# halajun/diasss

Hardware: AMD Instinct MI355X
Metric: sonar frames/sec end-to-end (extract+match+LM solve) (higher is better)
Workload: dtype u8/int32 (extract, match) + f64 (geo gate, LM); 1 GPU; 200 synthetic 2000x1024 frames, dense all-pairs; frames=200, pings=2000, bins=1024, pairs=19900

## Files before the change

diasss_amd/csrc/dsss_pg.hip:

```cpp
#include "dsss_internal.h"
#include "dsss_lm.h"
#include <utility>
#include "dsss_pg_kernels.h"
#include <algorithm>
#include <numeric>
#include <random>
#include <cstdlib>
#include <chrono>
#include <thread>
#include <mutex>
#include <future>

namespace {

struct pg_dev {
    dsss_ctx* ctx = nullptr;
    int rc = DSSS_OK;
    static constexpr size_t CHUNK = (size_t)256 << 20;
    template <typename T> int alloc(dsss_ctx* c, T** p, size_t n) { void* q = nullptr; if (!rc) rc = grab(c, &q, std::max<size_t>(n, 1) * sizeof(T)); *p = (T*)q; return rc; }
    int grab(dsss_ctx* c, void** p, size_t n) {
        if (!ctx) { ctx = c; c->pg_chunk_cur = 0; c->pg_chunk_off = 0; }
        const size_t bytes = (n + 255) & ~(size_t)255;
        for (;;) {
            if (c->pg_chunk_cur < c->pg_chunks.size()) {
                auto& ch = c->pg_chunks[c->pg_chunk_cur];
                if (c->pg_chunk_off + bytes <= ch.second) { *p = (char*)ch.first + c->pg_chunk_off; c->pg_chunk_off += bytes; return DSSS_OK; }
                ++c->pg_chunk_cur; c->pg_chunk_off = 0;
                continue;
            }
            void* q = nullptr; const size_t sz = std::max(bytes, CHUNK);
            HIPCHK(c, hipMalloc(&q, sz));
            c->pg_chunks.push_back({ q, sz });
        }
    }
    template <typename T> int upload(dsss_ctx* c, T** p, const std::vector<T>& v) { if (!alloc(c, p, v.size()) && !v.empty()) rc = copy(c, *p, v.data(), v.size() * sizeof(T)); return rc; }
    static int copy(dsss_ctx* c, void* d, const void* h, size_t bytes) { HIPCHK(c, hipMemcpy(d, h, bytes, hipMemcpyHostToDevice)); return DSSS_OK; }
    struct pend { void** p; const void* src; size_t bytes, off; };
    std::vector<pend> pending; size_t pend_total = 0;
    template <typename T> void later(T** p, const std::vector<T>& v) {
        *p = nullptr;
        pending.push_back({ (void**)p, v.data(), v.size() * sizeof(T), pend_total });
        pend_total += (std::max<size_t>(v.size(), 1) * sizeof(T) + 255) & ~(size_t)255;
    }
    hipEvent_t stage_ev = nullptr; bool stage_ev_live = false;
    int flush(dsss_ctx* c, hipStream_t st) { if (!rc) rc = flush_now(c, st); return rc; }
    int flush_now(dsss_ctx* c, hipStream_t st) {
        if (pending.empty()) return DSSS_OK;
        if (stage_ev_live) { hipEventSynchronize(stage_ev); stage_ev_live = false; }
        char* dev = nullptr;
        if (alloc(c, &dev, pend_total)) return rc;
        if (const int r = c->pg_stage.reserve(c, pend_total, pend_total + pend_total / 4)) return r;
        char* stage = c->pg_stage.as<char>();
        const int T = pend_total > ((size_t)1 << 20) ? 4 : 1;
        dsss_pool_run(T, [&](int t) { for (size_t k = t; k < pending.size(); k += T) if (pending[k].bytes) memcpy(stage + pending[k].off, pending[k].src, pending[k].bytes); });
        HIPCHK(c, hipMemcpyAsync(dev, stage, pend_total, hipMemcpyHostToDevice, st));
        if (!stage_ev) stage_ev = event();
        if (stage_ev) { hipEventRecord(stage_ev, st); stage_ev_live = true; }
        for (const pend& q : pending) *q.p = dev + q.off;
        pending.clear(); pend_total = 0;
        return DSSS_OK;
    }
    std::vector<hipEvent_t> events;
    hipEvent_t event() { hipEvent_t e = nullptr; hipEventCreateWithFlags(&e, hipEventDisableTiming); events.push_back(e); return e; }
    void release() { stage_ev_live = false; stage_ev = nullptr; if (ctx) { hipStreamSynchronize(ctx->stream); ctx->pg_chunk_cur = 0; ctx->pg_chunk_off = 0; } for (hipEvent_t e : events) if (e) hipEventDestroy(e); events.clear(); pending.clear(); pend_total = 0; }
};

}

void dsss_pg_free(dsss_ctx* c) { for (auto& ch : c->pg_chunks) hipFree(ch.first); c->pg_chunks.clear(); c->pg_chunk_cur = 0; c->pg_chunk_off = 0; }

namespace {

double ms_since(std::chrono::steady_clock::time_point t) { return std::chrono::duration<double, std::milli>(std::chrono::steady_clock::now() - t).count(); }

struct pg_window { int f0 = 0, p0 = 0; bool online = false; };

struct pg_solve {
    dsss_ctx* const c; const double* const dr6; const int n; const dsss_lc_edge* const edges; const int ne;
    double* const poses12; double* const stats4; double* const rpy6; const int nframes; const int* const ends; const pg_window win;
    const pg_switches sw = pg_switches_read();
    const hipStream_t st;
    int world = 1, rank = 0, nparts = 1, part_lo = 0, part_hi = 1, mp0 = 0, mp1 = 0;
    std::vector<int> foff, pbound;
    pg_weights W;
    std::vector<int> ea, eb, eo; std::vector<pose_t> emeas; std::vector<double> ew;
    std::vector<unsigned long long> tbits; std::vector<int> tpre;
    std::vector<int> sep1, sep_pose, t2, sym_part, ord1, ord2, adj_ptr, adj_edge, lc_link;
    int ns = 0, nseg = 0, ns1 = 0, nseg1 = 0, kp0 = 0, kp1 = 0, nf = 0, nblk = 0;
    std::vector<std::pair<int, int>> redges;
    std::vector<double> cx, cy, sxy; std::vector<unsigned long long> fp;
    static constexpr int chunk = 16;
    pg_analysis A;
    const pg_sym& S = A.S;
    std::promise<void> bottom_prom, lists_prom, coords_prom;
    std::future<void> bottom_fut = bottom_prom.get_future(), lists_fut = lists_prom.get_future(), coords_fut = coords_prom.get_future();
    bool bottom_signalled = false, lists_signalled = false, coords_given = false;
    std::thread sym_thread;
    pg_dev dv;
    pose_t *d_X, *d_Xn, *d_meas, *d_emeas; int *d_ea, *d_eb, *d_eo, *d_adj_ptr, *d_adj_edge, *d_lc_link = nullptr;
    int *d_sep, *d_sep1, *d_t2, *d_ord1, *d_ord2, *d_foff = nullptr; unsigned long long* d_fp = nullptr;
    double *d_dr6, *d_sxy, *d_ew, *d_r, *d_Ji, *d_r2, *d_Ji2, *d_D, *d_C, *d_g, *d_delta, *d_E, *d_Dl, *d_gi, *d_sDL, *d_sDR, *d_sGL, *d_sGR, *d_sS;
    double *d_D1, *d_C1, *d_g1, *d_E1, *d_Dl1, *d_gi1, *d_delta1, *d_s2DL, *d_s2DR, *d_s2GL, *d_s2GR, *d_s2S;
    double *d_part, *d_scal, *d_red; int* d_fail;
    int *d_perm, *d_binperm = nullptr, *d_colptr, *d_rowidx, *d_rlptr, *d_rlcol, *d_rlpos, *d_rlrow, *d_binptr, *d_bincols, *d_dest, *d_map; long long* d_mapptr;
    int *d_binroot_ptr, *d_binroot_idx, *d_broot_b, *d_broot_of_col, *d_anc_first, *d_anc_rel, *d_rel, *d_fa_src, *d_fa_col, *d_fa_tr, *d_frows, *d_xr_ptr;
    int *d_xr_child, *d_xr_row, *d_fa_rowptr, *d_pk_child, *d_pk_row, *d_ifslot = nullptr, *d_ifsep = nullptr;
    long long* d_broot_uoff; pg_front* d_FD; pg_child* d_CH; pg_pack* d_PK;
    double *d_rdiag, *d_x, *d_L, *d_ubin, *d_aval, *d_F, *d_R, *d_FL, *d_Tinv, *d_bwp = nullptr;
    double *d_comm = nullptr, *d_avalif = nullptr, *d_xif = nullptr, *d_commU = nullptr;
    struct dsched { int *lv_front, *lv_step, *asm_front, *asm_row, *tile_item, *tile_ij; } DO = {}, DI = {};
    std::vector<int> ifslot;
    size_t nnzL = 0, ncv = 0, nif = 0, comm_total = 8, if_ld = 0, if_count = 0;
    int nval = 0, bin_lo = 0, bin_hi = 0, nbins = 0, n_pack = 0, f_if = -1, bwd_lds = 0;
    double lambda = 0, err = 0, err0 = 0;
    int iters = 0, nfact = 0;
    bool will_iterate = false, pre_lin = false, pre_chain = false, pre_bins = false;

    pg_solve(dsss_ctx* c_, const double* dr6_, int n_, const dsss_lc_edge* edges_, int ne_, double* poses12_, double* stats4_, double* rpy6_ = nullptr,
             int nframes_ = 0, const int* ends_ = nullptr, pg_window win_ = {})
        : c(c_), dr6(dr6_), n(n_), edges(edges_), ne(ne_), poses12(poses12_), stats4(stats4_), rpy6(rpy6_), nframes(nframes_), ends(ends_), win(win_), st(c_->stream) {}
    ~pg_solve() {
        give_coords();
        if (sym_thread.joinable()) sym_thread.join();
        dv.release();
    }
    void give_coords() { if (!coords_given) { coords_given = true; coords_prom.set_value(); } }

    int run() {
        const auto T0 = std::chrono::steady_clock::now();
        int rc = plan();
        if (rc || (rc = separators())) return rc;
        const auto T1 = std::chrono::steady_clock::now();
        start_analysis();
        if ((rc = upload_dr()) || (rc = upload_chain())) return rc;
        const double t_prep = ms_since(T0);
        if ((rc = upload_links()) || (rc = initial_values()) || (rc = early_trial()) || (rc = join_analysis())) return rc;
        const double t_sym = ms_since(T1);
        const auto T2 = std::chrono::steady_clock::now();
        if ((rc = upload_fronts())) return rc;
        const double t_up = ms_since(T2);
        const auto T3 = std::chrono::steady_clock::now();
        dsss_scope sc(c, DSSS_K_PG);
        if ((rc = lm_loop())) return rc;
        const double t_lm = ms_since(T3);
        const auto T4 = std::chrono::steady_clock::now();
        if ((rc = finish())) return rc;
        if (sw.opt.verbose)
            fprintf(stderr, "[dsss pg] LM iterations %d  factorisations %d  err %.6g -> %.6g | host prep %.1f ms, symbolic %.1f ms, "
                    "alloc+upload %.1f ms, LM loop %.1f ms, download %.1f ms\n", iters, nfact, err0, err, t_prep, t_sym, t_up, t_lm, ms_since(T4));
        return DSSS_OK;
    }

    int plan() {
        if (!dr6) { foff.assign(nframes + 1, 0); for (int f = 0; f < nframes; ++f) foff[f + 1] = foff[f] + c->frames[win.f0 + f].N; }
        if (n < 2) DSSS_FAIL(c, DSSS_E_ARG, "pose graph needs at least 2 poses");
        world = dsss_comm_world(c); rank = dsss_comm_rank(c);
        nparts = std::max(world, c->pg_parts > 0 ? c->pg_parts : world);
        nparts = std::min(nparts, dr6 ? std::max(1, n / 4) : std::max(1, nframes));
        if (nparts < world) DSSS_FAIL(c, DSSS_E_ARG, "%d ranks need at least %d frames", world, world);
        pbound.assign(nparts + 1, n);
        for (int p = 0; p < nparts; ++p) pbound[p] = dr6 ? (int)((long long)n * p / nparts) : foff[(int)((long long)nframes * p / nparts)];
        for (int p = 0; p < nparts; ++p) if (pbound[p + 1] <= pbound[p]) DSSS_FAIL(c, DSSS_E_ARG, "empty pose-graph partition %d", p);
        part_lo = (int)((long long)nparts * rank / world); part_hi = (int)((long long)nparts * (rank + 1) / world);
        mp0 = pbound[part_lo]; mp1 = pbound[part_hi];
        const double PI = DSSS_PI_REF;
        { const double wgt1 = 0.001, wgt2 = 10;
          const double so[6] = { wgt1 * PI / 180, wgt1 * PI / 180, 0.1 * wgt1 * wgt2 * PI / 180, wgt1 * wgt2, wgt1 * wgt2, wgt1 };
          for (int k = 0; k < 6; ++k) { W.prior[k] = 1.0 / 0.000001; W.odo[k] = 1.0 / so[k]; } }
        ea.resize(ne); eb.resize(ne); eo.resize(ne);
        const int TE = ne >= 65536 ? 8 : 1;
        std::vector<int> bad(TE, -1);
        dsss_pool_run(TE, [&](int t) {
            const int e0 = (int)((long long)ne * t / TE), e1 = (int)((long long)ne * (t + 1) / TE);
            for (int e = e0; e < e1; ++e) {
                if (ends) { ea[e] = ends[2 * (size_t)e]; eb[e] = ends[2 * (size_t)e + 1]; } else { ea[e] = edges[e].a; eb[e] = edges[e].b; }
                eo[e] = std::max(ea[e], eb[e]);
                if ((ea[e] < 0 || ea[e] >= n || eb[e] < 0 || eb[e] >= n || ea[e] == eb[e]) && bad[t] < 0) bad[t] = e;
            }
        });
        for (int t = 0; t < TE; ++t) if (bad[t] >= 0) DSSS_FAIL(c, DSSS_E_ARG, "LC edge %d out of range", bad[t]);
        return DSSS_OK;
    }
    void mark(int i) { tbits[(size_t)i >> 6] |= 1ull << (i & 63); }
    static int rank_of(const std::vector<unsigned long long>& bits, const std::vector<int>& pre, int pose) {
        return pre[(size_t)pose >> 6] + __builtin_popcountll(bits[(size_t)pose >> 6] & ((1ull << (pose & 63)) - 1ull));
    }
    int separators() {
        tbits.assign(((size_t)n + 63) / 64, 0ull);
        mark(0); mark(n - 1);
        for (int e = 0; e < ne; ++e) { mark(ea[e]); mark(eb[e]); }
        if (const int rc = nparts > 1 && ne > 0 ? move_boundaries() : DSSS_OK) return rc;
        for (int p = 1; p < nparts; ++p) mark(pbound[p] - 1);
        const int run = 16 * chunk;
        sep_pose.reserve((size_t)2 * ne + nparts + n / run + 8);
        int last = 0;
        for (size_t w = 0; w < tbits.size(); ++w)
            for (unsigned long long bits = tbits[w]; bits; bits &= bits - 1) {
                const int b = (int)(w * 64) + __builtin_ctzll(bits);
                for (;;) {
                    const long long nx = ((long long)last + run + chunk - 1) / chunk * chunk;
                    if (nx >= b) break;
                    sep_pose.push_back((int)nx); last = (int)nx;
                }
                sep_pose.push_back(b); last = b;
            }
        for (int v : sep_pose) mark(v);
        tpre.assign(tbits.size() + 1, 0);
        for (size_t w = 0; w < tbits.size(); ++w) tpre[w + 1] = tpre[w] + __builtin_popcountll(tbits[w]);
        ns = (int)sep_pose.size(); nseg = ns - 1;
        redges.reserve((size_t)ns + ne);
        sym_part.resize(ns);
        { int p = 0; for (int k = 0; k < ns; ++k) { while (p + 1 < nparts && sep_pose[k] >= pbound[p + 1]) ++p; sym_part[k] = p; } }
        return DSSS_OK;
    }
    int move_boundaries() {
        std::vector<int> lc_ends; lc_ends.reserve((size_t)2 * ne + 2);
        for (size_t w = 0; w < tbits.size(); ++w)
            for (unsigned long long bits = tbits[w]; bits; bits &= bits - 1) lc_ends.push_back((int)(w * 64) + __builtin_ctzll(bits));
        std::vector<int> pre(tbits.size() + 1, 0);
        for (size_t w = 0; w < tbits.size(); ++w) pre[w + 1] = pre[w] + __builtin_popcountll(tbits[w]);
        const int m = (int)lc_ends.size();
        std::vector<int> cross(m + 1, 0);
        for (int e = 0; e < ne; ++e) { const int lo = rank_of(tbits, pre, std::min(ea[e], eb[e])), hi = rank_of(tbits, pre, std::max(ea[e], eb[e])); cross[lo + 1]++; cross[hi + 1]--; }
        for (int i = 1; i <= m; ++i) cross[i] += cross[i - 1];
        const int width = n / nparts / 3;
        for (int p = 1; p < nparts; ++p) {
            int bcost = 0;
            const int best = pg_cheapest_gap(lc_ends.data(), cross, pbound[p], width, pbound[p - 1], &bcost);
            if (best > pbound[p - 1] && best < n) pbound[p] = best;
        }
        for (int p = 0; p < nparts; ++p) if (pbound[p + 1] <= pbound[p]) DSSS_FAIL(c, DSSS_E_ARG, "empty pose-graph partition %d", p);
        mp0 = pbound[part_lo]; mp1 = pbound[part_hi];
        return DSSS_OK;
    }

    void start_analysis() {
        cx.resize(ns); cy.resize(ns);
        sym_thread = std::thread([this] {
            pg_sym_opts opt = sw.opt;
            opt.on_bottom_ready = [&] { bottom_signalled = true; bottom_prom.set_value(); };
            opt.on_lists_ready = [&] { lists_signalled = true; lists_prom.set_value(); };
            opt.before_order = [&] { coords_fut.wait(); };
            opt.lists_on_device = true;
            for (int k = 0; k + 1 < ns; ++k) redges.push_back({ k, k + 1 });
            for (int e = 0; e < ne; ++e) redges.push_back({ rank_of(tbits, tpre, ea[e]), rank_of(tbits, tpre, eb[e]) });
            pg_analyse(ns, redges, cx.data(), cy.data(), sym_part.data(), nparts, part_lo, part_hi, world, rank, sw, std::move(opt), A);
            if (!lists_signalled) lists_prom.set_value();
            if (!bottom_signalled) bottom_prom.set_value();
        });
    }

    int upload_dr() {
        dv.alloc(c, &d_dr6, (size_t)n * 6); dv.alloc(c, &d_sxy, (size_t)ns * 2); dv.later(&d_sep, sep_pose);
        sxy.resize((size_t)ns * 2);
        if (!dr6) {
            fp.resize(nframes);
            for (int f = 0; f < nframes; ++f) fp[f] = (unsigned long long)(uintptr_t)c->frames[win.f0 + f].pose6;
            dv.later(&d_fp, fp); dv.later(&d_foff, foff);
        }
        if (dv.flush(c, st)) return dv.rc;
        if (dr6) HIPCHK(c, hipMemcpyAsync(d_dr6, dr6, (size_t)n * 6 * sizeof(double), hipMemcpyHostToDevice, st));
        else {
            hipLaunchKernelGGL(pg_gather_dr_kernel, dim3(8, nframes), dim3(256), 0, st, d_fp, d_foff, d_dr6);
            HIPCHK(c, hipGetLastError());
        }
        hipLaunchKernelGGL(pg_sep_xy_kernel, dim3((ns + 255) / 256), dim3(256), 0, st, ns, d_sep, d_dr6, d_sxy);
        HIPCHK(c, hipGetLastError());
        HIPCHK(c, hipMemcpyAsync(sxy.data(), d_sxy, sxy.size() * sizeof(double), hipMemcpyDeviceToHost, st));
        HIPCHK(c, hipStreamSynchronize(st));
        for (int k = 0; k < ns; ++k) { cx[k] = sxy[2 * (size_t)k]; cy[k] = sxy[2 * (size_t)k + 1]; }
        give_coords();
        emeas.resize(ne); ew.resize((size_t)ne * 6);
        const int TE = ne >= 65536 ? 4 : 1;
        std::vector<int> bad_var(TE, -1), bad_rel(TE, -1);
        dsss_pool_run(TE, [&](int t) {
            const int e0 = (int)((long long)ne * t / TE), e1 = (int)((long long)ne * (t + 1) / TE);
            for (int e = e0; e < e1; ++e) {
                for (int k = 0; k < 9; ++k) emeas[e].R[k] = edges[e].rel[k];
                for (int k = 0; k < 3; ++k) emeas[e].t[k] = edges[e].rel[9 + k];
                for (int k = 0; k < 6; ++k) {
                    if ((!(edges[e].var[k] > 0) || !std::isfinite(edges[e].var[k])) && bad_var[t] < 0) bad_var[t] = e * 6 + k;
                    ew[(size_t)e * 6 + k] = 1.0 / std::sqrt(edges[e].var[k]);
                }
                for (int k = 0; k < 12; ++k) if (!std::isfinite(edges[e].rel[k]) && bad_rel[t] < 0) bad_rel[t] = e;
            }
        });
        for (int t = 0; t < TE; ++t) {
            if (bad_var[t] >= 0) DSSS_FAIL(c, DSSS_E_NUMERIC, "LC edge %d: variance %d is not finite and positive", bad_var[t] / 6, bad_var[t] % 6);
            if (bad_rel[t] >= 0) DSSS_FAIL(c, DSSS_E_NUMERIC, "LC edge %d: relative pose is not finite", bad_rel[t]);
        }
        return DSSS_OK;
    }
    int upload_chain() {
        sep1.reserve(sep_pose.size() + n / chunk + 2); t2.reserve(sep_pose.size());
        for (size_t it = 0, m = 0; it < sep_pose.size() || m < (size_t)n;) {
            const long long a = it < sep_pose.size() ? sep_pose[it] : (1LL << 40), bm = m < (size_t)n ? (long long)m : (1LL << 40);
            if (a <= bm) { t2.push_back((int)sep1.size()); sep1.push_back((int)a); ++it; if (a == bm) m += chunk; }
            else { sep1.push_back((int)bm); m += chunk; }
        }
        ns1 = (int)sep1.size(); nseg1 = ns1 - 1;
        kp0 = (int)(std::lower_bound(sep1.begin(), sep1.end(), mp0) - sep1.begin()); kp1 = (int)(std::lower_bound(sep1.begin(), sep1.end(), mp1) - sep1.begin());
        dv.later(&d_sep1, sep1); dv.later(&d_t2, t2);
        auto by_length = [](const std::vector<int>& ends, std::vector<int>& ord) {
            const int m = (int)ends.size() - 1;
            ord.resize(std::max(m, 1));
            int maxlen = 0;
            for (int k = 0; k < m; ++k) maxlen = std::max(maxlen, ends[k + 1] - ends[k]);
            std::vector<int> cnt(maxlen + 2, 0);
            for (int k = 0; k < m; ++k) cnt[maxlen - (ends[k + 1] - ends[k]) + 1]++;
            for (int l = 0; l <= maxlen; ++l) cnt[l + 1] += cnt[l];
            for (int k = 0; k < m; ++k) ord[cnt[maxlen - (ends[k + 1] - ends[k])]++] = k;
        };
        by_length(sep1, ord1); by_length(t2, ord2);
        dv.later(&d_ord1, ord1); dv.later(&d_ord2, ord2);
        return dv.flush(c, st);
    }
    int upload_links() {
        adj_ptr.assign(n + 1, 0); adj_edge.resize(2 * (size_t)ne);
        for (int e = 0; e < ne; ++e) { adj_ptr[ea[e] + 1]++; adj_ptr[eb[e] + 1]++; }
        for (int i = 0; i < n; ++i) adj_ptr[i + 1] += adj_ptr[i];
        { std::vector<int> fill(adj_ptr.begin(), adj_ptr.end() - 1);
          for (int e = 0; e < ne; ++e) { adj_edge[fill[ea[e]]++] = e << 1; adj_edge[fill[eb[e]]++] = (e << 1) | 1; } }
        bool plain = true;
        for (int e = 0; e < ne && plain; ++e) plain = ea[e] < eb[e] && (e == 0 || eb[e - 1] < eb[e]);
        if (!plain) {
            std::vector<std::pair<unsigned long long, int>> key(ne);
            for (int e = 0; e < ne; ++e) key[e] = { ((unsigned long long)(unsigned)std::min(ea[e], eb[e]) << 32) | (unsigned)std::max(ea[e], eb[e]), e };
            std::sort(key.begin(), key.end());
            bool dups = false;
            for (int k = 0; k + 1 < ne && !dups; ++k) dups = key[k].first == key[k + 1].first;
            if (dups) {
                lc_link.assign((size_t)2 * ne, -1);
                for (int k = 0; k < ne; ++k) {
                    lc_link[2 * (size_t)key[k].second] = (k == 0 || key[k - 1].first != key[k].first) ? 1 : 0;
                    if (k + 1 < ne && key[k + 1].first == key[k].first) lc_link[2 * (size_t)key[k].second + 1] = key[k + 1].second;
                }
            }
        }
        nf = n + ne; nblk = (nf + 255) / 256;
        const size_t sg = std::max(nseg, 1);
        dv.alloc(c, &d_X, n); dv.alloc(c, &d_Xn, n); dv.alloc(c, &d_meas, n); dv.upload(c, &d_emeas, emeas);
        dv.upload(c, &d_ea, ea); dv.upload(c, &d_eb, eb); dv.upload(c, &d_eo, eo); dv.upload(c, &d_ew, ew);
        dv.upload(c, &d_adj_ptr, adj_ptr); dv.upload(c, &d_adj_edge, adj_edge);
        if (!lc_link.empty()) dv.upload(c, &d_lc_link, lc_link);
        dv.alloc(c, &d_r, (size_t)nf * 6); dv.alloc(c, &d_Ji, (size_t)nf * 36);
        dv.alloc(c, &d_r2, (size_t)nf * 6); dv.alloc(c, &d_Ji2, (size_t)nf * 36);
        dv.alloc(c, &d_D, (size_t)n * 36); dv.alloc(c, &d_C, (size_t)n * 36); dv.alloc(c, &d_g, (size_t)n * 6); dv.alloc(c, &d_delta, (size_t)n * 6);
        dv.alloc(c, &d_E, (size_t)n * 36); dv.alloc(c, &d_Dl, (size_t)n * 36); dv.alloc(c, &d_gi, (size_t)n * 6);
        dv.alloc(c, &d_sDL, (size_t)nseg1 * 36); dv.alloc(c, &d_sDR, (size_t)nseg1 * 36); dv.alloc(c, &d_sGL, (size_t)nseg1 * 6);
        dv.alloc(c, &d_sGR, (size_t)nseg1 * 6); dv.alloc(c, &d_sS, (size_t)nseg1 * 36);
        dv.alloc(c, &d_D1, (size_t)ns1 * 36); dv.alloc(c, &d_C1, (size_t)ns1 * 36); dv.alloc(c, &d_g1, (size_t)ns1 * 6); dv.alloc(c, &d_delta1, (size_t)ns1 * 6);
        dv.alloc(c, &d_E1, (size_t)ns1 * 36); dv.alloc(c, &d_Dl1, (size_t)ns1 * 36); dv.alloc(c, &d_gi1, (size_t)ns1 * 6);
        dv.alloc(c, &d_s2DL, sg * 36); dv.alloc(c, &d_s2DR, sg * 36); dv.alloc(c, &d_s2GL, sg * 6); dv.alloc(c, &d_s2GR, sg * 6); dv.alloc(c, &d_s2S, sg * 36);
        dv.alloc(c, &d_rdiag, (size_t)ns * 6);
        dv.alloc(c, &d_x, (size_t)ns * 6); dv.alloc(c, &d_part, (size_t)nblk); dv.alloc(c, &d_scal, 8); dv.alloc(c, &d_fail, 1); dv.alloc(c, &d_red, 8);
        return dv.rc;
    }

    int reduce_scalars(double* host3, int* failed) {
        if (world > 1) {
            hipLaunchKernelGGL(pg_comm_scal_kernel, dim3(1), dim3(64), 0, st, d_scal, d_fail, d_red);
            if (const int rc = dsss_comm_allreduce(c, d_red, 4, st)) return rc;
            double h4[4];
            HIPCHK(c, hipMemcpyAsync(h4, d_red, 4 * sizeof(double), hipMemcpyDeviceToHost, st));
            HIPCHK(c, hipStreamSynchronize(st));
            host3[0] = h4[0]; host3[1] = h4[1]; host3[2] = h4[2]; *failed = h4[3] != 0.0;
        } else {
            if (const int r = c->pg_scal_host.reserve(c, 8 * sizeof(double))) return r;
            double* const scal_host = c->pg_scal_host.as<double>();
            HIPCHK(c, hipMemcpyAsync(scal_host, d_scal, 3 * sizeof(double), hipMemcpyDeviceToHost, st));
            HIPCHK(c, hipMemcpyAsync(scal_host + 4, d_fail, sizeof(int), hipMemcpyDeviceToHost, st));
            HIPCHK(c, hipStreamSynchronize(st));
            host3[0] = scal_host[0]; host3[1] = scal_host[1]; host3[2] = scal_host[2];
            *failed = *reinterpret_cast<const int*>(scal_host + 4);
        }
        return DSSS_OK;
    }
    int initial_values() {
        double* d_norm = nullptr;
        if (c->pg.add_noise) {
            const long long need_pairs = 3LL * n;
            long long natt = (long long)(need_pairs * 1.32) + 4096;
            for (int attempt = 0;; ++attempt) {
                double* d_pairs; int* d_flags; int* d_bsum; int* d_total;
                const int nb = (int)((natt + 4095) / 4096);
                dv.alloc(c, &d_pairs, (size_t)natt * 2); dv.alloc(c, &d_flags, (size_t)natt); dv.alloc(c, &d_bsum, (size_t)nb); dv.alloc(c, &d_total, 1);
                if (!d_norm) dv.alloc(c, &d_norm, (size_t)need_pairs * 2);
                if (dv.rc) return dv.rc;
                const long long nthr = (natt + RNG_PER_THREAD - 1) / RNG_PER_THREAD;
                hipLaunchKernelGGL(pg_rng_attempts_kernel, dim3((unsigned)((nthr + 255) / 256)), dim3(256), 0, st, natt, d_pairs, d_flags);
                hipLaunchKernelGGL(pg_flag_blocksum_kernel, dim3(nb), dim3(256), 0, st, d_flags, natt, d_bsum);
                hipLaunchKernelGGL(pg_flag_scan_kernel, dim3(1), dim3(256), 0, st, d_bsum, nb, d_total);
                hipLaunchKernelGGL(pg_flag_compact_kernel, dim3(nb), dim3(256), 0, st, d_flags, d_pairs, natt, d_bsum, need_pairs, d_norm);
                int total_ok = 0;
                HIPCHK(c, hipMemcpyAsync(&total_ok, d_total, sizeof(int), hipMemcpyDeviceToHost, st));
                HIPCHK(c, hipStreamSynchronize(st));
                if (total_ok >= need_pairs) break;
                if (attempt > 3) DSSS_FAIL(c, DSSS_E_NUMERIC, "normal generator: not enough accepted attempts");
                natt *= 2;
            }
        }
        hipLaunchKernelGGL(pg_init_kernel, dim3((n + 255) / 256), dim3(256), 0, st, n, d_dr6, d_norm, c->pg.add_noise, d_X, d_meas);
        if (win.online && c->pg_warm_n > win.p0) {
            const pose_t* warm = c->pg_warm.as<const pose_t>() + win.p0;
            HIPCHK(c, hipMemcpyAsync(d_X, warm, (size_t)std::min(n, c->pg_warm_n - win.p0) * sizeof(pose_t), hipMemcpyDeviceToDevice, st));
            if (win.p0 > 0) HIPCHK(c, hipMemcpyAsync(d_meas, warm, sizeof(pose_t), hipMemcpyDeviceToDevice, st));
        }
        hipLaunchKernelGGL(pg_linearize_kernel<false>, dim3(nblk), dim3(256), 0, st, n, ne, d_X, d_meas, W, d_ea, d_eb, d_eo, d_emeas, d_ew, (double*)nullptr, (double*)nullptr, d_part, mp0, mp1);
        hipLaunchKernelGGL(pg_final_sum_kernel, dim3(1), dim3(256), 0, st, d_part, nblk, 0.5, d_scal);
        double h3[3]; int failed = 0;
        HIPCHK(c, hipMemsetAsync(d_fail, 0, sizeof(int), st));
        if (const int rc = reduce_scalars(h3, &failed)) return rc;
        lambda = c->pg.lambda0; err = err0 = h3[0];
        return DSSS_OK;
    }

    void chain_part() {
        hipMemsetAsync(d_fail, 0, sizeof(int), st);
        hipLaunchKernelGGL(pg_assemble_kernel, dim3((ns1 + PG_ASM_POSES - 1) / PG_ASM_POSES), dim3(6 * PG_ASM_POSES), 0, st, n, W, d_r, d_Ji, d_adj_ptr, d_adj_edge, d_ew, d_scal + 3, d_D, d_C, d_g, d_eo, mp0, mp1, d_sep1, ns1);
        hipLaunchKernelGGL(pg_segment_kernel<true>, dim3((nseg1 + 31) / 32), dim3(256), 0, st, nseg1, d_ord1, d_sep1, d_D, d_C, d_g, d_E, d_Dl, d_gi, d_sDL, d_sDR, d_sGL, d_sGR, d_sS, d_fail, mp0, mp1, d_r, d_Ji, W, d_scal + 3);
        hipLaunchKernelGGL(pg_chain1_kernel, dim3((unsigned)(((long long)ns1 * 42 + 255) / 256)), dim3(256), 0, st, ns1, d_sep1, d_D, d_g, d_sDL, d_sDR, d_sGL, d_sGR, d_sS, d_D1, d_C1, d_g1, mp0, mp1);
        if (nseg > 0) hipLaunchKernelGGL(pg_segment_kernel<false>, dim3((nseg + 31) / 32), dim3(256), 0, st, nseg, d_ord2, d_t2, d_D1, d_C1, d_g1, d_E1, d_Dl1, d_gi1, d_s2DL, d_s2DR, d_s2GL, d_s2GR, d_s2S, d_fail, kp0, kp1, (const double*)nullptr, (const double*)nullptr, W, (const double*)nullptr);
    }
    int early_trial() {
        will_iterate = err > 0 && c->pg.max_iters > 0;
        if (!will_iterate) return DSSS_OK;
        hipLaunchKernelGGL(pg_linearize_kernel<true>, dim3(nblk), dim3(256), 0, st, n, ne, d_X, d_meas, W, d_ea, d_eb, d_eo, d_emeas, d_ew, d_r, d_Ji, d_part, mp0, mp1);
        hipLaunchKernelGGL(pg_final_sum_kernel, dim3(1), dim3(256), 0, st, d_part, nblk, 0.5, d_scal);
        HIPCHK(c, hipMemcpyAsync(d_scal + 3, &lambda, sizeof(double), hipMemcpyHostToDevice, st));
        chain_part();
        pre_lin = pre_chain = true;
        if (nparts > 1) return DSSS_OK;
        lists_fut.wait();
        if (const int rc = upload_lists()) return rc;
        bottom_fut.wait();
        if (const int rc = upload_bottom()) return rc;
        bottom_trial(0.0);
        pre_bins = true;
        return DSSS_OK;
    }
    int upload_lists() {
        nnzL = S.rowidx.size();
        const int nsa = S.ns;
        char* d_binned = nullptr; int* d_rootof = nullptr;
        dv.later(&d_colptr, S.colptr); dv.later(&d_rowidx, S.rowidx); dv.later(&d_binned, S.binned); dv.later(&d_rootof, S.root_of);
        dv.flush(c, st);
        int *d_cnt, *d_cur, *d_bs32, *d_tot32; long long *d_bs64, *d_tot64;
        const int nsb = (nsa + 1023) / 1024;
        dv.alloc(c, &d_cnt, (size_t)nsa); dv.alloc(c, &d_cur, (size_t)nsa); dv.alloc(c, &d_bs32, (size_t)nsb); dv.alloc(c, &d_tot32, 1);
        dv.alloc(c, &d_bs64, (size_t)nsb); dv.alloc(c, &d_tot64, 1); dv.alloc(c, &d_rlptr, (size_t)nsa + 1); dv.alloc(c, &d_mapptr, (size_t)nsa + 1);
        dv.alloc(c, &d_rlcol, nnzL); dv.alloc(c, &d_rlpos, nnzL); dv.alloc(c, &d_rlrow, nnzL);
        if (dv.alloc(c, &d_anc_first, (size_t)nsa) || dv.alloc(c, &d_anc_rel, nnzL)) return dv.rc;
        if (nsb > 1024 * 1024) DSSS_FAIL(c, DSSS_E_CAPACITY, "%d separators", nsa);
        hipMemsetAsync(d_cnt, 0, sizeof(int) * (size_t)nsa, st); hipMemsetAsync(d_cur, 0, sizeof(int) * (size_t)nsa, st);
        hipMemsetAsync(d_anc_first, 0, sizeof(int) * (size_t)nsa, st); hipMemsetAsync(d_anc_rel, 0xff, sizeof(int) * nnzL, st);
        const dim3 gcol((nsa + 255) / 256);
        hipLaunchKernelGGL(pg_rl_count_kernel, gcol, dim3(256), 0, st, nsa, d_colptr, d_rowidx, d_binned, d_cnt);
        hipLaunchKernelGGL((pg_scan_block_kernel<int, 0>), dim3(nsb), dim3(1024), 0, st, nsa, d_cnt, d_colptr, d_rlptr, d_bs32);
        hipLaunchKernelGGL((pg_scan_tops_kernel<int>), dim3(1), dim3(1024), 0, st, nsb, d_bs32, d_tot32);
        hipLaunchKernelGGL((pg_scan_add_kernel<int>), dim3(nsb), dim3(1024), 0, st, nsa, d_rlptr, d_bs32, d_tot32);
        hipLaunchKernelGGL((pg_scan_block_kernel<long long, 1>), dim3(nsb), dim3(1024), 0, st, nsa, d_cnt, d_colptr, d_mapptr, d_bs64);
        hipLaunchKernelGGL((pg_scan_tops_kernel<long long>), dim3(1), dim3(1024), 0, st, nsb, d_bs64, d_tot64);
        hipLaunchKernelGGL((pg_scan_add_kernel<long long>), dim3(nsb), dim3(1024), 0, st, nsa, d_mapptr, d_bs64, d_tot64);
        hipLaunchKernelGGL(pg_rl_fill_kernel, gcol, dim3(256), 0, st, nsa, d_colptr, d_rowidx, d_binned, d_rlptr, d_cur, d_rlcol, d_rlpos);
        hipLaunchKernelGGL(pg_rl_sort_kernel, dim3((nsa + 3) / 4), dim3(256), 0, st, nsa, d_rlptr, d_rlcol, d_rlpos, d_rlrow, d_fail);
        hipLaunchKernelGGL(pg_anc_rel_kernel, gcol, dim3(256), 0, st, nsa, d_colptr, d_rowidx, d_binned, d_rootof, d_anc_first, d_anc_rel);
        const long long mapsz = 42LL * (long long)nnzL; const int nupd = (int)nnzL;
        if (mapsz > (1LL << 31)) DSSS_FAIL(c, DSSS_E_CAPACITY, "update map bound of %lld entries", mapsz);
        if (dv.alloc(c, &d_map, (size_t)mapsz)) return dv.rc;
        hipLaunchKernelGGL(pg_fill_map_kernel, dim3(2048), dim3(256), 0, st, d_map, d_tot64);
        if (nupd > 0) hipLaunchKernelGGL(pg_build_map_kernel, dim3((nupd + 255) / 256), dim3(256), 0, st, nupd, d_rlrow, d_rlptr, d_rlcol, d_rlpos, d_colptr, d_rowidx, d_mapptr, d_map, d_tot32);
        return DSSS_OK;
    }
    int upload_bottom() {
        nnzL = S.rowidx.size(); nval = A.local ? (int)A.dest_g.size() : (int)S.dest_bin.size();
        ncv = S.comm_vals.size(); nif = S.iface_seps.size();
        comm_total = ncv * 36 + nif * 6 + (size_t)S.comm_doubles + 8;
        dv.later(&d_perm, A.local ? A.perm_g : S.perm);
        dv.alloc(c, &d_L, nnzL * 36); dv.alloc(c, &d_ubin, (size_t)S.ubin_doubles);
        if (dv.alloc(c, &d_aval, (size_t)nval * 36 + comm_total)) return dv.rc;
        d_comm = d_aval + (size_t)nval * 36; d_avalif = d_comm; d_xif = d_comm + ncv * 36; d_commU = d_xif + nif * 6;
        if (A.local) ifslot.swap(A.ifslot_g);
        else { ifslot.assign(ns, -1); for (size_t q = 0; q < nif; ++q) ifslot[S.iface_seps[q]] = (int)q; }
        dv.later(&d_ifslot, ifslot); dv.later(&d_ifsep, A.local ? A.ifsep_g : S.iface_seps);
        dv.later(&d_binptr, S.binptr); dv.later(&d_bincols, S.bincols); dv.later(&d_binperm, S.bin_perm);
        dv.later(&d_dest, A.local ? A.dest_g : S.dest_bin);
        dv.later(&d_binroot_ptr, S.binroot_ptr); dv.later(&d_binroot_idx, S.binroot_idx); dv.later(&d_broot_b, S.broot_b); dv.later(&d_broot_uoff, S.broot_uoff);
        dv.later(&d_broot_of_col, S.broot_of_col);
        if (dv.flush(c, st)) return dv.rc;
        { const int nb_all = (int)S.binptr.size() - 1, sel_lo = A.local ? 0 : part_lo, sel_hi = A.local ? 1 : part_hi;
          bin_lo = 0; while (bin_lo < nb_all && S.bin_part[bin_lo] < sel_lo) ++bin_lo; bin_hi = bin_lo; while (bin_hi < nb_all && S.bin_part[bin_hi] < sel_hi) ++bin_hi; }
        nbins = bin_hi - bin_lo;
        return DSSS_OK;
    }
    void bottom_trial(double bins_flops) {
        hipMemsetAsync(d_L, 0, nnzL * 36 * sizeof(double), st);
        if (nparts > 1) hipMemsetAsync(d_comm, 0, comm_total * sizeof(double), st);
        hipLaunchKernelGGL(pg_scatter_base_kernel, dim3((unsigned)(((long long)ns * 78 + 255) / 256)), dim3(256), 0, st, ns, d_t2, d_perm, d_D1, d_g1, d_s2DL, d_s2DR, d_s2GL, d_s2GR, d_s2S, d_dest, d_L, d_aval, d_x,
                           d_ifslot, d_avalif, d_xif, kp0, kp1);
        if (ne > 0) hipLaunchKernelGGL(pg_scatter_lc_kernel, dim3((unsigned)(((long long)ne * 36 + 255) / 256)), dim3(256), 0, st, n, ne, ns, d_Ji, d_ew, d_dest, d_L, d_aval, d_avalif, d_eo, mp0, mp1, d_lc_link);
        if (nbins > 0) { dsss_scope s1(c, DSSS_K_PG_SUBTREE, bins_flops);
                         hipLaunchKernelGGL(sw.bins_serial ? pg_factor_subtree_serial_kernel : pg_factor_subtree_kernel, dim3(nbins), dim3(256), 0, st, d_binperm + bin_lo, d_binptr, d_bincols, d_colptr, d_rlptr, d_rlcol, d_rlpos, d_mapptr, d_map, d_L, d_x, d_fail,
                                            d_binroot_ptr, d_binroot_idx, d_broot_b, d_broot_uoff, d_broot_of_col, d_anc_first, d_anc_rel, d_ubin, d_rdiag); }
    }
    int join_analysis() {
        sym_thread.join();
        if (S.ownership_violations) DSSS_FAIL(c, DSSS_E_STATE, "pose-graph analysis: %d separators with a higher-rank neighbour are not interface", S.ownership_violations);
        return DSSS_OK;
    }

    int upload_fronts() {
        if (!pre_bins) {
            if (const int rc = upload_lists()) return rc;
            if (const int rc = upload_bottom()) return rc;
        } else if (c->prof.on) c->prof.work[DSSS_K_PG_SUBTREE] += std::max(0.0, S.flops_factor - S.flops_fronts);
        if (sw.opt.verbose)
            fprintf(stderr, "[dsss pg] rank %d/%d parts %d (own %d..%d, poses %d..%d)  %s analysis of %d separators  poses %d  LC edges %d  separators %d "
                    "(interface %zu)  nnz(L) blocks %zu  bins %d (%d cols)  fronts %d (largest %d block rows, arena %.0f MB)  panels %d in %d levels  "
                    "all-reduce %.1f MB\n", rank, world, nparts, part_lo, part_hi, mp0, mp1, A.local ? "rank-local" : "replicated", S.ns, n, ne, ns,
                    S.iface_seps.size(), nnzL, (int)S.binptr.size() - 1, (int)S.bincols.size(), (int)S.f_c0.size(), S.max_front_n, S.front_doubles * 8e-6,
                    S.npanels, S.nlev, (S.comm_doubles + 36.0 * S.comm_vals.size() + 6.0 * S.iface_seps.size()) * 8e-6);
        const int nfr = (int)S.f_c0.size();
        f_if = A.local && !S.iface_seps.empty() ? nfr - 1 : -1;
        if_ld = f_if >= 0 ? (size_t)S.f_ld[f_if] : 0; if_count = if_ld * if_ld + if_ld;
        if (f_if >= 0 && (S.f_part[f_if] != -1 || S.f_off[f_if] + (long long)(if_ld * if_ld) != S.front_doubles))
            DSSS_FAIL(c, DSSS_E_STATE, "pose-graph analysis: the interface front is not the last one");
        dv.alloc(c, &d_F, (size_t)S.front_doubles + if_ld); dv.alloc(c, &d_R, (size_t)S.frhs_doubles); dv.alloc(c, &d_FL, (size_t)S.front_doubles);
        dv.later(&d_rel, S.rel); dv.later(&d_fa_src, S.fa_src); dv.later(&d_fa_col, S.fa_col); dv.later(&d_fa_tr, S.fa_tr);
        dv.later(&d_frows, S.f_rows); dv.later(&d_xr_ptr, S.xr_ptr); dv.later(&d_xr_child, S.xr_child);
        dv.later(&d_xr_row, S.xr_row); dv.later(&d_fa_rowptr, S.fa_rowptr);
        for (int w2 = 0; w2 < 2; ++w2) {
            const pg_sched& H = w2 ? A.SI : A.SO; dsched& Dv = w2 ? DI : DO;
            dv.later(&Dv.lv_front, H.lv_front); dv.later(&Dv.lv_step, H.lv_step); dv.later(&Dv.asm_front, H.asmrow_front); dv.later(&Dv.asm_row, H.asmrow_row);
            dv.later(&Dv.tile_item, H.tile_item); dv.later(&Dv.tile_ij, H.tile_ij);
        }
        std::vector<pg_front> FD(nfr); std::vector<pg_child> CH(S.ch_kind.size());
        for (int f = 0; f < nfr; ++f) {
            pg_front& d = FD[f];
            d.off = S.f_off[f]; d.roff = S.f_roff[f]; d.ld = S.f_ld[f]; d.n6 = 6 * S.f_n[f]; d.s6 = 6 * S.f_s[f]; d.c0 = S.f_c0[f];
            d.rowptr = S.f_rowptr[f]; d.pan0 = S.f_pan0[f]; d.ch0 = S.ch_ptr[f]; d.ch1 = S.ch_ptr[f + 1]; d.fa0 = S.fa_ptr[f]; d.fa1 = S.fa_ptr[f + 1];
            if (f == f_if) d.roff = (d_F + S.front_doubles) - d_R;
        }
        for (size_t q = 0; q < CH.size(); ++q) {
            pg_child& d = CH[q]; d.relptr = S.ch_relptr[q];
            if (S.ch_kind[q]) { const int ri = S.ch_id[q]; d.cb = S.broot_b[ri]; d.cld = 6 * d.cb; d.U = d_ubin + S.broot_uoff[ri]; d.g = d.U + (size_t)d.cld * d.cld; }
            else { const int gf = S.ch_id[q]; d.cb = S.f_n[gf] - S.f_s[gf]; d.cld = S.f_ld[gf]; d.U = d_F + S.f_off[gf] + (size_t)(6 * S.f_s[gf]) * d.cld + 6 * S.f_s[gf]; d.g = d_R + S.f_roff[gf] + 6 * S.f_s[gf]; }
        }
        std::vector<int> comm_of_front(nfr, -1), comm_of_broot(S.broot.size(), -1);
        for (size_t q = 0; q < S.comm_kind.size(); ++q) (S.comm_kind[q] ? comm_of_broot[S.comm_id[q]] : comm_of_front[S.comm_id[q]]) = (int)q;
        std::vector<pg_pack> PK(S.comm_kind.size()); std::vector<int> pk_child, pk_row;
        for (int f = 0; f < nfr; ++f) {
            if (S.f_part[f] >= 0) continue;
            for (int q = S.ch_ptr[f]; q < S.ch_ptr[f + 1]; ++q) {
                const int cq = S.ch_kind[q] ? comm_of_broot[S.ch_id[q]] : comm_of_front[S.ch_id[q]];
                if (cq < 0) continue;
                pg_child& d = CH[q];
                pg_pack& k = PK[cq]; k.U = d.U; k.g = d.g; k.cld = d.cld; k.cb = d.cb; k.dst = d_commU + S.comm_off[cq];
                d.U = k.dst; d.cld = 6 * d.cb; d.g = d.U + (size_t)d.cld * d.cld;
                if (S.comm_part[cq] >= part_lo && S.comm_part[cq] < part_hi) for (int r2 = 0; r2 < d.cb; ++r2) { pk_child.push_back(cq); pk_row.push_back(r2); }
            }
        }
        dv.later(&d_FD, FD); dv.later(&d_CH, CH); dv.later(&d_PK, PK); dv.later(&d_pk_child, pk_child); dv.later(&d_pk_row, pk_row);
        if (dv.flush(c, st)) return dv.rc;
        n_pack = (int)pk_child.size();
        const int max_n6 = std::max(A.SO.max_n6, A.SI.max_n6);
        c->pg_last_levels.clear();
        for (const pg_sched* H : { &A.SO, &A.SI })
            for (int l = 0; l < H->nlev; ++l) {
                const int nit = H->lv_ptr[l + 1] - H->lv_ptr[l];
                if (nit > 0) c->pg_last_levels.insert(c->pg_last_levels.end(), { nit, H->max_w6[l], H->max_rows[l], H == &A.SI ? 1 : 0 });
            }
        dv.alloc(c, &d_Tinv, (size_t)std::max(S.npanels, 1) * PG_NB4 * 16);
        size_t need = 0;
        for (const pg_sched* H : { &A.SO, &A.SI })
            for (int l = 0; l < H->nlev; ++l)
                if (64 * H->trsm_chunks[l] > PG_BWD_SPLIT) need = std::max(need, (size_t)(H->lv_ptr[l + 1] - H->lv_ptr[l]) * ((64 * H->trsm_chunks[l] + PG_BWD_RC - 1) / PG_BWD_RC) * 96);
        if ((need > 0 && dv.alloc(c, &d_bwp, need)) || dv.rc) return dv.rc;
        bwd_lds = (int)(((PG_PW * 6) * PG_BWD2_LD + PG_NB4 * 16 + 10 * (PG_PW * 6) + std::min(max_n6, PG_BWD2_SX) + 16) * sizeof(double));
        if (bwd_lds > 160 * 1024) DSSS_FAIL(c, DSSS_E_CAPACITY, "front of %d scalar rows: back-substitution needs %d B of LDS", max_n6, bwd_lds);
        hipFuncSetAttribute((const void*)pg_front_bwd2_kernel, hipFuncAttributeMaxDynamicSharedMemorySize, 160 * 1024);
        (void)hipGetLastError();
        return DSSS_OK;
    }

    void run_levels(const pg_sched& H, const dsched& Dv, int part = 0) {
        for (int l = 0; l < H.nlev; ++l) {
            const int nas = part == 2 ? 0 : H.asmrow_ptr[l + 1] - H.asmrow_ptr[l], nit = part == 1 ? 0 : H.lv_ptr[l + 1] - H.lv_ptr[l], ntl = H.tile_ptr[l + 1] - H.tile_ptr[l];
            const int* itf = Dv.lv_front + H.lv_ptr[l]; const int* its = Dv.lv_step + H.lv_ptr[l];
            if (nas > 0) { dsss_scope s2(c, DSSS_K_PG_ASM);
                hipLaunchKernelGGL(pg_front_asm_kernel, dim3(nas), dim3(256), 0, st, Dv.asm_front + H.asmrow_ptr[l], Dv.asm_row + H.asmrow_ptr[l], d_FD, d_CH, d_rel, d_xr_ptr, d_xr_child, d_xr_row,
                                   d_fa_rowptr, d_fa_src, d_fa_col, d_fa_tr, d_aval, d_x, d_F, d_R); }
            if (nit == 0) continue;
            { dsss_scope s3(c, DSSS_K_PG_DIAG, H.fl_diag[l]);
              hipLaunchKernelGGL(pg_front_diag4_kernel, dim3(nit), dim3(256), 0, st, itf, its, d_FD, d_F, d_R, d_fail, d_Tinv); }
            if (ntl > 0 && ntl <= PG_RSU_MAX_TILES) {
                dsss_scope s45(c, DSSS_K_PG_RSU, H.fl_trsm[l] + H.fl_syrk[l]);
                if (ntl <= PG_RSU32_MAX_TILES)
                    hipLaunchKernelGGL(pg_front_rsu_kernel<32>, dim3(4 * ntl), dim3(256), 0, st, itf, its, d_FD, Dv.tile_item + H.tile_ptr[l], Dv.tile_ij + H.tile_ptr[l], d_F, d_FL, d_R, d_Tinv);
                else hipLaunchKernelGGL(pg_front_rsu_kernel<64>, dim3(ntl), dim3(512), 0, st, itf, its, d_FD, Dv.tile_item + H.tile_ptr[l], Dv.tile_ij + H.tile_ptr[l], d_F, d_FL, d_R, d_Tinv);
            } else if (H.trsm_chunks[l] > 0) {
                { dsss_scope s4(c, DSSS_K_PG_TRSM, H.fl_trsm[l]);
                  hipLaunchKernelGGL(pg_front_trsm2_kernel, dim3(nit, H.trsm_chunks[l]), dim3(256), 0, st, itf, its, d_FD, d_F, d_R, d_Tinv); }
                { dsss_scope s5(c, DSSS_K_PG_ACC, H.fl_syrk[l]);
                  if (ntl > 0) hipLaunchKernelGGL(pg_front_syrk_kernel, dim3(ntl), dim3(256), 0, st, itf, its, d_FD, Dv.tile_item + H.tile_ptr[l], Dv.tile_ij + H.tile_ptr[l], d_F); }
            }
        }
    }
    void run_levels_bwd(const pg_sched& H, const dsched& Dv) {
        for (int l = H.nlev - 1; l >= 0; --l) {
            const int nit = H.lv_ptr[l + 1] - H.lv_ptr[l];
            if (nit == 0) continue;
            dsss_scope s6(c, DSSS_K_PG_BWD, H.fl_bwd[l], 2);
            const int ntl = H.tile_ptr[l + 1] - H.tile_ptr[l];
            const double* Fl = (ntl > 0 && ntl <= PG_RSU_MAX_TILES) ? d_FL : d_F;
            const int nch = 64 * H.trsm_chunks[l] > PG_BWD_SPLIT ? (64 * H.trsm_chunks[l] + PG_BWD_RC - 1) / PG_BWD_RC : 0;
            if (nch > 0) hipLaunchKernelGGL(pg_front_bwd_part_kernel, dim3(nch, nit), dim3(1024), 0, st, Dv.lv_front + H.lv_ptr[l], Dv.lv_step + H.lv_ptr[l], d_FD, d_frows, Fl, d_x, d_bwp, nch);
            hipLaunchKernelGGL(pg_front_bwd2_kernel, dim3(nit), dim3(1024), bwd_lds, st, Dv.lv_front + H.lv_ptr[l], Dv.lv_step + H.lv_ptr[l], d_FD, d_frows, d_F, Fl, d_R, d_x, d_Tinv,
                               nch > 0 ? (const double*)d_bwp : (const double*)nullptr, nch);
        }
    }
    int trial() {
        if (!pre_chain) {
            HIPCHK(c, hipMemcpyAsync(d_scal + 3, &lambda, sizeof(double), hipMemcpyHostToDevice, st));
            chain_part();
        }
        pre_chain = false;
        if (!pre_bins) bottom_trial(std::max(0.0, S.flops_factor - S.flops_fronts));
        pre_bins = false;
        run_levels(A.SO, DO);
        if (A.local) {
            if (f_if >= 0) {
                hipLaunchKernelGGL(pg_comm_xif_kernel, dim3(((int)nif + 255) / 256), dim3(256), 0, st, (int)nif, d_ifsep, d_perm, d_xif, d_x);
                hipMemsetAsync(d_F + S.f_off[f_if], 0, if_count * sizeof(double), st);
                run_levels(A.SI, DI, 1);
                { dsss_scope s8(c, DSSS_K_PG_COMM, (double)if_count * 8);
                  if (const int rc = dsss_comm_allreduce(c, d_F + S.f_off[f_if], if_count, st)) return rc; }
                run_levels(A.SI, DI, 2);
                run_levels_bwd(A.SI, DI);
            }
        } else if (nparts > 1) {
            if (n_pack > 0) hipLaunchKernelGGL(pg_comm_pack_kernel, dim3(n_pack), dim3(256), 0, st, d_pk_child, d_pk_row, d_PK);
            { dsss_scope s8(c, DSSS_K_PG_COMM, (double)comm_total * 8);
              if (const int rc = dsss_comm_allreduce(c, d_comm, comm_total - 8, st)) return rc; }
            if (nif > 0) hipLaunchKernelGGL(pg_comm_xif_kernel, dim3(((int)nif + 255) / 256), dim3(256), 0, st, (int)nif, d_ifsep, d_perm, d_xif, d_x);
            run_levels(A.SI, DI);
            run_levels_bwd(A.SI, DI);
        }
        run_levels_bwd(A.SO, DO);
        if (nbins > 0) { dsss_scope s7(c, DSSS_K_PG_SUBTREE);
            hipLaunchKernelGGL(pg_bwd_subtree_kernel, dim3(nbins), dim3(64), 0, st, d_binperm + bin_lo, d_binptr, d_bincols, d_colptr, d_rowidx, d_L, d_x, d_rdiag); }
        hipLaunchKernelGGL(pg_sep_delta_kernel, dim3((ns + 255) / 256), dim3(256), 0, st, ns, d_t2, d_perm, d_x, d_delta1);
        if (nseg > 0)
            hipLaunchKernelGGL(pg_backsub_kernel<false>, dim3((nseg + 31) / 32), dim3(256), 0, st, nseg, d_ord2, d_t2, d_C1, d_E1, d_Dl1, d_gi1, d_delta1, kp0, kp1, (const double*)nullptr, W);
        hipLaunchKernelGGL(pg_sep_delta_kernel, dim3((ns1 + 255) / 256), dim3(256), 0, st, ns1, d_sep1, (const int*)nullptr, d_delta1, d_delta);
        hipLaunchKernelGGL(pg_backsub_kernel<true>, dim3((nseg1 + 31) / 32), dim3(256), 0, st, nseg1, d_ord1, d_sep1, d_C, d_E, d_Dl, d_gi, d_delta, mp0, mp1, d_Ji, W);
        hipLaunchKernelGGL(pg_linerr_kernel, dim3(nblk), dim3(256), 0, st, n, ne, W, d_ea, d_eb, d_eo, d_ew, d_r, d_Ji, d_delta, d_part, mp0, mp1);
        hipLaunchKernelGGL(pg_final_sum_kernel, dim3(1), dim3(256), 0, st, d_part, nblk, 0.5, d_scal + 1);
        return DSSS_OK;
    }

    int lm_loop() {
        const lm_rule R = { c->pg.rel_tol, c->pg.abs_tol, c->pg.lambda_max, c->pg.min_fidelity, c->pg.lambda_factor, c->pg.max_iters };
        double cur = 0;
        if (will_iterate) do {
            cur = err;
            double oldLin = err;
            if (!pre_lin) {
                hipLaunchKernelGGL(pg_linearize_kernel<true>, dim3(nblk), dim3(256), 0, st, n, ne, d_X, d_meas, W, d_ea, d_eb, d_eo, d_emeas, d_ew, d_r, d_Ji, d_part, mp0, mp1);
                hipLaunchKernelGGL(pg_final_sum_kernel, dim3(1), dim3(256), 0, st, d_part, nblk, 0.5, d_scal);
            }
            pre_lin = false;
            for (;;) {
                if (const int rc = trial()) return rc;
                ++nfact;
                hipLaunchKernelGGL(pg_retract_kernel, dim3((n + 255) / 256), dim3(256), 0, st, n, d_X, d_delta, d_Xn);
                hipLaunchKernelGGL(pg_linearize_kernel<true>, dim3(nblk), dim3(256), 0, st, n, ne, d_Xn, d_meas, W, d_ea, d_eb, d_eo, d_emeas, d_ew, d_r2, d_Ji2, d_part, mp0, mp1);
                hipLaunchKernelGGL(pg_final_sum_kernel, dim3(1), dim3(256), 0, st, d_part, nblk, 0.5, d_scal + 2);
                HIPCHK(c, hipGetLastError());
                double h[3]; int failed = 0;
                if (const int rc = reduce_scalars(h, &failed)) return rc;
                const lm_verdict v = !failed && std::isfinite(h[1]) ? lm_judge(R, oldLin, h[1], err, h[2]) : lm_verdict{ false, false };
                if (v.success) { std::swap(d_X, d_Xn); std::swap(d_r, d_r2); std::swap(d_Ji, d_Ji2); pre_lin = true; err = h[2]; lm_accepted(R, &lambda); ++iters; break; }
                if (v.stop || lm_refused(R, &lambda)) break;
            }
        } while (lm_continue(R, iters, cur, err));
        return DSSS_OK;
    }

    int finish() {
        if (world > 1) {
            size_t maxlen = 0;
            std::vector<int> r_lo(world), r_len(world);
            for (int r = 0; r < world; ++r) {
                r_lo[r] = pbound[(int)((long long)nparts * r / world)]; r_len[r] = pbound[(int)((long long)nparts * (r + 1) / world)] - r_lo[r];
                maxlen = std::max(maxlen, (size_t)r_len[r]);
            }
            const size_t slice = maxlen * sizeof(pose_t);
            char* d_gath;
            if (dv.alloc(c, &d_gath, slice * (size_t)world)) return dv.rc;
            HIPCHK(c, hipMemcpyAsync(d_gath + slice * (size_t)rank, d_X + mp0, (size_t)(mp1 - mp0) * sizeof(pose_t), hipMemcpyDeviceToDevice, st));
            if (const int rc = dsss_comm_allgather(c, d_gath, slice, st)) return rc;
            for (int r = 0; r < world; ++r)
                if (r != rank && r_len[r] > 0) HIPCHK(c, hipMemcpyAsync(d_X + r_lo[r], d_gath + slice * (size_t)r, (size_t)r_len[r] * sizeof(pose_t), hipMemcpyDeviceToDevice, st));
        }
        static_assert(sizeof(pose_t) == 12 * sizeof(double), "pose_t layout");
        const int p0 = win.p0;
        if (win.online) {
            const size_t all = (size_t)p0 + (size_t)n;
            if (const int r = c->pg_warm.reserve_keep(c, all * sizeof(pose_t), (all + all / 2 + 1024) * sizeof(pose_t), (size_t)p0 * sizeof(pose_t))) return r;
            HIPCHK(c, hipMemcpyAsync(c->pg_warm.as<pose_t>() + p0, d_X, (size_t)n * sizeof(pose_t), hipMemcpyDeviceToDevice, st));
            c->pg_warm_n = (int)all;
        }
        const pose_t* d_out = p0 > 0 ? c->pg_warm.as<const pose_t>() : d_X;
        const int n_out = p0 + n;
        if (poses12)
            HIPCHK(c, hipMemcpyAsync(poses12, d_out, (size_t)n_out * sizeof(pose_t), hipMemcpyDeviceToHost, st));
        if (rpy6) {
            double* d_rpy;
            if (dv.alloc(c, &d_rpy, (size_t)n_out * 6)) return dv.rc;
            hipLaunchKernelGGL(pg_rpy_kernel, dim3((n_out + 255) / 256), dim3(256), 0, st, n_out, d_out, d_rpy);
            HIPCHK(c, hipMemcpyAsync(rpy6, d_rpy, (size_t)n_out * 6 * sizeof(double), hipMemcpyDeviceToHost, st));
        }
        HIPCHK(c, hipStreamSynchronize(st));
        if (stats4) { stats4[0] = iters; stats4[1] = err0; stats4[2] = err; stats4[3] = lambda; }
        c->pg_last_trials = nfact;
        return DSSS_OK;
    }
};

}

__global__ __launch_bounds__(256) void lc_select_kernel(const double* __restrict__ kp7, int n, const int* __restrict__ kp7_pair,
                                                        const int* __restrict__ kp7_off, const int* __restrict__ act_t,
                                                        const int* __restrict__ frame_off, unsigned long long* __restrict__ slot)
{
    const int i = blockIdx.x * 256 + threadIdx.x;
    if (i >= n) return;
    const int p = kp7_pair[i];
    const int t = act_t[p];
    const int ping = (int)kp7[(size_t)i * 7 + 3];
    const unsigned long long key = ((unsigned long long)(unsigned)(p + 1) << 32) | (unsigned long long)(0xffffffffu - (unsigned)(i - kp7_off[p]));
    atomicMax(&slot[frame_off[t] + ping], key);
}

__global__ __launch_bounds__(256) void lc_edge_flag_kernel(const unsigned long long* __restrict__ slot, int total, const int* __restrict__ kp7_off,
                                                           const dsss_lc* __restrict__ lcs, int* __restrict__ flags)
{
    const int g = blockIdx.x * 256 + threadIdx.x;
    if (g >= total) return;
    const unsigned long long key = slot[g];
    int f = 0;
    if (key) {
        const int p = (int)(key >> 32) - 1, k = (int)(0xffffffffu - (unsigned)(key & 0xffffffffu));
        const dsss_lc& m = lcs[kp7_off[p] + k];
        f = m.score > 0 && isfinite(m.score);
        for (int q = 0; q < 6; ++q) f = f && m.var[q] > 0 && isfinite(m.var[q]);
    }
    flags[g] = f;
}

#define PG_AB_PREFIX 32768
static int pg_select_impl(dsss_ctx* c, int nframes, dsss_lc_edge* edges, int cap, int* n_edges, const int** ends)
{
    if (!c || nframes <= 0 || nframes > c->max_frames) return DSSS_E_ARG;
    if (!c->has_lc) DSSS_FAIL(c, DSSS_E_STATE, "dsss_lc_solve_all has not run");
    HIPCHK(c, hipSetDevice(c->device));
    std::vector<int> off(nframes + 1, 0);
    for (int f = 0; f < nframes; ++f) {
        if (!c->frames[f].has_geom) DSSS_FAIL(c, DSSS_E_STATE, "frame %d has no geometry", f);
        off[f + 1] = off[f] + c->frames[f].N;
    }
    const int total = off[nframes], n = c->total_kp7;
    int ne = 0;
    if (n > 0) {
        for (int p = 0; p < c->npairs; ++p)
            if (c->pair_s[p] >= nframes || c->pair_t[p] >= nframes) DSSS_FAIL(c, DSSS_E_ARG, "pair %d references a frame >= nframes", p);
        pg_dev dv;
        unsigned long long* d_slot; int *d_off, *d_flags, *d_bsum, *d_total; dsss_lc_edge* d_edges; int2* d_ab = nullptr;
        const int nb = (total + 4095) / 4096;
        int rc = dv.alloc(c, &d_slot, (size_t)total); if (rc) return rc;
        rc = dv.alloc(c, &d_off, (size_t)nframes + 1); if (rc) return rc;
        rc = dv.alloc(c, &d_flags, (size_t)total); if (rc) return rc;
        rc = dv.alloc(c, &d_bsum, (size_t)nb); if (rc) return rc;
        rc = dv.alloc(c, &d_total, 1); if (rc) return rc;
        rc = dv.alloc(c, &d_edges, (size_t)cap); if (rc) return rc;
        if (ends) {
            rc = dv.alloc(c, &d_ab, (size_t)cap); if (rc) return rc;
            if ((rc = c->pg_ab_host.reserve(c, (size_t)cap * sizeof(int2)))) return rc;
        }
        hipStream_t st = c->stream;
        HIPCHK(c, hipMemsetAsync(d_slot, 0, (size_t)total * sizeof(unsigned long long), st));
        HIPCHK(c, hipMemcpyAsync(d_off, off.data(), (nframes + 1) * sizeof(int), hipMemcpyHostToDevice, st));
        hipLaunchKernelGGL(lc_select_kernel, dim3((n + 255) / 256), dim3(256), 0, st, c->kp7, n, c->kp7_pair, c->kp7_off, c->act_t, d_off, d_slot);
        hipLaunchKernelGGL(lc_edge_flag_kernel, dim3((total + 255) / 256), dim3(256), 0, st, d_slot, total, c->kp7_off, c->lcs.as<dsss_lc>(), d_flags);
        hipLaunchKernelGGL(pg_flag_blocksum_kernel, dim3(nb), dim3(256), 0, st, d_flags, (long long)total, d_bsum);
        hipLaunchKernelGGL(pg_flag_scan_kernel, dim3(1), dim3(256), 0, st, d_bsum, nb, d_total);
        hipLaunchKernelGGL(lc_edge_compact_kernel, dim3(nb), dim3(256), 0, st, d_flags, d_bsum, d_slot, total, c->kp7_off, c->kp7, c->lcs.as<dsss_lc>(), c->act_s, d_off, cap, d_edges, d_ab);
        HIPCHK(c, hipGetLastError());
        HIPCHK(c, hipMemcpyAsync(&ne, d_total, sizeof(int), hipMemcpyDeviceToHost, st));
        const int pre = std::min(cap, PG_AB_PREFIX);
        if (ends) HIPCHK(c, hipMemcpyAsync(c->pg_ab_host.p, d_ab, (size_t)pre * sizeof(int2), hipMemcpyDeviceToHost, st));
        HIPCHK(c, hipStreamSynchronize(st));
        if (ne > cap) { dv.release(); DSSS_FAIL(c, DSSS_E_CAPACITY, "more than %d LC edges", cap); }
        if (ends) {
            if (ne > pre) { HIPCHK(c, hipMemcpyAsync(c->pg_ab_host.as<int>() + 2 * (size_t)pre, d_ab + pre, (size_t)(ne - pre) * sizeof(int2), hipMemcpyDeviceToHost, st)); HIPCHK(c, hipStreamSynchronize(st)); }
            if (ne > 0) HIPCHK(c, hipMemcpyAsync(edges, d_edges, (size_t)ne * sizeof(dsss_lc_edge), hipMemcpyDeviceToHost, st));
            *ends = c->pg_ab_host.as<int>();
        }
        else if (ne > 0) HIPCHK(c, hipMemcpy(edges, d_edges, (size_t)ne * sizeof(dsss_lc_edge), hipMemcpyDeviceToHost));
        dv.release();
    }
    else if (ends) *ends = nullptr;
    if (n_edges) *n_edges = ne;
    return DSSS_OK;
}

static int pg_exchange_edges(dsss_ctx* c, dsss_lc_edge** edges, int* n_edges)
{
    const int world = dsss_comm_world(c), rank = dsss_comm_rank(c);
    dsss_lc_edge* edges_p = *edges;
    int ne = *n_edges, rc;
    std::vector<double> cnt(world, 0.0); cnt[rank] = ne;
    auto xch = [&](size_t n) { return c->xch_dev.reserve(c, n * sizeof(double), (n + n / 2 + 1024) * sizeof(double)); };
    rc = xch(world); if (rc) return rc;
    double* d_tmp = c->xch_dev.as<double>();
    hipError_t e = hipMemcpyAsync(d_tmp, cnt.data(), world * sizeof(double), hipMemcpyHostToDevice, c->stream);
    if (e == hipSuccess) { rc = dsss_comm_allreduce(c, d_tmp, world, c->stream); if (rc) return rc; }
    if (e == hipSuccess) e = hipMemcpyAsync(cnt.data(), d_tmp, world * sizeof(double), hipMemcpyDeviceToHost, c->stream);
    if (e == hipSuccess) e = hipStreamSynchronize(c->stream);
    HIPCHK(c, e);
    size_t tot = 0, maxc = 0;
    for (int r = 0; r < world; ++r) { tot += (size_t)cnt[r]; maxc = std::max(maxc, (size_t)cnt[r]); }
    if (tot > 0) {
        const size_t slice = maxc * sizeof(dsss_lc_edge), all = slice * (size_t)world;
        rc = xch((2 * all + sizeof(double) - 1) / sizeof(double)); if (rc) return rc;
        if ((rc = c->xch_host.reserve(c, all, all + all / 2))) return rc;
        char* d_all = c->xch_dev.as<char>();
        char* d_cmp = d_all + all;
        e = hipSuccess;
        if (ne > 0) e = hipMemcpyAsync(d_all + slice * (size_t)rank, edges_p, (size_t)ne * sizeof(dsss_lc_edge), hipMemcpyHostToDevice, c->stream);
        if (e == hipSuccess) { rc = dsss_comm_allgather(c, d_all, slice, c->stream); if (rc) return rc; }
        size_t w = 0;
        for (int r = 0; r < world && e == hipSuccess; ++r) {
            const size_t k = (size_t)cnt[r];
            if (k) e = hipMemcpyAsync(d_cmp + w * sizeof(dsss_lc_edge), d_all + slice * (size_t)r, k * sizeof(dsss_lc_edge), hipMemcpyDeviceToDevice, c->stream);
            w += k;
        }
        if (e == hipSuccess) e = hipMemcpyAsync(c->xch_host.p, d_cmp, tot * sizeof(dsss_lc_edge), hipMemcpyDeviceToHost, c->stream);
        if (e == hipSuccess) e = hipStreamSynchronize(c->stream);
        HIPCHK(c, e);
        edges_p = c->xch_host.as<dsss_lc_edge>();
    }
    ne = (int)tot;
    bool ascending = true;
    for (int i = 1; i < ne && ascending; ++i) ascending = edges_p[i - 1].b <= edges_p[i].b;
    if (!ascending) std::stable_sort(edges_p, edges_p + ne, [](const dsss_lc_edge& x, const dsss_lc_edge& y) { return x.b < y.b; });
    *edges = edges_p; *n_edges = ne;
    return DSSS_OK;
}

extern "C" {

int dsss_posegraph_select(dsss_ctx* c, int nframes, dsss_lc_edge* edges, int cap, int* n_edges) { return pg_select_impl(c, nframes, edges, cap, n_edges, nullptr); }

int dsss_posegraph_solve_edges(dsss_ctx* c, const double* dr6, int total, const dsss_lc_edge* edges, int ne, double* poses12, double* stats4)
{
    if (!c || !dr6 || total <= 0 || ne < 0 || (ne > 0 && !edges)) return DSSS_E_ARG;
    HIPCHK(c, hipSetDevice(c->device));
    std::vector<double> h_dr((size_t)total * 6);
    HIPCHK(c, hipMemcpy(h_dr.data(), dr6, h_dr.size() * sizeof(double), hipMemcpyDefault));
    std::vector<dsss_lc_edge> h_e(ne);
    if (ne) HIPCHK(c, hipMemcpy(h_e.data(), edges, (size_t)ne * sizeof(dsss_lc_edge), hipMemcpyDefault));
    return pg_solve(c, h_dr.data(), total, h_e.data(), ne, poses12, stats4).run();
}

int dsss_posegraph_solve(dsss_ctx* c, int nframes, double* poses12, double* rpy6, double* stats4)
{
    if (!c || nframes <= 0 || nframes > c->max_frames) return DSSS_E_ARG;
    const auto t0 = std::chrono::steady_clock::now();
    auto ms = [&](std::chrono::steady_clock::time_point a) { return std::chrono::duration<double, std::milli>(std::chrono::steady_clock::now() - a).count(); };
    size_t total = 0;
    for (int f = 0; f < nframes; ++f) {
        if (!c->frames[f].has_geom) DSSS_FAIL(c, DSSS_E_STATE, "frame %d has no geometry", f);
        total += (size_t)c->frames[f].N;
    }
    const size_t ecap = (size_t)std::max(c->total_kp7, 1);
    if (const int r = c->pg_edges_host.reserve(c, ecap * sizeof(dsss_lc_edge))) return r;
    dsss_lc_edge* edges_p = c->pg_edges_host.as<dsss_lc_edge>();
    int ne = 0;
    const double t_dr = ms(t0);
    const auto t1 = std::chrono::steady_clock::now();
    const int world = dsss_comm_world(c);
    const int* ends = nullptr;
    int rc = pg_select_impl(c, nframes, edges_p, (int)ecap, &ne, world == 1 ? &ends : nullptr);
    if (rc) return rc;
    if (world > 1 && (rc = pg_exchange_edges(c, &edges_p, &ne))) return rc;
    const double t_sel = ms(t1);
    const auto t2 = std::chrono::steady_clock::now();
    rc = pg_solve(c, nullptr, (int)total, edges_p, ne, poses12, stats4, rpy6, nframes, ends).run();
    if (rc) return rc;
    if (pg_switches_read().opt.verbose) fprintf(stderr, "[dsss pg] DR rows %.1f ms, LC selection %.1f ms, solve + download %.1f ms\n", t_dr, t_sel, ms(t2));
    return DSSS_OK;
}

int dsss_posegraph_reset(dsss_ctx* c)
{
    if (!c) return DSSS_E_ARG;
    c->pg_inc_edges.clear(); c->pg_inc_gen = c->lc_gen; c->pg_warm_n = 0;
    return DSSS_OK;
}

int dsss_posegraph_online_edges(dsss_ctx* c) { return c ? (int)c->pg_inc_edges.size() : DSSS_E_ARG; }

int dsss_posegraph_schedule_get(dsss_ctx* c, int* levels4, int cap_levels, int* n_levels, int* n_trials)
{
    if (!c || (cap_levels > 0 && !levels4)) return DSSS_E_ARG;
    const int nl = (int)(c->pg_last_levels.size() / 4);
    if (n_levels) *n_levels = nl;
    if (n_trials) *n_trials = c->pg_last_trials;
    for (int l = 0; l < std::min(nl, cap_levels); ++l) for (int k = 0; k < 4; ++k) levels4[4 * l + k] = c->pg_last_levels[4 * (size_t)l + k];
    return DSSS_OK;
}

static int pg_update_impl(dsss_ctx* c, int nframes, int window_frames, double* poses12, double* rpy6, double* stats4)
{
    if (!c || nframes <= 0 || nframes > c->max_frames) return DSSS_E_ARG;
    if (dsss_comm_world(c) > 1) DSSS_FAIL(c, DSSS_E_STATE, "dsss_posegraph_update is a single-rank call (the online use is one vehicle, one GPU)");
    size_t total = 0;
    for (int f = 0; f < nframes; ++f) {
        if (!c->frames[f].has_geom) DSSS_FAIL(c, DSSS_E_STATE, "frame %d has no geometry", f);
        total += (size_t)c->frames[f].N;
    }
    for (const dsss_lc_edge& e : c->pg_inc_edges)
        if (e.a >= (int)total || e.b >= (int)total)
            DSSS_FAIL(c, DSSS_E_ARG, "an accumulated LC edge references ping %d of %zu: nframes went down; dsss_posegraph_reset first", std::max(e.a, e.b), total);
    if (c->has_lc && c->pg_inc_gen != c->lc_gen && c->total_kp7 > 0) {
        std::vector<dsss_lc_edge> fresh((size_t)c->total_kp7);
        int ne = 0;
        const int rc = dsss_posegraph_select(c, nframes, fresh.data(), (int)fresh.size(), &ne);
        if (rc) return rc;
        if (ne > 0 && !c->pg_inc_edges.empty()) {
            std::vector<char> hit(total, 0);
            for (int e = 0; e < ne; ++e) hit[fresh[e].b] = 1;
            size_t w = 0;
            for (size_t e = 0; e < c->pg_inc_edges.size(); ++e) if (!hit[c->pg_inc_edges[e].b]) c->pg_inc_edges[w++] = c->pg_inc_edges[e];
            c->pg_inc_edges.resize(w);
        }
        const bool append_only = ne == 0 || c->pg_inc_edges.empty() || c->pg_inc_edges.back().b <= fresh[0].b;
        c->pg_inc_edges.insert(c->pg_inc_edges.end(), fresh.begin(), fresh.begin() + ne);
        if (!append_only) std::stable_sort(c->pg_inc_edges.begin(), c->pg_inc_edges.end(), [](const dsss_lc_edge& x, const dsss_lc_edge& y) { return x.b < y.b; });
    }
    c->pg_inc_gen = c->lc_gen;
    int f0 = window_frames > 0 ? std::max(0, nframes - window_frames) : 0;
    int p0 = 0;
    for (int f = 0; f < f0; ++f) p0 += c->frames[f].N;
    while (f0 > 0 && c->pg_warm_n <= p0) { --f0; p0 -= c->frames[f0].N; }
    if (f0 == 0)
        return pg_solve(c, nullptr, (int)total, c->pg_inc_edges.data(), (int)c->pg_inc_edges.size(), poses12, stats4, rpy6, nframes, nullptr, { 0, 0, true }).run();
    std::vector<dsss_lc_edge> we; std::vector<int> frozen;
    for (const dsss_lc_edge& e : c->pg_inc_edges) {
        if (std::max(e.a, e.b) < p0) continue;
        if (e.a >= p0 && e.b >= p0) { dsss_lc_edge w = e; w.a -= p0; w.b -= p0; we.push_back(w); continue; }
        if (e.a > e.b) DSSS_FAIL(c, DSSS_E_ARG, "window update: loop closure %d -> %d runs from the window into the frozen part (the pipeline's closures end in the later frame)", e.a, e.b);
        dsss_lc_edge w = e; w.b -= p0; w.a = -1 - (int)frozen.size(); frozen.push_back(e.a); we.push_back(w);
    }
    if (!frozen.empty()) {
        HIPCHK(c, hipSetDevice(c->device));
        std::vector<int> idx(frozen); idx.push_back(p0);
        pg_dev gv;
        int* d_idx = nullptr; pose_t* d_g = nullptr;
        int rg = gv.alloc(c, &d_idx, idx.size()); if (rg) return rg;
        rg = gv.alloc(c, &d_g, idx.size()); if (rg) { gv.release(); return rg; }
        std::vector<pose_t> g(idx.size());
        hipError_t e = hipMemcpyAsync(d_idx, idx.data(), idx.size() * sizeof(int), hipMemcpyHostToDevice, c->stream);
        if (e == hipSuccess) { hipLaunchKernelGGL(pg_gather_pose_kernel, dim3(((int)idx.size() + 255) / 256), dim3(256), 0, c->stream, (int)idx.size(), d_idx, c->pg_warm.as<const pose_t>(), d_g); e = hipGetLastError(); }
        if (e == hipSuccess) e = hipMemcpyAsync(g.data(), d_g, g.size() * sizeof(pose_t), hipMemcpyDeviceToHost, c->stream);
        gv.release();
        HIPCHK(c, e);
        pose_t X0inv; pose_inverse(&g.back(), &X0inv);
        for (dsss_lc_edge& w : we) {
            if (w.a >= 0) continue;
            const pose_t& Xa = g[(size_t)(-1 - w.a)];
            pose_t rel, Y, M;
            for (int k = 0; k < 9; ++k) rel.R[k] = w.rel[k];
            for (int k = 0; k < 3; ++k) rel.t[k] = w.rel[9 + k];
            pose_compose(&X0inv, &Xa, &Y); pose_compose(&Y, &rel, &M);
            for (int k = 0; k < 9; ++k) w.rel[k] = M.R[k];
            for (int k = 0; k < 3; ++k) w.rel[9 + k] = M.t[k];
            w.a = 0;
        }
    }
    return pg_solve(c, nullptr, (int)total - p0, we.data(), (int)we.size(), poses12, stats4, rpy6, nframes - f0, nullptr, { f0, p0, true }).run();
}

int dsss_posegraph_update(dsss_ctx* c, int nframes, double* poses12, double* rpy6, double* stats4) { return pg_update_impl(c, nframes, 0, poses12, rpy6, stats4); }
int dsss_posegraph_update_window(dsss_ctx* c, int nframes, int window_frames, double* poses12, double* rpy6, double* stats4)
{
    if (window_frames < 1) { if (c) c->err = "window_frames must be at least 1"; return DSSS_E_ARG; }
    return pg_update_impl(c, nframes, window_frames, poses12, rpy6, stats4);
}

}
```

diasss_amd/csrc/dsss_pg_bins.hip:

```cpp
#include "dsss_pg_kernels.h"
#include "dsss_pg_dev.h"
#pragma clang fp contract(fast)
__global__ __launch_bounds__(256) void pg_build_map_kernel(int nupd, const int* __restrict__ rlrow, const int* __restrict__ rlptr,
                                                           const int* __restrict__ rlcol, const int* __restrict__ rlpos,
                                                           const int* __restrict__ colptr, const int* __restrict__ rowidx,
                                                           const long long* __restrict__ mapptr, int* __restrict__ upd_map, const int* __restrict__ nupd_dev)
{
    const int e = blockIdx.x * 256 + threadIdx.x;
    if (e >= (nupd_dev ? *nupd_dev : nupd)) return;
    const int j = rlrow[e], k = rlcol[e];
    const int c0 = colptr[j], m = colptr[j + 1] - c0;
    int* mp = upd_map + mapptr[j] + (long long)(e - rlptr[j]) * m;
    int q = 0;
    for (int p = rlpos[e]; p < colptr[k + 1]; ++p) {
        const int i = rowidx[p];
        while (q < m && rowidx[c0 + q] < i) ++q;
        if (q < m && rowidx[c0 + q] == i) mp[q] = p;
    }
}

__global__ __launch_bounds__(256) void pg_rl_count_kernel(int ns, const int* __restrict__ colptr, const int* __restrict__ rowidx, const char* __restrict__ binned,
                                                          int* __restrict__ cnt)
{
    const int k = blockIdx.x * 256 + threadIdx.x;
    if (k >= ns || !binned[k]) return;
    for (int q = colptr[k] + 1; q < colptr[k + 1]; ++q) { const int j = rowidx[q]; if (binned[j]) atomicAdd(&cnt[j], 1); }
}
template <typename T, int VAL>
__global__ __launch_bounds__(1024) void pg_scan_block_kernel(int n, const int* __restrict__ cnt, const int* __restrict__ colptr, T* __restrict__ out, T* __restrict__ block_sum)
{
    __shared__ T s_w[16];
    const int i = blockIdx.x * 1024 + threadIdx.x;
    T v = 0, tot;
    if (i < n) v = VAL == 0 ? (T)cnt[i] : (T)cnt[i] * (T)(colptr[i + 1] - colptr[i]);
    const T pos = dsss_block_scan_excl<16, T>(v, &tot, s_w);
    if (i < n) out[i] = pos;
    if (threadIdx.x == 0) block_sum[blockIdx.x] = tot;
}
template <typename T>
__global__ __launch_bounds__(1024) void pg_scan_tops_kernel(int nblocks, T* __restrict__ block_sum, T* __restrict__ total)
{
    __shared__ T s_w[16];
    T carry = 0;
    for (int b0 = 0; b0 < nblocks; b0 += 1024) {
        const int i = b0 + threadIdx.x;
        const T v = i < nblocks ? block_sum[i] : (T)0;
        T tot;
        const T pos = dsss_block_scan_excl<16, T>(v, &tot, s_w);
        if (i < nblocks) block_sum[i] = carry + pos;
        carry += tot;
    }
    if (threadIdx.x == 0) *total = carry;
}
template <typename T>
__global__ __launch_bounds__(1024) void pg_scan_add_kernel(int n, T* __restrict__ out, const T* __restrict__ block_sum, const T* __restrict__ total)
{
    const int i = blockIdx.x * 1024 + threadIdx.x;
    if (i < n) out[i] += block_sum[blockIdx.x];
    if (i == 0) out[n] = *total;
}
__global__ __launch_bounds__(256) void pg_rl_fill_kernel(int ns, const int* __restrict__ colptr, const int* __restrict__ rowidx, const char* __restrict__ binned,
                                                         const int* __restrict__ rlptr, int* __restrict__ cur, int* __restrict__ rlcol, int* __restrict__ rlpos)
{
    const int k = blockIdx.x * 256 + threadIdx.x;
    if (k >= ns || !binned[k]) return;
    for (int q = colptr[k] + 1; q < colptr[k + 1]; ++q) {
        const int j = rowidx[q];
        if (!binned[j]) continue;
        const int at = rlptr[j] + atomicAdd(&cur[j], 1);
        rlcol[at] = k; rlpos[at] = q;
    }
}
#define PG_RL_SORT_CAP 1024
__global__ __launch_bounds__(256) void pg_rl_sort_kernel(int ns, const int* __restrict__ rlptr, int* __restrict__ rlcol, int* __restrict__ rlpos, int* __restrict__ rlrow,
                                                         int* __restrict__ fail)
{
    __shared__ int s_k[4][PG_RL_SORT_CAP], s_q[4][PG_RL_SORT_CAP];
    const int wv = threadIdx.x >> 6, lane = threadIdx.x & 63;
    const int j = blockIdx.x * 4 + wv;
    if (j >= ns) return;
    const int b = rlptr[j], len = rlptr[j + 1] - b;
    if (len <= 0) return;
    if (len > PG_RL_SORT_CAP) { if (lane == 0) *fail = 2; return; }
    for (int e = lane; e < len; e += 64) { s_k[wv][e] = rlcol[b + e]; s_q[wv][e] = rlpos[b + e]; }
    asm volatile("s_waitcnt vmcnt(0) lgkmcnt(0)" ::: "memory"); __builtin_amdgcn_wave_barrier();
    for (int e = lane; e < len; e += 64) {
        const int key = s_k[wv][e];
        int rank = 0;
        for (int f = 0; f < len; ++f) rank += s_k[wv][f] < key;
        rlcol[b + rank] = key; rlpos[b + rank] = s_q[wv][e]; rlrow[b + rank] = j;
    }
}
__global__ __launch_bounds__(256) void pg_fill_map_kernel(int* __restrict__ upd_map, const long long* __restrict__ total)
{
    const long long n = *total;
    for (long long i = (long long)blockIdx.x * 256 + threadIdx.x; i < n; i += (long long)gridDim.x * 256) upd_map[i] = -1;
}
__global__ __launch_bounds__(256) void pg_anc_rel_kernel(int ns, const int* __restrict__ colptr, const int* __restrict__ rowidx, const char* __restrict__ binned,
                                                         const int* __restrict__ root_of, int* __restrict__ anc_first, int* __restrict__ anc_rel)
{
    const int k = blockIdx.x * 256 + threadIdx.x;
    if (k >= ns || !binned[k]) return;
    const int r = root_of[k], c0 = colptr[k], m = colptr[k + 1] - c0;
    int q = 0;
    while (q < m && rowidx[c0 + q] <= r) ++q;
    anc_first[k] = q;
    const int* __restrict__ rb = rowidx + colptr[r] + 1; const int nb = colptr[r + 1] - colptr[r] - 1;
    int w = 0;
    for (; q < m; ++q) { const int row = rowidx[c0 + q]; while (w < nb && rb[w] < row) ++w; anc_rel[c0 + q] = (w < nb && rb[w] == row) ? w : -1; }
}

#define PG_TCH 128
__device__ inline void pg_acc_rows(const int* __restrict__ mp, int m, int tn, const double* __restrict__ Lvals, int r,
                                   const double* __restrict__ s_Ljk, double* acc)
{
    int t = 0;
    for (; t + 4 <= tn; t += 4) {
        int pos[4]; double a[4][6];
#pragma unroll
        for (int u = 0; u < 4; ++u) pos[u] = mp[(size_t)(t + u) * m];
#pragma unroll
        for (int u = 0; u < 4; ++u) {
            const double* Lik = Lvals + (size_t)(pos[u] < 0 ? 0 : pos[u]) * 36 + r * 6;
#pragma unroll
            for (int c = 0; c < 6; ++c) a[u][c] = Lik[c];
        }
#pragma unroll
        for (int u = 0; u < 4; ++u) {
            if (pos[u] < 0) continue;
            const double* B = s_Ljk + (t + u) * 36;
#pragma unroll
            for (int s = 0; s < 6; ++s)
                acc[s] += a[u][0] * B[s * 6] + a[u][1] * B[s * 6 + 1] + a[u][2] * B[s * 6 + 2] + a[u][3] * B[s * 6 + 3] + a[u][4] * B[s * 6 + 4] + a[u][5] * B[s * 6 + 5];
        }
    }
    for (; t < tn; ++t) {
        const int pos = mp[(size_t)t * m];
        if (pos < 0) continue;
        const double* Lik = Lvals + (size_t)pos * 36 + r * 6;
        const double* B = s_Ljk + t * 36;
        const double a0 = Lik[0], a1 = Lik[1], a2 = Lik[2], a3 = Lik[3], a4 = Lik[4], a5 = Lik[5];
#pragma unroll
        for (int s = 0; s < 6; ++s)
            acc[s] += a0 * B[s * 6] + a1 * B[s * 6 + 1] + a2 * B[s * 6 + 2] + a3 * B[s * 6 + 3] + a4 * B[s * 6 + 4] + a5 * B[s * 6 + 5];
    }
}
__global__ __launch_bounds__(256) void pg_factor_subtree_serial_kernel(const int* __restrict__ bin_perm, const int* __restrict__ binptr, const int* __restrict__ bincols,
                                                                const int* __restrict__ colptr, const int* __restrict__ rlptr,
                                                                const int* __restrict__ rlcol, const int* __restrict__ rlpos,
                                                                const long long* __restrict__ mapptr, const int* __restrict__ upd_map,
                                                                double* __restrict__ Lvals, double* __restrict__ x, int* __restrict__ fail,
                                                                const int* __restrict__ binroot_ptr, const int* __restrict__ binroot_idx,
                                                                const int* __restrict__ broot_b, const long long* __restrict__ broot_uoff,
                                                                const int* __restrict__ broot_of_col, const int* __restrict__ anc_first,
                                                                const int* __restrict__ anc_rel, double* __restrict__ ubin, double* __restrict__ rdiag)
{
    __shared__ double s_Ljk[PG_TCH * 36];
    __shared__ double s_yk[PG_TCH * 6];
    __shared__ double s_diag[36];
    __shared__ int s_arel[48];
    __shared__ double s_ri[6];
    __shared__ double s_y[6];
    __shared__ double s_xj[6];
    __shared__ int s_ok;
    const int bin = bin_perm[blockIdx.x];
    for (int q = binroot_ptr[bin]; q < binroot_ptr[bin + 1]; ++q) {
        const int ri = binroot_idx[q]; const long long b6 = 6LL * broot_b[ri]; double* U = ubin + broot_uoff[ri];
        for (long long e = threadIdx.x; e < b6 * b6 + b6; e += 256) U[e] = 0.0;
    }
    struct colinfo { int j, c0, m, t0, T, af, ri, b6; long long mapoff, uoff; };
    auto col_of = [&](int ci2) {
        colinfo k;
        k.j = bincols[ci2];
        k.c0 = colptr[k.j]; k.m = colptr[k.j + 1] - k.c0;
        k.t0 = rlptr[k.j]; k.T = rlptr[k.j + 1] - k.t0;
        k.mapoff = mapptr[k.j]; k.af = anc_first[k.j]; k.ri = broot_of_col[k.j];
        k.b6 = k.ri >= 0 ? 6 * broot_b[k.ri] : 0; k.uoff = k.ri >= 0 ? broot_uoff[k.ri] : 0;
        return k;
    };
    const int ci_end = binptr[bin + 1];
    colinfo cur = {}, nxt = {};
    if (binptr[bin] < ci_end) cur = col_of(binptr[bin]);
    for (int ci = binptr[bin]; ci < ci_end; ++ci, cur = nxt) {
        if (ci + 1 < ci_end) nxt = col_of(ci + 1);
        const int j = cur.j;
        const int c0 = cur.c0, m = cur.m;
        const int t0 = cur.t0, T = cur.T;
        const int* mp = upd_map + cur.mapoff;
        const int idx = threadIdx.x;
        const bool act = idx < 6 * m;
        const int q = act ? idx / 6 : 0, r = idx - q * 6;
        const bool rhs = threadIdx.x >= 250;
        const int rs_ = threadIdx.x - 250;
        double acc[6] = { 0, 0, 0, 0, 0, 0 }, accy = 0;
        double rowv[6] = { 0, 0, 0, 0, 0, 0 };
        if (act) {
#pragma unroll
            for (int s2 = 0; s2 < 6; ++s2) rowv[s2] = Lvals[(size_t)(c0 + q) * 36 + r * 6 + s2];
        }
        for (int tc = 0; tc < T; tc += PG_TCH) {
            const int tn = min(PG_TCH, T - tc);
            __syncthreads();
            for (int x0 = threadIdx.x; x0 < tn * 36; x0 += 4 * 256) {
                int pos[4]; double val[4];
#pragma unroll
                for (int u = 0; u < 4; ++u) { const int xx = x0 + u * 256; pos[u] = xx < tn * 36 ? rlpos[t0 + tc + xx / 36] : 0; }
#pragma unroll
                for (int u = 0; u < 4; ++u) { const int xx = x0 + u * 256; val[u] = xx < tn * 36 ? Lvals[(size_t)pos[u] * 36 + (xx % 36)] : 0.0; }
#pragma unroll
                for (int u = 0; u < 4; ++u) { const int xx = x0 + u * 256; if (xx < tn * 36) s_Ljk[xx] = val[u]; }
            }
            for (int xx = threadIdx.x; xx < tn * 6; xx += 256) s_yk[xx] = x[(size_t)rlcol[t0 + tc + xx / 6] * 6 + (xx % 6)];
            __syncthreads();
            if (rhs)
                for (int t = 0; t < tn; ++t) {
                    const double* yk = s_yk + t * 6; const double* B = s_Ljk + t * 36 + rs_ * 6;
                    accy += B[0] * yk[0] + B[1] * yk[1] + B[2] * yk[2] + B[3] * yk[3] + B[4] * yk[4] + B[5] * yk[5];
                }
            if (act)
                pg_acc_rows(mp + (size_t)tc * m + q, m, tn, Lvals, r, s_Ljk, acc);
        }
        if (rhs) s_xj[rs_] = x[(size_t)j * 6 + rs_] - accy;
        if (act) {
#pragma unroll
            for (int s = 0; s < 6; ++s) rowv[s] -= acc[s];
            if (idx < 6) { for (int s = 0; s < 6; ++s) s_diag[r * 6 + s] = rowv[s]; }
        }
        __syncthreads();
        if (threadIdx.x == 0) {
            double A[36], xj[6], ri[6];
#pragma unroll
            for (int a = 0; a < 36; ++a) A[a] = s_diag[a];
#pragma unroll
            for (int a = 0; a < 6; ++a) xj[a] = s_xj[a];
            const int bad = chol6_recip(A, ri);
            if (bad) *fail = 1;
            s_ok = !bad;
#pragma unroll
            for (int a = 0; a < 6; ++a)
#pragma unroll
                for (int b = 0; b < 6; ++b) { const double v = b <= a ? A[a * 6 + b] : 0.0; s_diag[a * 6 + b] = v; Lvals[(size_t)c0 * 36 + a * 6 + b] = v; }
#pragma unroll
            for (int a = 0; a < 6; ++a) { s_ri[a] = ri[a]; rdiag[(size_t)j * 6 + a] = ri[a]; }
            if (!bad) {
                double v[6];
#pragma unroll
                for (int a = 0; a < 6; ++a) {
                    double t = xj[a];
#pragma unroll
                    for (int b = 0; b < 6; ++b) if (b < a) t -= A[a * 6 + b] * v[b];
                    v[a] = t * ri[a];
                }
#pragma unroll
                for (int a = 0; a < 6; ++a) { x[(size_t)j * 6 + a] = v[a]; s_y[a] = v[a]; }
            }
        }
        __syncthreads();
        if (!s_ok) return;
        const int af = cur.af, ta = m - af;
        if (act && idx >= 6) {
            double* row = Lvals + (size_t)(c0 + q) * 36 + r * 6;
            double xr[6];
#pragma unroll
            for (int s = 0; s < 6; ++s) { double v = rowv[s];
#pragma unroll
                                          for (int c = 0; c < 6; ++c) if (c < s) v -= xr[c] * s_diag[s * 6 + c];
                                          xr[s] = v * s_ri[s]; }
            for (int s = 0; s < 6; ++s) row[s] = xr[s];
            if (q >= af) for (int s = 0; s < 6; ++s) s_Ljk[(q - af) * 36 + r * 6 + s] = xr[s];
        }
        __syncthreads();
        const int ri = cur.ri;
        if (ri >= 0 && ta > 0) {
            const int b6 = cur.b6;
            double* __restrict__ U = ubin + cur.uoff;
            double* __restrict__ g = U + (size_t)b6 * b6;
            if ((int)threadIdx.x < ta) s_arel[threadIdx.x] = anc_rel[c0 + af + threadIdx.x];
            __syncthreads();
            if ((int)threadIdx.x < 6 * ta) {
                const int pa = threadIdx.x / 6, a = threadIdx.x - pa * 6;
                const double* La = s_Ljk + pa * 36 + a * 6;
                g[s_arel[pa] * 6 + a] -= La[0] * s_y[0] + La[1] * s_y[1] + La[2] * s_y[2] + La[3] * s_y[3] + La[4] * s_y[4] + La[5] * s_y[5];
            }
            const int npair = ta * (ta + 1) / 2;
            for (int e = threadIdx.x; e < 36 * npair; e += 256) {
                const int pr = e / 36, ab = e - 36 * pr;
                int pa = (int)((sqrtf(8.0f * (float)pr + 1.0f) - 1.0f) * 0.5f);
                while (pa * (pa + 1) / 2 > pr) --pa;
                while ((pa + 1) * (pa + 2) / 2 <= pr) ++pa;
                const int pb = pr - pa * (pa + 1) / 2, a = ab / 6, b = ab - 6 * a;
                const double* La = s_Ljk + pa * 36 + a * 6; const double* Lb = s_Ljk + pb * 36 + b * 6;
                U[(size_t)(s_arel[pa] * 6 + a) * b6 + s_arel[pb] * 6 + b] -= La[0] * Lb[0] + La[1] * Lb[1] + La[2] * Lb[2] + La[3] * Lb[3] + La[4] * Lb[4] + La[5] * Lb[5];
            }
        }
        __syncthreads();
        __threadfence_block();
    }
}
#define PG_PCH 42
#define PG_NIDX 4
#define PG_DW 64
struct pg_coldesc { int j, c0, m, t0, T, af, ri, b6, fpos, c0p; long long mapoff, uoff; };
__device__ inline void pg_upd_term(double (&acc)[6], const double (&a)[6], const double* __restrict__ B)
{
#pragma unroll
    for (int s = 0; s < 6; ++s)
        acc[s] += a[0] * B[s * 6] + a[1] * B[s * 6 + 1] + a[2] * B[s * 6 + 2] + a[3] * B[s * 6 + 3] + a[4] * B[s * 6 + 4] + a[5] * B[s * 6 + 5];
}
__device__ inline void pg_upd_group(const int (&pos)[4], int t, const double* __restrict__ Lvals, int r, const double* __restrict__ s_B, double (&acc)[6])
{
    double a[4][6];
#pragma unroll
    for (int u = 0; u < 4; ++u) {
        const double* Lik = Lvals + (size_t)(pos[u] < 0 ? 0 : pos[u]) * 36 + r * 6;
#pragma unroll
        for (int c = 0; c < 6; ++c) a[u][c] = Lik[c];
    }
#pragma unroll
    for (int u = 0; u < 4; ++u) {
        if (pos[u] < 0) continue;
        pg_upd_term(acc, a[u], s_B + (t + u) * 36);
    }
}
__device__ inline void pg_acc_rows_ahead(const int (&mpi)[PG_NIDX], const int* __restrict__ mp, int m, int tn, const double* __restrict__ Lvals, int r,
                                         const double* __restrict__ s_B, double (&acc)[6])
{
    const int ng = (tn + 3) >> 2;
#pragma unroll
    for (int g = 0; g < PG_NIDX / 4; ++g)
        if (g < ng) {
            int pos[4];
#pragma unroll
            for (int u = 0; u < 4; ++u) pos[u] = 4 * g + u < tn ? mpi[4 * g + u] : -1;
            pg_upd_group(pos, 4 * g, Lvals, r, s_B, acc);
        }
    for (int g = PG_NIDX / 4; g < ng; ++g) {
        int pos[4];
#pragma unroll
        for (int u = 0; u < 4; ++u) pos[u] = mp[(size_t)min(4 * g + u, tn - 1) * m];
#pragma unroll
        for (int u = 0; u < 4; ++u) if (4 * g + u >= tn) pos[u] = -1;
        pg_upd_group(pos, 4 * g, Lvals, r, s_B, acc);
    }
}
__global__ __launch_bounds__(256, 3) void pg_factor_subtree_kernel(const int* __restrict__ bin_perm, const int* __restrict__ binptr, const int* __restrict__ bincols,
                                                                const int* __restrict__ colptr, const int* __restrict__ rlptr,
                                                                const int* __restrict__ rlcol, const int* __restrict__ rlpos,
                                                                const long long* __restrict__ mapptr, const int* __restrict__ upd_map,
                                                                double* __restrict__ Lvals, double* __restrict__ x, int* __restrict__ fail,
                                                                const int* __restrict__ binroot_ptr, const int* __restrict__ binroot_idx,
                                                                const int* __restrict__ broot_b, const long long* __restrict__ broot_uoff,
                                                                const int* __restrict__ broot_of_col, const int* __restrict__ anc_first,
                                                                const int* __restrict__ anc_rel, double* __restrict__ ubin, double* __restrict__ rdiag)
{
    __shared__ double s_st[2][PG_PCH * 36];
    __shared__ double s_sy[2][PG_PCH * 6];
    __shared__ double s_col[42 * 36];
    __shared__ double s_diag[36];
    __shared__ double s_ri[6];
    __shared__ double s_y[2][6];
    __shared__ int s_arel[2][48];
    __shared__ int s_di[PG_DW][10];
    __shared__ long long s_dl[PG_DW][2];
    __shared__ double s_xj[6];
    __shared__ int s_ok;
    const int tid = threadIdx.x;
    const int bin = bin_perm[blockIdx.x];
    for (int q = binroot_ptr[bin]; q < binroot_ptr[bin + 1]; ++q) {
        const int ri = binroot_idx[q]; const long long b6 = 6LL * broot_b[ri]; double* U = ubin + broot_uoff[ri];
        for (long long e = threadIdx.x; e < b6 * b6 + b6; e += 256) U[e] = 0.0;
    }
    const int ci0 = binptr[bin], ci_end = binptr[bin + 1];
    if (ci0 >= ci_end) return;
    auto fill = [&](int base, int cnt) {
        if (tid < cnt) {
            const int ci = base + tid, j = bincols[ci];
            const int c0 = colptr[j], m = colptr[j + 1] - c0, t0 = rlptr[j], T = rlptr[j + 1] - t0, ri = broot_of_col[j];
            int fpos = -1, c0p = 0;
            if (ci > ci0 && T > 0) {
                const int jp = bincols[ci - 1];
                if (rlcol[t0 + T - 1] == jp) { c0p = colptr[jp]; fpos = rlpos[t0 + T - 1] - c0p; }
            }
            int* d = s_di[(ci - ci0) & (PG_DW - 1)];
            d[0] = j; d[1] = c0; d[2] = m; d[3] = t0; d[4] = T; d[5] = anc_first[j]; d[6] = ri; d[7] = ri >= 0 ? 6 * broot_b[ri] : 0; d[8] = fpos; d[9] = c0p;
            long long* dl = s_dl[(ci - ci0) & (PG_DW - 1)];
            dl[0] = mapptr[j]; dl[1] = ri >= 0 ? broot_uoff[ri] : 0;
        }
    };
    auto desc = [&](int ci) {
        const int* d = s_di[(ci - ci0) & (PG_DW - 1)]; const long long* dl = s_dl[(ci - ci0) & (PG_DW - 1)];
        pg_coldesc k;
        k.j = __builtin_amdgcn_readfirstlane(d[0]); k.c0 = __builtin_amdgcn_readfirstlane(d[1]); k.m = __builtin_amdgcn_readfirstlane(d[2]);
        k.t0 = __builtin_amdgcn_readfirstlane(d[3]); k.T = __builtin_amdgcn_readfirstlane(d[4]); k.af = __builtin_amdgcn_readfirstlane(d[5]);
        k.ri = __builtin_amdgcn_readfirstlane(d[6]); k.b6 = __builtin_amdgcn_readfirstlane(d[7]); k.fpos = __builtin_amdgcn_readfirstlane(d[8]);
        k.c0p = __builtin_amdgcn_readfirstlane(d[9]);
        const long long mo = dl[0], uo = dl[1];
        k.mapoff = ((long long)__builtin_amdgcn_readfirstlane((int)(mo >> 32)) << 32) | (unsigned)__builtin_amdgcn_readfirstlane((int)mo);
        k.uoff = ((long long)__builtin_amdgcn_readfirstlane((int)(uo >> 32)) << 32) | (unsigned)__builtin_amdgcn_readfirstlane((int)uo);
        return k;
    };
    auto u_update = [&](const pg_coldesc& k, const double* sy, const int* sa) {
        const int ta = k.m - k.af;
        if (k.ri < 0 || ta <= 0) return;
        const int b6 = k.b6;
        double* __restrict__ U = ubin + k.uoff;
        double* __restrict__ g = U + (size_t)b6 * b6;
        const double* sL = s_col + k.af * 36;
        if (tid < 6 * ta) {
            const int pa = tid / 6, a = tid - pa * 6;
            const double* La = sL + pa * 36 + a * 6;
            g[sa[pa] * 6 + a] -= La[0] * sy[0] + La[1] * sy[1] + La[2] * sy[2] + La[3] * sy[3] + La[4] * sy[4] + La[5] * sy[5];
        }
        const int npair = ta * (ta + 1) / 2;
        for (int it = tid; it < 6 * npair; it += 256) {
            const int pr = it / 6, a = it - 6 * pr;
            int pa = (int)((sqrtf(8.0f * (float)pr + 1.0f) - 1.0f) * 0.5f);
            while (pa * (pa + 1) / 2 > pr) --pa;
            while ((pa + 1) * (pa + 2) / 2 <= pr) ++pa;
            const int pb = pr - pa * (pa + 1) / 2;
            const double* La = sL + pa * 36 + a * 6;
            double* Ur = U + (size_t)(sa[pa] * 6 + a) * b6 + sa[pb] * 6;
            double old[6];
#pragma unroll
            for (int b = 0; b < 6; ++b) old[b] = Ur[b];
            const double la[6] = { La[0], La[1], La[2], La[3], La[4], La[5] };
#pragma unroll
            for (int b = 0; b < 6; ++b) {
                const double* Lb = sL + pb * 36 + b * 6;
                Ur[b] = old[b] - (la[0] * Lb[0] + la[1] * Lb[1] + la[2] * Lb[2] + la[3] * Lb[3] + la[4] * Lb[4] + la[5] * Lb[5]);
            }
        }
    };
    fill(ci0, min(PG_DW, ci_end - ci0));
    __syncthreads();
    const int q = tid / 6, r = tid - q * 6;
    const bool rhs = tid >= 250;
    const int rs_ = rhs ? tid - 250 : 0;
    pg_coldesc cur = desc(ci0), prv = cur;
    double acc[6] = { 0, 0, 0, 0, 0, 0 }, accy = 0, rowv[6] = { 0, 0, 0, 0, 0, 0 }, xa = 0;
    const int* idle = bin_perm + blockIdx.x;
    int mpf = -1, arel, ip, ic;
#pragma unroll
    for (int s = 0; s < 6; ++s) rowv[s] = Lvals[(size_t)(cur.c0 + (tid < 6 * cur.m ? q : 0)) * 36 + r * 6 + s];
    xa = x[(size_t)cur.j * 6 + rs_];
    arel = *(tid < cur.m - cur.af ? anc_rel + cur.c0 + cur.af + tid : idle);
    {
        const pg_coldesc d1 = ci0 + 1 < ci_end ? desc(ci0 + 1) : cur;
        const bool st1 = ci0 + 1 < ci_end && tid < 6 * min(PG_PCH, d1.T - (d1.fpos >= 0));
        ip = *(st1 ? rlpos + d1.t0 + q : idle); ic = *(st1 ? rlcol + d1.t0 + q : idle);
    }
    for (int ci = ci0; ci < ci_end; ++ci) {
        const int par = ci & 1, rel = ci - ci0;
        const bool have1 = ci + 1 < ci_end, have2 = ci + 2 < ci_end;
        if (rel >= 32 && (rel & 31) == 0 && ci + 32 < ci_end) fill(ci + 32, min(32, ci_end - (ci + 32)));
        const pg_coldesc d1 = have1 ? desc(ci + 1) : cur;
        const int m = cur.m, c0 = cur.c0, j = cur.j;
        const bool act = tid < 6 * m;
        const int Tnf = cur.T - (cur.fpos >= 0);
        const int* mp = upd_map + cur.mapoff;
        const int Tnf1 = have1 ? d1.T - (d1.fpos >= 0) : 0, tn1 = min(PG_PCH, Tnf1);
        const bool act1 = have1 && tid < 6 * d1.m;
        const int* mp1 = upd_map + d1.mapoff;
        int mpi[PG_NIDX], mpf1, arel1, ip2, ic2;
#pragma unroll
        for (int u = 0; u < PG_NIDX; ++u) mpi[u] = *(act1 && u < tn1 ? mp1 + (size_t)u * d1.m + q : idle);
        mpf1 = *(act1 && d1.fpos >= 0 ? mp1 + (size_t)(d1.T - 1) * d1.m + q : idle);
        arel1 = *(have1 && tid < d1.m - d1.af ? anc_rel + d1.c0 + d1.af + tid : idle);
        double sv[6], syv;
        {
            const bool st1 = tid < 6 * tn1;
            const size_t ipc = st1 ? ip : 0, icc = st1 ? ic : 0;
#pragma unroll
            for (int s = 0; s < 6; ++s) sv[s] = Lvals[ipc * 36 + r * 6 + s];
            syv = x[icc * 6 + r];
        }
        {
            const pg_coldesc d2 = have2 ? desc(ci + 2) : cur;
            const bool st2 = have2 && tid < 6 * min(PG_PCH, d2.T - (d2.fpos >= 0));
            ip2 = *(st2 ? rlpos + d2.t0 + q : idle); ic2 = *(st2 ? rlcol + d2.t0 + q : idle);
        }
        for (int tc = ci == ci0 ? 0 : min(PG_PCH, Tnf); tc < Tnf; tc += PG_PCH) {
            const int tn = min(PG_PCH, Tnf - tc);
            __syncthreads();
            if (tid < 6 * tn) {
                const int pos = rlpos[cur.t0 + tc + q], col = rlcol[cur.t0 + tc + q];
#pragma unroll
                for (int s = 0; s < 6; ++s) s_st[par][tid * 6 + s] = Lvals[(size_t)pos * 36 + r * 6 + s];
                s_sy[par][tid] = x[(size_t)col * 6 + r];
            }
            __syncthreads();
            if (rhs)
                for (int t = 0; t < tn; ++t) {
                    const double* yk = s_sy[par] + t * 6; const double* B = s_st[par] + t * 36 + rs_ * 6;
                    accy += B[0] * yk[0] + B[1] * yk[1] + B[2] * yk[2] + B[3] * yk[3] + B[4] * yk[4] + B[5] * yk[5];
                }
            if (act) pg_acc_rows(mp + (size_t)tc * m + q, m, tn, Lvals, r, s_st[par], acc);
        }
        if (cur.fpos >= 0) {
            const double* Bf = s_col + cur.fpos * 36;
            if (rhs) {
                const double* yk = s_y[par ^ 1]; const double* B = Bf + rs_ * 6;
                accy += B[0] * yk[0] + B[1] * yk[1] + B[2] * yk[2] + B[3] * yk[3] + B[4] * yk[4] + B[5] * yk[5];
            }
            if (act && mpf >= 0) {
                const double* Lik = s_col + (mpf - cur.c0p) * 36 + r * 6;
                const double a[6] = { Lik[0], Lik[1], Lik[2], Lik[3], Lik[4], Lik[5] };
                pg_upd_term(acc, a, Bf);
            }
        }
        if (rhs) s_xj[rs_] = xa - accy;
        if (act) {
#pragma unroll
            for (int s = 0; s < 6; ++s) rowv[s] -= acc[s];
            if (tid < 6) { for (int s = 0; s < 6; ++s) s_diag[r * 6 + s] = rowv[s]; }
        }
        if (tid < m - cur.af) s_arel[par][tid] = arel;
        if (tid < 6 * tn1) {
#pragma unroll
            for (int s = 0; s < 6; ++s) s_st[par ^ 1][tid * 6 + s] = sv[s];
            s_sy[par ^ 1][tid] = syv;
        }
        __syncthreads();
        double acc1[6] = { 0, 0, 0, 0, 0, 0 }, accy1 = 0, rowv1[6] = { 0, 0, 0, 0, 0, 0 }, xa1 = 0;
        if (tid == 250) {
            double A[36], xj[6], ri[6];
#pragma unroll
            for (int a = 0; a < 36; ++a) A[a] = s_diag[a];
#pragma unroll
            for (int a = 0; a < 6; ++a) xj[a] = s_xj[a];
            const int bad = chol6_recip(A, ri);
            if (bad) *fail = 1;
            s_ok = !bad;
#pragma unroll
            for (int a = 0; a < 6; ++a)
#pragma unroll
                for (int b = 0; b < 6; ++b) { const double v = b <= a ? A[a * 6 + b] : 0.0; s_diag[a * 6 + b] = v; Lvals[(size_t)c0 * 36 + a * 6 + b] = v; }
#pragma unroll
            for (int a = 0; a < 6; ++a) { s_ri[a] = ri[a]; rdiag[(size_t)j * 6 + a] = ri[a]; }
            if (!bad) {
                double v[6];
#pragma unroll
                for (int a = 0; a < 6; ++a) {
                    double t = xj[a];
#pragma unroll
                    for (int b = 0; b < 6; ++b) if (b < a) t -= A[a * 6 + b] * v[b];
                    v[a] = t * ri[a];
                }
#pragma unroll
                for (int a = 0; a < 6; ++a) { x[(size_t)j * 6 + a] = v[a]; s_y[par][a] = v[a]; }
            }
        }
        if (ci > ci0) u_update(prv, s_y[par ^ 1], s_arel[par ^ 1]);
        if (tn1 > 0) {
            if (rhs)
                for (int t = 0; t < tn1; ++t) {
                    const double* yk = s_sy[par ^ 1] + t * 6; const double* B = s_st[par ^ 1] + t * 36 + rs_ * 6;
                    accy1 += B[0] * yk[0] + B[1] * yk[1] + B[2] * yk[2] + B[3] * yk[3] + B[4] * yk[4] + B[5] * yk[5];
                }
            if (act1) pg_acc_rows_ahead(mpi, mp1 + q, d1.m, tn1, Lvals, r, s_st[par ^ 1], acc1);
        }
#pragma unroll
        for (int s = 0; s < 6; ++s) rowv1[s] = Lvals[(size_t)(d1.c0 + (act1 ? q : 0)) * 36 + r * 6 + s];
        xa1 = x[(size_t)d1.j * 6 + rs_];
        __syncthreads();
        if (!s_ok) return;
        if (act && tid >= 6) {
            double* row = Lvals + (size_t)(c0 + q) * 36 + r * 6;
            double xr[6];
#pragma unroll
            for (int s = 0; s < 6; ++s) { double v = rowv[s];
#pragma unroll
                                          for (int c = 0; c < 6; ++c) if (c < s) v -= xr[c] * s_diag[s * 6 + c];
                                          xr[s] = v * s_ri[s]; }
            for (int s = 0; s < 6; ++s) { row[s] = xr[s]; s_col[tid * 6 + s] = xr[s]; }
        }
        __syncthreads();
        prv = cur; cur = d1;
#pragma unroll
        for (int s = 0; s < 6; ++s) { acc[s] = acc1[s]; rowv[s] = rowv1[s]; }
        accy = accy1; xa = xa1; mpf = mpf1; arel = arel1; ip = ip2; ic = ic2;
    }
    u_update(prv, s_y[(ci_end - 1) & 1], s_arel[(ci_end - 1) & 1]);
}
__global__ __launch_bounds__(64) void pg_bwd_subtree_kernel(const int* __restrict__ bin_perm, const int* __restrict__ binptr, const int* __restrict__ bincols,
                                                            const int* __restrict__ colptr, const int* __restrict__ rowidx,
                                                            const double* __restrict__ Lvals, double* __restrict__ x, const double* __restrict__ rdiag)
{
    const int lane = threadIdx.x;
    const int bin = bin_perm[blockIdx.x];
    const int ci_lo = binptr[bin];
    int jn = 0, cn0 = 0, cn1 = 0;
    double ldn[36], rin[6];
    auto ahead = [&](int ci2) {
        jn = bincols[ci2]; cn0 = colptr[jn]; cn1 = colptr[jn + 1];
        if (lane == 0) {
            const double* Ld = Lvals + (size_t)cn0 * 36;
#pragma unroll
            for (int a = 0; a < 36; ++a) ldn[a] = Ld[a];
#pragma unroll
            for (int a = 0; a < 6; ++a) rin[a] = rdiag[(size_t)jn * 6 + a];
        }
    };
    if (binptr[bin + 1] - 1 >= ci_lo) ahead(binptr[bin + 1] - 1);
    for (int ci = binptr[bin + 1] - 1; ci >= ci_lo; --ci) {
        const int j = jn, c0 = cn0, c1 = cn1;
        double ld[36], ri[6];
#pragma unroll
        for (int a = 0; a < 36; ++a) ld[a] = ldn[a];
#pragma unroll
        for (int a = 0; a < 6; ++a) ri[a] = rin[a];
        if (ci - 1 >= ci_lo) ahead(ci - 1);
        double acc[6] = { 0, 0, 0, 0, 0, 0 };
        for (int p = c0 + 1 + lane; p < c1; p += 64) {
            const double* B = Lvals + (size_t)p * 36; const double* xi = x + (size_t)rowidx[p] * 6;
            for (int a = 0; a < 6; ++a) { double s = 0; for (int b = 0; b < 6; ++b) s += B[b * 6 + a] * xi[b]; acc[a] += s; }
        }
#pragma unroll
        for (int a = 0; a < 6; ++a) acc[a] = dsss_wave_sum(acc[a]);
        if (lane == 0) {
            double v[6], xj[6];
#pragma unroll
            for (int a = 0; a < 6; ++a) xj[a] = x[(size_t)j * 6 + a];
#pragma unroll
            for (int a = 5; a >= 0; --a) { double s = xj[a] - acc[a];
#pragma unroll
                                           for (int b = 0; b < 6; ++b) if (b > a) s -= ld[b * 6 + a] * v[b];
                                           v[a] = s * ri[a]; }
#pragma unroll
            for (int a = 0; a < 6; ++a) x[(size_t)j * 6 + a] = v[a];
        }
        __threadfence_block();
        __builtin_amdgcn_s_barrier();
    }
}

template __global__ void pg_scan_block_kernel<int, 0>(int, const int* __restrict__, const int* __restrict__, int* __restrict__, int* __restrict__);
template __global__ void pg_scan_block_kernel<long long, 1>(int, const int* __restrict__, const int* __restrict__, long long* __restrict__, long long* __restrict__);
template __global__ void pg_scan_tops_kernel<int>(int, int* __restrict__, int* __restrict__);
template __global__ void pg_scan_tops_kernel<long long>(int, long long* __restrict__, long long* __restrict__);
template __global__ void pg_scan_add_kernel<int>(int, int* __restrict__, const int* __restrict__, const int* __restrict__);
template __global__ void pg_scan_add_kernel<long long>(int, long long* __restrict__, const long long* __restrict__, const long long* __restrict__);
```

diasss_amd/csrc/dsss_pg_chain.hip:

```cpp
#include "dsss_pg_kernels.h"
#include "dsss_pg_dev.h"
__device__ inline bool pg_owned_factor(int k, int n, const int* __restrict__ eo, int mp0, int mp1)
{
    const int p = k < n ? k : eo[k - n];
    return p >= mp0 && p < mp1;
}
template <bool WJ>
__global__ __launch_bounds__(256) void pg_linearize_kernel(int n, int ne, const pose_t* __restrict__ X, const pose_t* __restrict__ meas,
                                                           pg_weights W, const int* __restrict__ ea, const int* __restrict__ eb, const int* __restrict__ eo,
                                                           const pose_t* __restrict__ emeas, const double* __restrict__ ew,
                                                           double* __restrict__ r, double* __restrict__ Ji, double* __restrict__ partial, int mp0, int mp1)
{
    __shared__ double s_w[4];
    __shared__ double s_j[4][64 * 19];
    const int k = blockIdx.x * 256 + threadIdx.x;
    const int lane = threadIdx.x & 63, wv = threadIdx.x >> 6;
    double e2 = 0;
    const bool own = k < n + ne && pg_owned_factor(k, n, eo, mp0, mp1);
    double rr[6], J[36];
    if (own) {
        factor_eval<WJ>(k, n, X, meas, W, ea, eb, emeas, ew, rr, J);
#pragma unroll
        for (int a = 0; a < 6; ++a) { e2 += rr[a] * rr[a]; if (WJ) r[(size_t)k * 6 + a] = rr[a]; }
    }
    if (WJ) {
        const unsigned long long owned = __ballot(own);
        const size_t k0 = (size_t)(blockIdx.x * 256 + wv * 64);
        double* __restrict__ sj = s_j[wv];
#pragma unroll
        for (int h = 0; h < 2; ++h) {
            if (own) {
#pragma unroll
                for (int a = 0; a < 18; ++a) sj[lane * 19 + a] = J[18 * h + a];
            }
            __builtin_amdgcn_wave_barrier();
            asm volatile("s_waitcnt lgkmcnt(0)" ::: "memory");
#pragma unroll
            for (int i = 0; i < 18; ++i) {
                const int e = i * 64 + lane, f = e / 18, a = e - 18 * f;
                if ((owned >> f) & 1ull) Ji[(k0 + f) * 36 + 18 * h + a] = sj[f * 19 + a];
            }
            __builtin_amdgcn_wave_barrier();
            asm volatile("s_waitcnt lgkmcnt(0)" ::: "memory");
        }
    }
    const double s = block_sum256(e2, s_w);
    if (threadIdx.x == 0) partial[blockIdx.x] = s;
}

template __global__ void pg_linearize_kernel<false>(int, int, const pose_t* __restrict__, const pose_t* __restrict__, pg_weights, const int* __restrict__, const int* __restrict__, const int* __restrict__, const pose_t* __restrict__, const double* __restrict__, double* __restrict__, double* __restrict__, double* __restrict__, int, int);
template __global__ void pg_linearize_kernel<true>(int, int, const pose_t* __restrict__, const pose_t* __restrict__, pg_weights, const int* __restrict__, const int* __restrict__, const int* __restrict__, const pose_t* __restrict__, const double* __restrict__, double* __restrict__, double* __restrict__, double* __restrict__, int, int);

__global__ __launch_bounds__(256) void pg_final_sum_kernel(const double* __restrict__ partial, int n, double scale, double* __restrict__ out)
{
    __shared__ double s_w[4];
    double acc = 0;
    for (int i = threadIdx.x; i < n; i += 256) acc += partial[i];
    const double s = block_sum256(acc, s_w);
    if (threadIdx.x == 0) *out = s * scale;
}

__global__ __launch_bounds__(6 * PG_ASM_POSES) void pg_assemble_kernel(int n, pg_weights W, const double* __restrict__ r, const double* __restrict__ Ji,
                                                          const int* __restrict__ adj_ptr, const int* __restrict__ adj_edge,
                                                          const double* __restrict__ ew, const double* __restrict__ lambda_ptr,
                                                          double* __restrict__ D, double* __restrict__ C, double* __restrict__ g,
                                                          const int* __restrict__ eo, int mp0, int mp1, const int* __restrict__ plist, int np)
{
    __shared__ double s_dc[2][PG_ASM_POSES * 36];
    __shared__ double s_j[PG_ASM_POSES * 36];
    const int slot_ = blockIdx.x * PG_ASM_POSES + threadIdx.x / 6, a = threadIdx.x % 6;
    const int i = plist ? (slot_ < np ? plist[slot_] : n) : slot_;
    const bool live = i < n;
    if (!plist) {
        const size_t jb = ((size_t)blockIdx.x * PG_ASM_POSES + 1) * 36, lim = (size_t)n * 36;
#pragma unroll
        for (int u = 0; u < 3; ++u) {
            const int e = 2 * (u * (6 * PG_ASM_POSES) + (int)threadIdx.x);
            double2 v = make_double2(0.0, 0.0);
            if (jb + e + 1 < lim) v = *reinterpret_cast<const double2*>(Ji + jb + e);
            s_j[e] = v.x; s_j[e + 1] = v.y;
        }
    }
    __syncthreads();
    double Dd[6] = { 0, 0, 0, 0, 0, 0 }, Cc[6] = { 0, 0, 0, 0, 0, 0 }, gg = 0;
    if (live) {
    const bool own_i = i >= mp0 && i < mp1, own_next = i + 1 >= mp0 && i + 1 < mp1;
    const double* w2 = i == 0 ? W.prior : W.odo;
    if (own_i) {
        const double wa = w2[a];
#pragma unroll
        for (int b = 0; b < 6; ++b) if (b == a) Dd[b] += wa * wa;
        gg += wa * r[(size_t)i * 6 + a];
    }
    if (i + 1 < n && own_next) {
        const double* J = plist ? Ji + (size_t)(i + 1) * 36 : s_j + (threadIdx.x / 6) * 36; const double* rr = r + (size_t)(i + 1) * 6;
        double ja[6], sb[6] = { 0, 0, 0, 0, 0, 0 };
#pragma unroll
        for (int q = 0; q < 6; ++q) ja[q] = J[q * 6 + a];
#pragma unroll
        for (int q = 0; q < 6; ++q)
#pragma unroll
            for (int b = 0; b < 6; ++b) sb[b] += ja[q] * J[q * 6 + b];
#pragma unroll
        for (int b = 0; b < 6; ++b) { Dd[b] += sb[b]; Cc[b] = ja[b] * W.odo[b]; }
        double s = 0;
#pragma unroll
        for (int q = 0; q < 6; ++q) s += ja[q] * rr[q];
        gg += s;
    }
    for (int p = adj_ptr[i]; p < adj_ptr[i + 1]; ++p) {
        const int code = adj_edge[p], e = code >> 1, second = code & 1;
        if (eo[e] < mp0 || eo[e] >= mp1) continue;
        const double* rr = r + (size_t)(n + e) * 6;
        if (second) {
            const double wa = ew[(size_t)e * 6 + a];
#pragma unroll
            for (int b = 0; b < 6; ++b) if (b == a) Dd[b] += wa * wa;
            gg += wa * rr[a];
        } else {
            const double* J = Ji + (size_t)(n + e) * 36;
            double ja[6], sb[6] = { 0, 0, 0, 0, 0, 0 };
#pragma unroll
            for (int q = 0; q < 6; ++q) ja[q] = J[q * 6 + a];
#pragma unroll
            for (int q = 0; q < 6; ++q)
#pragma unroll
                for (int b = 0; b < 6; ++b) sb[b] += ja[q] * J[q * 6 + b];
#pragma unroll
            for (int b = 0; b < 6; ++b) Dd[b] += sb[b];
            double s = 0;
#pragma unroll
            for (int q = 0; q < 6; ++q) s += ja[q] * rr[q];
            gg += s;
        }
    }
    const double lambda = *lambda_ptr;
    if (own_i) {
#pragma unroll
        for (int b = 0; b < 6; ++b) if (b == a) Dd[b] += lambda;
    }
    g[(size_t)i * 6 + a] = gg;
    if (plist) {
#pragma unroll
        for (int b = 0; b < 6; ++b) { D[(size_t)i * 36 + a * 6 + b] = Dd[b]; C[(size_t)i * 36 + a * 6 + b] = Cc[b]; }
    }
    }
    if (plist) return;
#pragma unroll
    for (int b = 0; b < 6; ++b) { s_dc[0][threadIdx.x * 6 + b] = Dd[b]; s_dc[1][threadIdx.x * 6 + b] = Cc[b]; }
    __syncthreads();
    {
        const size_t base = (size_t)blockIdx.x * PG_ASM_POSES * 36;
        const size_t lim = (size_t)n * 36;
#pragma unroll
        for (int u = 0; u < 3; ++u) {
            const int e = 2 * (u * (6 * PG_ASM_POSES) + (int)threadIdx.x);
            if (base + e + 1 < lim) {
                *reinterpret_cast<double2*>(D + base + e) = make_double2(s_dc[0][e], s_dc[0][e + 1]);
                *reinterpret_cast<double2*>(C + base + e) = make_double2(s_dc[1][e], s_dc[1][e + 1]);
            }
        }
    }
}

struct pg_seg_lds { double E[2][36], D[2][36], G[2][6], C[36], L[36], Rv[6], Wo[6]; };
#define PG_COMPILER_FENCE() asm volatile("" ::: "memory")
#define PG_GROUP_SYNC() do { asm volatile("s_waitcnt lgkmcnt(0)" ::: "memory"); __builtin_amdgcn_wave_barrier(); } while (0)
#define PG_SEG_LANES 8
template <bool FROMJ>
__device__ __forceinline__ void pg_seg_from_j(const double* __restrict__ Jl, const double* __restrict__ Rn, double rp, const double* __restrict__ Wl, double wa, double lambda,
                                              int c, double* __restrict__ nC, double* __restrict__ pre, double& gpre)
{
    if constexpr (FROMJ) {
#pragma unroll
        for (int u = 0; u < 5; ++u) { const int a = c + PG_SEG_LANES * u; if (a < 36) { const int row = a / 6, col = a - 6 * row; nC[u] = Jl[col * 6 + row] * Wl[col]; } }
        if (c < 6) {
            double ja[6], sb[6] = { 0, 0, 0, 0, 0, 0 };
#pragma unroll
            for (int q = 0; q < 6; ++q) ja[q] = Jl[q * 6 + c];
#pragma unroll
            for (int q = 0; q < 6; ++q)
#pragma unroll
                for (int b = 0; b < 6; ++b) sb[b] += ja[q] * Jl[q * 6 + b];
#pragma unroll
            for (int b = 0; b < 6; ++b) { double d = b == c ? 0.0 + wa * wa : 0.0; d += sb[b]; if (b == c) d += lambda; pre[b] = d; }
            double gg = 0.0 + wa * rp, s2 = 0;
#pragma unroll
            for (int q = 0; q < 6; ++q) s2 += ja[q] * Rn[q];
            gpre = gg + s2;
        }
    }
}
template <bool FROMJ>
__global__ __launch_bounds__(256, 2) void pg_segment_kernel(int nseg, const int* __restrict__ seg_order, const int* __restrict__ sep_pose, const double* __restrict__ D,
                                                         const double* __restrict__ C, const double* __restrict__ g,
                                                         double* __restrict__ E, double* __restrict__ Dl, double* __restrict__ gi,
                                                         double* __restrict__ segDL, double* __restrict__ segDR, double* __restrict__ segGL,
                                                         double* __restrict__ segGR, double* __restrict__ segS, int* __restrict__ fail, int mp0, int mp1,
                                                         const double* __restrict__ rf, const double* __restrict__ Jf, pg_weights W, const double* __restrict__ lambda_ptr)
{
    __shared__ pg_seg_lds sh_all[256 / PG_SEG_LANES];
    const int grp = threadIdx.x / PG_SEG_LANES, c = threadIdx.x % PG_SEG_LANES;
    const int slot = blockIdx.x * (256 / PG_SEG_LANES) + grp;
    if (slot >= nseg) return;
    const int s = seg_order[slot];
    pg_seg_lds& sh = sh_all[grp];
    const int L = sep_pose[s], R = sep_pose[s + 1];
    if (L + 1 < mp0 || L + 1 >= mp1) return;
    if (R == L + 1) {
        for (int a = c; a < 36; a += PG_SEG_LANES) { segDL[(size_t)s * 36 + a] = 0; segDR[(size_t)s * 36 + a] = 0; segS[(size_t)s * 36 + a] = C[(size_t)L * 36 + a]; }
        if (c < 6) { segGL[(size_t)s * 6 + c] = 0; segGR[(size_t)s * 6 + c] = 0; }
        return;
    }
    double lambda = 0.0, rp = 0.0, rn = 0.0, jn[5] = { 0, 0, 0, 0, 0 }, gpre = 0.0, wa = 0.0;
    if constexpr (FROMJ) {
        lambda = *lambda_ptr;
        wa = c == 0 ? W.odo[0] : c == 1 ? W.odo[1] : c == 2 ? W.odo[2] : c == 3 ? W.odo[3] : c == 4 ? W.odo[4] : W.odo[5];
        if (c < 6) sh.Wo[c] = wa;
        for (int a = c; a < 36; a += PG_SEG_LANES) { sh.E[0][a] = C[(size_t)L * 36 + a]; sh.C[a] = Jf[(size_t)(L + 2) * 36 + a]; }
        if (c < 6) { rp = rf[(size_t)(L + 1) * 6 + c]; rn = rf[(size_t)(L + 2) * 6 + c]; sh.Rv[c] = rn; }
    } else {
        for (int a = c; a < 36; a += PG_SEG_LANES) { sh.E[0][a] = C[(size_t)L * 36 + a]; sh.D[0][a] = D[(size_t)(L + 1) * 36 + a]; }
        if (c < 6) sh.G[0][c] = g[(size_t)(L + 1) * 6 + c];
    }
    double nC[5], acc[6] = { 0, 0, 0, 0, 0, 0 }, pre[6] = { 0, 0, 0, 0, 0, 0 };
    const bool has_role = c < 7, is_col = c < 6;
    const int pre_stride = is_col ? 6 : 1;
    const double* pre_src = is_col ? D + c : g;
    const int pre_lds = is_col ? (int)(&sh.D[0][0] - &sh.E[0][0]) + c : (int)(&sh.G[0][0] - &sh.E[0][0]);
    const int pre_flip = is_col ? 36 : 6;
    int cb = 0;
    if constexpr (FROMJ) {
#pragma unroll
        for (int u = 0; u < 5; ++u) nC[u] = 0.0;
        PG_GROUP_SYNC();
        double d0[6] = { 0, 0, 0, 0, 0, 0 };
        pg_seg_from_j<true>(sh.C, sh.Rv, rp, sh.Wo, wa, lambda, c, nC, d0, gpre);
        if (c < 6) {
#pragma unroll
            for (int a = 0; a < 6; ++a) sh.D[0][a * 6 + c] = d0[a];
            sh.G[0][c] = gpre;
            rp = rn;
        }
        gpre = 0.0;
        PG_GROUP_SYNC();
    } else {
#pragma unroll
        for (int u = 0; u < 5; ++u) { const int a = c + PG_SEG_LANES * u; nC[u] = a < 36 ? C[(size_t)(L + 1) * 36 + a] : 0.0; }
    }
    for (int i = L + 1; i < R; ++i) {
        const bool last = (i + 1 == R);
        double* __restrict__ Ec = sh.E[cb]; double* __restrict__ Dc = sh.D[cb]; double* __restrict__ Gc = sh.G[cb];
        double* __restrict__ En = sh.E[cb ^ 1]; double* __restrict__ Dn = sh.D[cb ^ 1]; double* __restrict__ Gn = sh.G[cb ^ 1];
#pragma unroll
        for (int u = 0; u < 5; ++u) { const int a = c + PG_SEG_LANES * u; if (a < 36) sh.C[a] = nC[u]; }
        if constexpr (FROMJ) {
            if (is_col) {
#pragma unroll
                for (int a = 0; a < 6; ++a) Dc[a * 6 + c] += pre[a];
                Gc[c] += gpre;
            }
            if (!last) {
#pragma unroll
                for (int u = 0; u < 5; ++u) { const int a = c + PG_SEG_LANES * u; if (a < 36) jn[u] = Jf[(size_t)(i + 2) * 36 + a]; }
                if (is_col) rn = rf[(size_t)(i + 2) * 6 + c];
            }
        } else {
        if (has_role) {
            double* dst = &sh.E[0][0] + pre_lds + cb * pre_flip;
#pragma unroll
            for (int a = 0; a < 6; ++a) dst[a * pre_stride] += pre[a];
        }
        if (!last) {
#pragma unroll
            for (int u = 0; u < 5; ++u) { const int a = c + PG_SEG_LANES * u; if (a < 36) nC[u] = C[(size_t)(i + 1) * 36 + a]; }
            if (has_role) {
                const double* src = pre_src + (size_t)(i + 1) * (is_col ? 36 : 6);
#pragma unroll
                for (int a = 0; a < 6; ++a) pre[a] = src[a * pre_stride];
            }
        } else if (has_role) {
#pragma unroll
            for (int a = 0; a < 6; ++a) pre[a] = 0.0;
        }
        }
        if (i > L + 1) for (int a = c; a < 36; a += PG_SEG_LANES) Dl[(size_t)(i - 1) * 36 + a] = sh.L[a];
        PG_GROUP_SYNC();
        for (int a = c; a < 36; a += PG_SEG_LANES) E[(size_t)i * 36 + a] = Ec[a];
        if (c < 6) gi[(size_t)i * 6 + c] = Gc[c];
        double Li[36];
#pragma unroll
        for (int a = 0; a < 6; ++a)
#pragma unroll
            for (int b2 = 0; b2 < 6; ++b2) Li[a * 6 + b2] = b2 <= a ? Dc[a * 6 + b2] : 0.0;
        if (chol6_rdiag(Li)) { *fail = 1; return; }
        if (c == 0) {
#pragma unroll
            for (int a = 0; a < 36; ++a) sh.L[a] = Li[a];
        }
        PG_COMPILER_FENCE();
        double yA[6], yB[6];
        {
            const double* ya = is_col ? Ec + c * 6 : Gc;
            const double* yb = is_col ? sh.C + c : Gc;
            const int bstr = is_col ? 6 : 1;
#pragma unroll
            for (int q = 0; q < 6; ++q) { yA[q] = ya[q]; yB[q] = yb[q * bstr]; }
        }
#pragma unroll
        for (int a = 0; a < 6; ++a) {
            double t = yA[a], u = yB[a];
            for (int k = 0; k < a; ++k) { t -= Li[a * 6 + k] * yA[k]; u -= Li[a * 6 + k] * yB[k]; }
            yA[a] = t * Li[a * 7]; yB[a] = u * Li[a * 7];
        }
#pragma unroll
        for (int a = 5; a >= 0; --a) {
            double t = yA[a], u = yB[a];
            for (int k = a + 1; k < 6; ++k) { t -= Li[k * 6 + a] * yA[k]; u -= Li[k * 6 + a] * yB[k]; }
            yA[a] = t * Li[a * 7]; yB[a] = u * Li[a * 7];
        }
        PG_COMPILER_FENCE();
        {
#pragma unroll
            for (int a = 0; a < 6; ++a) {
                double t = 0, u = 0;
#pragma unroll
                for (int q = 0; q < 6; ++q) { t += Ec[a * 6 + q] * yA[q]; u += Ec[a * 6 + q] * yB[q]; }
                acc[a] -= t;
                if (is_col) En[a * 6 + c] = -u;
            }
        }
        PG_COMPILER_FENCE();
        {
            double yc[6];
#pragma unroll
            for (int q = 0; q < 6; ++q) {
                double ya1 = yA[q], yb1 = yB[q];
                if constexpr (FROMJ) asm volatile("" : "+v"(ya1), "+v"(yb1));
                yc[q] = is_col ? yb1 : ya1;
            }
#pragma unroll
            for (int a = 0; a < 6; ++a) {
                double u = 0;
#pragma unroll
                for (int q = 0; q < 6; ++q) u += sh.C[q * 6 + a] * yc[q];
                if (is_col) Dn[a * 6 + c] = -u;
                else if (c == 6) Gn[a] = -u;
            }
        }
        if constexpr (FROMJ) {
            if (!last) {
                PG_GROUP_SYNC();
#pragma unroll
                for (int u = 0; u < 5; ++u) { const int a = c + PG_SEG_LANES * u; if (a < 36) sh.C[a] = jn[u]; }
                if (is_col) sh.Rv[c] = rn;
                PG_GROUP_SYNC();
                pg_seg_from_j<true>(sh.C, sh.Rv, rp, sh.Wo, wa, lambda, c, nC, pre, gpre);
                rp = rn;
            } else {
#pragma unroll
                for (int a = 0; a < 6; ++a) pre[a] = 0.0;
                gpre = 0.0;
            }
        }
        cb ^= 1;
        PG_GROUP_SYNC();
    }
    for (int a = c; a < 36; a += PG_SEG_LANES) Dl[(size_t)(R - 1) * 36 + a] = sh.L[a];
    if (c < 6) for (int a = 0; a < 6; ++a) segDL[(size_t)s * 36 + a * 6 + c] = acc[a];
    if (c == 6) for (int a = 0; a < 6; ++a) segGL[(size_t)s * 6 + a] = acc[a];
    for (int a = c; a < 36; a += PG_SEG_LANES) { segDR[(size_t)s * 36 + a] = sh.D[cb][a]; segS[(size_t)s * 36 + a] = sh.E[cb][a]; }
    if (c < 6) segGR[(size_t)s * 6 + c] = sh.G[cb][c];
}
template __global__ void pg_segment_kernel<false>(int, const int* __restrict__, const int* __restrict__, const double* __restrict__, const double* __restrict__, const double* __restrict__, double* __restrict__, double* __restrict__, double* __restrict__, double* __restrict__, double* __restrict__, double* __restrict__, double* __restrict__, double* __restrict__, int* __restrict__, int, int, const double* __restrict__, const double* __restrict__, pg_weights, const double* __restrict__);
template __global__ void pg_segment_kernel<true>(int, const int* __restrict__, const int* __restrict__, const double* __restrict__, const double* __restrict__, const double* __restrict__, double* __restrict__, double* __restrict__, double* __restrict__, double* __restrict__, double* __restrict__, double* __restrict__, double* __restrict__, double* __restrict__, int* __restrict__, int, int, const double* __restrict__, const double* __restrict__, pg_weights, const double* __restrict__);

__global__ __launch_bounds__(256) void pg_chain1_kernel(int ns1, const int* __restrict__ sep1, const double* __restrict__ D, const double* __restrict__ g,
                                                        const double* __restrict__ segDL, const double* __restrict__ segDR,
                                                        const double* __restrict__ segGL, const double* __restrict__ segGR, const double* __restrict__ segS,
                                                        double* __restrict__ D1, double* __restrict__ C1, double* __restrict__ g1, int mp0, int mp1)
{
    const long long t = (long long)blockIdx.x * 256 + threadIdx.x;
    const int k = (int)(t / 42), a = (int)(t - 42LL * k);
    if (k >= ns1) return;
    const int p = sep1[k];
    const bool segl = k > 0 && sep1[k - 1] + 1 >= mp0 && sep1[k - 1] + 1 < mp1, segr = k + 1 < ns1 && p + 1 >= mp0 && p + 1 < mp1;
    if (a < 36) {
        double v = D[(size_t)p * 36 + a];
        if (segl) v += segDR[(size_t)(k - 1) * 36 + a];
        if (segr) v += segDL[(size_t)k * 36 + a];
        D1[(size_t)k * 36 + a] = v;
        C1[(size_t)k * 36 + a] = segr ? segS[(size_t)k * 36 + a] : 0.0;
    } else {
        const int b = a - 36;
        double v = g[(size_t)p * 6 + b];
        if (segl) v += segGR[(size_t)(k - 1) * 6 + b];
        if (segr) v += segGL[(size_t)k * 6 + b];
        g1[(size_t)k * 6 + b] = v;
    }
}

__global__ __launch_bounds__(256) void pg_scatter_base_kernel(int ns, const int* __restrict__ sep_pose, const int* __restrict__ perm,
                                                              const double* __restrict__ D, const double* __restrict__ g,
                                                              const double* __restrict__ segDL, const double* __restrict__ segDR,
                                                              const double* __restrict__ segGL, const double* __restrict__ segGR,
                                                              const double* __restrict__ segS, const int* __restrict__ dest,
                                                              double* __restrict__ Lvals, double* __restrict__ aval, double* __restrict__ rhs,
                                                              const int* __restrict__ if_slot, double* __restrict__ aval_if, double* __restrict__ x_if, int mp0, int mp1)
{
    const long long t = (long long)blockIdx.x * 256 + threadIdx.x;
    const int k = (int)(t / 78), el = (int)(t - 78LL * k);
    if (k >= ns) return;
    const int p = sep_pose[k];
    const bool segl = k > 0 && sep_pose[k - 1] + 1 >= mp0 && sep_pose[k - 1] + 1 < mp1, segr = k + 1 < ns && p + 1 >= mp0 && p + 1 < mp1;
    const int code = dest[k];
    const bool iface = code <= -2, own = p >= mp0 && p < mp1;
    if (el < 42) {
        if (!(iface || own)) return;
        if (el < 36) {
            double* dst = code >= 0 ? Lvals + (size_t)(code >> 1) * 36 : (iface ? aval_if + (size_t)(-2 - code) * 36 : aval + (size_t)k * 36);
            double v = D[(size_t)p * 36 + el];
            if (segl) v += segDR[(size_t)(k - 1) * 36 + el];
            if (segr) v += segDL[(size_t)k * 36 + el];
            dst[el] = v;
        } else {
            const int a = el - 36;
            double* rr = iface ? x_if + (size_t)if_slot[k] * 6 : rhs + (size_t)perm[k] * 6;
            double v = g[(size_t)p * 6 + a];
            if (segl) v += segGR[(size_t)(k - 1) * 6 + a];
            if (segr) v += segGL[(size_t)k * 6 + a];
            rr[a] = -v;
        }
    } else if (segr) {
        const int e = el - 42, a = e / 6, b = e - 6 * a;
        const int cc = dest[ns + k];
        const double* S = segS + (size_t)k * 36;
        if (cc >= 0) Lvals[(size_t)(cc >> 1) * 36 + e] = (cc & 1) ? S[b * 6 + a] : S[e];
        else (cc <= -2 ? aval_if + (size_t)(-2 - cc) * 36 : aval + (size_t)(ns + k) * 36)[e] = S[e];
    }
}
__global__ __launch_bounds__(256) void pg_scatter_lc_kernel(int n, int ne, int ns, const double* __restrict__ Ji, const double* __restrict__ ew,
                                                            const int* __restrict__ dest, double* __restrict__ Lvals, double* __restrict__ aval,
                                                            double* __restrict__ aval_if, const int* __restrict__ eo, int mp0, int mp1, const int* __restrict__ lc_link)
{
    const long long t = (long long)blockIdx.x * 256 + threadIdx.x;
    const int e = (int)(t / 36), el = (int)(t - 36LL * e);
    if (e >= ne) return;
    if (eo[e] < mp0 || eo[e] >= mp1) return;
    const int code = dest[2 * ns - 1 + e];
    if (code >= 0) {
        if (lc_link && !lc_link[2 * e]) return;
        double* dst = Lvals + (size_t)(code >> 1) * 36 + el;
        double v = *dst;
        for (int q = e; q >= 0; q = lc_link ? lc_link[2 * q + 1] : -1) {
            const int tr = dest[2 * ns - 1 + q] & 1;
            const int a = tr ? el % 6 : el / 6, b = tr ? el / 6 : el % 6;
            v += Ji[(size_t)(n + q) * 36 + b * 6 + a] * ew[(size_t)q * 6 + b];
        }
        *dst = v;
    } else {
        const int a = el / 6, b = el - 6 * a;
        (code <= -2 ? aval_if + (size_t)(-2 - code) * 36 : aval + (size_t)(2 * ns - 1 + e) * 36)[el] = Ji[(size_t)(n + e) * 36 + b * 6 + a] * ew[(size_t)e * 6 + b];
    }
}

__global__ __launch_bounds__(256) void pg_comm_pack_kernel(const int* __restrict__ it_child, const int* __restrict__ it_row, const pg_pack* __restrict__ PK)
{
    const pg_pack pk = PK[it_child[blockIdx.x]];
    const int i = it_row[blockIdx.x], b6 = 6 * pk.cb, wcols = 6 * (i + 1);
    for (int cc = threadIdx.x; cc < wcols; cc += 256) {
#pragma unroll
        for (int a = 0; a < 6; ++a) pk.dst[(size_t)(6 * i + a) * b6 + cc] = pk.U[(size_t)(6 * i + a) * pk.cld + cc];
    }
    if (threadIdx.x < 6) pk.dst[(size_t)b6 * b6 + 6 * i + threadIdx.x] = pk.g[6 * i + threadIdx.x];
}
__global__ __launch_bounds__(256) void pg_comm_xif_kernel(int nif, const int* __restrict__ if_sep, const int* __restrict__ perm, const double* __restrict__ x_if, double* __restrict__ x)
{
    const int q = blockIdx.x * 256 + threadIdx.x;
    if (q >= nif) return;
    for (int a = 0; a < 6; ++a) x[(size_t)perm[if_sep[q]] * 6 + a] = x_if[(size_t)q * 6 + a];
}
__global__ void pg_comm_scal_kernel(const double* __restrict__ scal, const int* __restrict__ fail, double* __restrict__ red)
{
    if (threadIdx.x < 3) red[threadIdx.x] = scal[threadIdx.x];
    if (threadIdx.x == 3) red[3] = (double)*fail;
}

__global__ __launch_bounds__(256) void pg_sep_delta_kernel(int ns, const int* __restrict__ sep_pose, const int* __restrict__ perm,
                                                           const double* __restrict__ x, double* __restrict__ delta)
{
    const int k = blockIdx.x * 256 + threadIdx.x;
    if (k >= ns) return;
    const int src = perm ? perm[k] : k;
    if (src < 0) return;
    for (int a = 0; a < 6; ++a) delta[(size_t)sep_pose[k] * 6 + a] = x[(size_t)src * 6 + a];
}

#define PG_BS_LANES 8
struct pg_bs_blk { double Ec[6], Cr[6], gv, Lm[21]; };
template <bool FROMJ>
__device__ __forceinline__ void pg_bs_load(pg_bs_blk& B, int i, int aa, const double* __restrict__ C, const double* __restrict__ E,
                                           const double* __restrict__ Dl, const double* __restrict__ gi, const double* __restrict__ Jf, const pg_weights& W)
{
#pragma unroll
    for (int q = 0; q < 6; ++q) {
        B.Ec[q] = E[(size_t)i * 36 + q * 6 + aa];
        if constexpr (FROMJ) B.Cr[q] = Jf[(size_t)(i + 1) * 36 + q * 6 + aa] * W.odo[q];
        else B.Cr[q] = C[(size_t)i * 36 + aa * 6 + q];
    }
    B.gv = gi[(size_t)i * 6 + aa];
#pragma unroll
    for (int r = 0; r < 6; ++r)
#pragma unroll
        for (int k = 0; k <= r; ++k) B.Lm[r * (r + 1) / 2 + k] = Dl[(size_t)i * 36 + r * 6 + k];
}
template <bool FROMJ>
__global__ __launch_bounds__(256) void pg_backsub_kernel(int nseg, const int* __restrict__ seg_order, const int* __restrict__ sep_pose, const double* __restrict__ C,
                                                         const double* __restrict__ E, const double* __restrict__ Dl, const double* __restrict__ gi,
                                                         double* __restrict__ delta, int mp0, int mp1, const double* __restrict__ Jf, pg_weights W)
{
    const int slot = blockIdx.x * (256 / PG_BS_LANES) + threadIdx.x / PG_BS_LANES, a = threadIdx.x % PG_BS_LANES;
    if (slot >= nseg) return;
    const int s = seg_order[slot];
    const int L = sep_pose[s], R = sep_pose[s + 1];
    if (L + 1 < mp0 || L + 1 >= mp1 || R == L + 1) return;
    const int aa = a < 6 ? a : 5;
    double dL[6], dn[6];
#pragma unroll
    for (int q = 0; q < 6; ++q) { dL[q] = delta[(size_t)L * 6 + q]; dn[q] = delta[(size_t)R * 6 + q]; }
    pg_bs_blk cur, nxt;
    pg_bs_load<FROMJ>(cur, R - 1, aa, C, E, Dl, gi, Jf, W);
    for (int i = R - 1; i > L; --i) {
        if (i - 1 > L) pg_bs_load<FROMJ>(nxt, i - 1, aa, C, E, Dl, gi, Jf, W);
        double t = -cur.gv;
#pragma unroll
        for (int q = 0; q < 6; ++q) { t -= cur.Ec[q] * dL[q]; t -= cur.Cr[q] * dn[q]; }
        double b[6];
#pragma unroll
        for (int q = 0; q < 6; ++q) b[q] = __shfl(t, q, PG_BS_LANES);
#pragma unroll
        for (int r = 0; r < 6; ++r) { double v = b[r]; for (int k = 0; k < r; ++k) v -= cur.Lm[r * (r + 1) / 2 + k] * b[k]; b[r] = v * cur.Lm[r * (r + 1) / 2 + r]; }
#pragma unroll
        for (int r = 5; r >= 0; --r) { double v = b[r]; for (int k = r + 1; k < 6; ++k) v -= cur.Lm[k * (k + 1) / 2 + r] * b[k]; b[r] = v * cur.Lm[r * (r + 1) / 2 + r]; }
        const double mine = a == 0 ? b[0] : a == 1 ? b[1] : a == 2 ? b[2] : a == 3 ? b[3] : a == 4 ? b[4] : b[5];
        if (a < 6) delta[(size_t)i * 6 + a] = mine;
#pragma unroll
        for (int q = 0; q < 6; ++q) dn[q] = b[q];
        cur = nxt;
    }
}
template __global__ void pg_backsub_kernel<false>(int, const int* __restrict__, const int* __restrict__, const double* __restrict__, const double* __restrict__, const double* __restrict__, const double* __restrict__, double* __restrict__, int, int, const double* __restrict__, pg_weights);
template __global__ void pg_backsub_kernel<true>(int, const int* __restrict__, const int* __restrict__, const double* __restrict__, const double* __restrict__, const double* __restrict__, const double* __restrict__, double* __restrict__, int, int, const double* __restrict__, pg_weights);

__global__ __launch_bounds__(256) void pg_linerr_kernel(int n, int ne, pg_weights W, const int* __restrict__ ea, const int* __restrict__ eb, const int* __restrict__ eo,
                                                        const double* __restrict__ ew, const double* __restrict__ r, const double* __restrict__ Ji,
                                                        const double* __restrict__ delta, double* __restrict__ partial, int mp0, int mp1)
{
    __shared__ double s_w[4];
    double e2 = 0;
#pragma unroll
    for (int it = 0; it < 6; ++it) {
        const int el = it * 256 + threadIdx.x, k = blockIdx.x * 256 + el / 6, a = el % 6;
        if (k < n + ne && pg_owned_factor(k, n, eo, mp0, mp1)) {
            int i = -1, j; double wa;
            if (k == 0) { j = 0; wa = W.prior[a]; }
            else if (k < n) { i = k - 1; j = k; wa = W.odo[a]; }
            else { i = ea[k - n]; j = eb[k - n]; wa = ew[(size_t)(k - n) * 6 + a]; }
            double s = r[(size_t)k * 6 + a] + wa * delta[(size_t)j * 6 + a];
            if (i >= 0) for (int q = 0; q < 6; ++q) s += Ji[(size_t)k * 36 + a * 6 + q] * delta[(size_t)i * 6 + q];
            e2 += s * s;
        }
    }
    const double s = block_sum256(e2, s_w);
    if (threadIdx.x == 0) partial[blockIdx.x] = s;
}

__global__ __launch_bounds__(256) void pg_retract_kernel(int n, const pose_t* __restrict__ X, const double* __restrict__ delta, pose_t* __restrict__ Xn)
{
    const int i = blockIdx.x * 256 + threadIdx.x;
    if (i >= n) return;
    pose_t o;
    pose_retract(&X[i], delta + (size_t)i * 6, &o);
    Xn[i] = o;
}

__device__ inline unsigned long long minstd_pow(unsigned long long e)
{
    unsigned long long r = 1, b = 16807ULL;
    const unsigned long long m = 2147483647ULL;
    while (e) { if (e & 1) r = (r * b) % m; b = (b * b) % m; e >>= 1; }
    return r;
}
__global__ __launch_bounds__(256) void pg_rng_attempts_kernel(long long nattempts, double* __restrict__ pairs, int* __restrict__ flags)
{
    const long long a0 = ((long long)blockIdx.x * 256 + threadIdx.x) * RNG_PER_THREAD;
    if (a0 >= nattempts) return;
    const unsigned long long m = 2147483647ULL;
    unsigned long long x = minstd_pow((unsigned long long)(4 * a0));
    const double R = 2147483646.0;
    for (int k = 0; k < RNG_PER_THREAD && a0 + k < nattempts; ++k) {
        double cn[2];
        for (int q = 0; q < 2; ++q) {
            x = (x * 16807ULL) % m; const double e1 = (double)(x - 1);
            x = (x * 16807ULL) % m; const double e2 = (double)(x - 1);
            double can = (e1 + e2 * R) / (R * R);
            if (can >= 1.0) can = 0.99999999999999988897769753748;
            cn[q] = can;
        }
        const double u = 2.0 * cn[0] - 1.0, v = 2.0 * cn[1] - 1.0, r2 = u * u + v * v;
        const bool ok = !(r2 > 1.0 || r2 == 0.0);
        double mult = 0;
        if (ok) mult = sqrt(-2 * log(r2) / r2);
        pairs[2 * (a0 + k)] = v * mult; pairs[2 * (a0 + k) + 1] = u * mult;
        flags[a0 + k] = ok ? 1 : 0;
    }
}
__global__ __launch_bounds__(256) void pg_flag_blocksum_kernel(const int* __restrict__ flags, long long n, int* __restrict__ bsum)
{
    __shared__ int s_w[4];
    const long long i0 = (long long)blockIdx.x * 4096;
    int acc = 0;
    for (int k = threadIdx.x; k < 4096; k += 256) if (i0 + k < n) acc += flags[i0 + k];
    acc = dsss_wave_sum(acc);
    if ((threadIdx.x & 63) == 0) s_w[threadIdx.x >> 6] = acc;
    __syncthreads();
    if (threadIdx.x == 0) bsum[blockIdx.x] = s_w[0] + s_w[1] + s_w[2] + s_w[3];
}
__global__ __launch_bounds__(256) void pg_flag_scan_kernel(int* __restrict__ bsum, int nb, int* __restrict__ total)
{
    if (threadIdx.x == 0) { int run = 0; for (int i = 0; i < nb; ++i) { const int v = bsum[i]; bsum[i] = run; run += v; } *total = run; }
}
template <typename STORE>
__device__ inline void pg_compact_block(const int* __restrict__ flags, long long n, const int* __restrict__ bsum, STORE store)
{
    __shared__ int s_w[4];
    const long long i0 = (long long)blockIdx.x * 4096;
    int run = bsum[blockIdx.x];
    for (int c = 0; c < 4096; c += 256) {
        const long long i = i0 + c + threadIdx.x;
        const int f = (i < n) ? flags[i] : 0;
        int tot;
        const int pos = run + dsss_block_scan_excl<4, int>(f, &tot, s_w);
        if (f) store(i, pos);
        run += tot;
    }
}
__global__ __launch_bounds__(256) void pg_flag_compact_kernel(const int* __restrict__ flags, const double* __restrict__ pairs, long long n,
                                                              const int* __restrict__ bsum, long long need_pairs, double* __restrict__ normals)
{
    pg_compact_block(flags, n, bsum, [&](long long i, int pos) {
        if (pos < need_pairs) { normals[2 * (size_t)pos] = pairs[2 * i]; normals[2 * (size_t)pos + 1] = pairs[2 * i + 1]; }
    });
}
__global__ __launch_bounds__(256) void lc_edge_compact_kernel(const int* __restrict__ flags, const int* __restrict__ bsum, const unsigned long long* __restrict__ slot,
                                                              int total, const int* __restrict__ kp7_off, const double* __restrict__ kp7,
                                                              const dsss_lc* __restrict__ lcs, const int* __restrict__ act_s, const int* __restrict__ frame_off,
                                                              int cap, dsss_lc_edge* __restrict__ edges, int2* __restrict__ ab)
{
    pg_compact_block(flags, total, bsum, [&](long long g, int pos) {
        if (pos >= cap) return;
        const unsigned long long key = slot[g];
        const int p = (int)(key >> 32) - 1, k = (int)(0xffffffffu - (unsigned)(key & 0xffffffffu));
        const int i = kp7_off[p] + k;
        dsss_lc_edge ed;
        ed.a = frame_off[act_s[p]] + (int)kp7[(size_t)i * 7 + 0];
        ed.b = (int)g;
        for (int q = 0; q < 12; ++q) ed.rel[q] = lcs[i].rel[q];
        for (int q = 0; q < 6; ++q) ed.var[q] = lcs[i].var[q];
        edges[pos] = ed;
        if (ab) ab[pos] = make_int2(ed.a, ed.b);
    });
}
__global__ __launch_bounds__(256) void pg_gather_dr_kernel(const unsigned long long* __restrict__ fptr, const int* __restrict__ foff, double* __restrict__ out)
{
    const int f = blockIdx.y;
    const double* __restrict__ src = reinterpret_cast<const double*>(fptr[f]);
    const size_t n6 = (size_t)(foff[f + 1] - foff[f]) * 6;
    double* __restrict__ dst = out + (size_t)foff[f] * 6;
    for (size_t i = (size_t)blockIdx.x * 256 + threadIdx.x; i < n6; i += (size_t)gridDim.x * 256) dst[i] = src[i];
}
__global__ __launch_bounds__(256) void pg_gather_pose_kernel(int n, const int* __restrict__ idx, const pose_t* __restrict__ X, pose_t* __restrict__ out)
{
    const int i = blockIdx.x * 256 + threadIdx.x;
    if (i < n) out[i] = X[idx[i]];
}
__global__ __launch_bounds__(256) void pg_sep_xy_kernel(int ns, const int* __restrict__ sep_pose, const double* __restrict__ dr6, double* __restrict__ xy)
{
    const int k = blockIdx.x * 256 + threadIdx.x;
    if (k >= ns) return;
    xy[2 * k] = dr6[(size_t)sep_pose[k] * 6 + 3]; xy[2 * k + 1] = dr6[(size_t)sep_pose[k] * 6 + 4];
}
__global__ __launch_bounds__(256) void pg_init_kernel(int n, const double* __restrict__ dr6, const double* __restrict__ normals, int add_noise,
                                                      pose_t* __restrict__ X, pose_t* __restrict__ meas)
{
    const int i = blockIdx.x * 256 + threadIdx.x;
    if (i >= n) return;
    const double PI = DSSS_PI_REF;
    pose_t cur, prev, m;
    pose_from_rodrigues(dr6 + (size_t)i * 6, &cur);
    if (i == 0) m = cur;
    else { pose_from_rodrigues(dr6 + (size_t)(i - 1) * 6, &prev); pose_between(&prev, &cur, &m); }
    meas[i] = m;
    if (add_noise) {
        const double* z = normals + (size_t)i * 6;
        const double noise_xyz = 0.5, noise_rpy = 0.5 * PI / 180;
        const double w[3] = { z[0] * noise_rpy, z[1] * noise_rpy, z[2] * noise_rpy };
        pose_t N, o;
        so3_exp(w, N.R);
        N.t[0] = z[3] * noise_xyz; N.t[1] = z[4] * noise_xyz; N.t[2] = z[5] * noise_xyz;
        pose_compose(&cur, &N, &o);
        X[i] = o;
    } else X[i] = cur;
}

__global__ __launch_bounds__(256) void pg_rpy_kernel(int n, const pose_t* __restrict__ X, double* __restrict__ rpy6)
{
    const int i = blockIdx.x * 256 + threadIdx.x;
    if (i >= n) return;
    const pose_t T = X[i];
    double rpy[3];
    pose_rpy(&T, rpy);
    double* o = rpy6 + (size_t)i * 6;
    o[0] = rpy[0]; o[1] = rpy[1]; o[2] = rpy[2]; o[3] = T.t[0]; o[4] = T.t[1]; o[5] = T.t[2];
}
```

diasss_amd/csrc/dsss_pg_kernels.h:

```cpp
#pragma once
#include "dsss_internal.h"
#include "dsss_pose.h"
#include "dsss_pg_sym.h"

struct pg_weights { double prior[6], odo[6]; };

struct pg_pack { const double* U; const double* g; double* dst; int cld, cb; };
struct pg_front {
    long long off, roff;
    int ld, n6, s6, c0;
    int rowptr, pan0;
    int ch0, ch1, fa0, fa1;
};
struct pg_child { const double* U; const double* g; long long relptr; int cld, cb; };

#define PG_ASM_POSES 32
#define PG_NB4 24
#define PG_RSU_MAX_TILES 320
#define PG_RSU32_MAX_TILES 80
#define PG_BWD2_LD 97
#define PG_BWD2_SX 8192
#define PG_BWD_SPLIT 2048
#define PG_BWD_RC 512
#define RNG_PER_THREAD 16

template <bool WJ> __global__ void pg_linearize_kernel(int n, int ne, const pose_t* __restrict__ X, const pose_t* __restrict__ meas, pg_weights W, const int* __restrict__ ea, const int* __restrict__ eb, const int* __restrict__ eo, const pose_t* __restrict__ emeas, const double* __restrict__ ew, double* __restrict__ r, double* __restrict__ Ji, double* __restrict__ partial, int mp0, int mp1);
__global__ void pg_final_sum_kernel(const double* __restrict__ partial, int n, double scale, double* __restrict__ out);
__global__ void pg_assemble_kernel(int n, pg_weights W, const double* __restrict__ r, const double* __restrict__ Ji, const int* __restrict__ adj_ptr, const int* __restrict__ adj_edge, const double* __restrict__ ew, const double* __restrict__ lambda_ptr, double* __restrict__ D, double* __restrict__ C, double* __restrict__ g, const int* __restrict__ eo, int mp0, int mp1, const int* __restrict__ plist, int np);
template <bool FROMJ> __global__ void pg_segment_kernel(int nseg, const int* __restrict__ seg_order, const int* __restrict__ sep_pose, const double* __restrict__ D, const double* __restrict__ C, const double* __restrict__ g, double* __restrict__ E, double* __restrict__ Dl, double* __restrict__ gi, double* __restrict__ segDL, double* __restrict__ segDR, double* __restrict__ segGL, double* __restrict__ segGR, double* __restrict__ segS, int* __restrict__ fail, int mp0, int mp1, const double* __restrict__ rf, const double* __restrict__ Jf, pg_weights W, const double* __restrict__ lambda_ptr);
__global__ void pg_chain1_kernel(int ns1, const int* __restrict__ sep1, const double* __restrict__ D, const double* __restrict__ g, const double* __restrict__ segDL, const double* __restrict__ segDR, const double* __restrict__ segGL, const double* __restrict__ segGR, const double* __restrict__ segS, double* __restrict__ D1, double* __restrict__ C1, double* __restrict__ g1, int mp0, int mp1);
__global__ void pg_scatter_base_kernel(int ns, const int* __restrict__ sep_pose, const int* __restrict__ perm, const double* __restrict__ D, const double* __restrict__ g, const double* __restrict__ segDL, const double* __restrict__ segDR, const double* __restrict__ segGL, const double* __restrict__ segGR, const double* __restrict__ segS, const int* __restrict__ dest, double* __restrict__ Lvals, double* __restrict__ aval, double* __restrict__ rhs, const int* __restrict__ if_slot, double* __restrict__ aval_if, double* __restrict__ x_if, int mp0, int mp1);
__global__ void pg_scatter_lc_kernel(int n, int ne, int ns, const double* __restrict__ Ji, const double* __restrict__ ew, const int* __restrict__ dest, double* __restrict__ Lvals, double* __restrict__ aval, double* __restrict__ aval_if, const int* __restrict__ eo, int mp0, int mp1, const int* __restrict__ lc_link);
__global__ void pg_comm_pack_kernel(const int* __restrict__ it_child, const int* __restrict__ it_row, const pg_pack* __restrict__ PK);
__global__ void pg_comm_xif_kernel(int nif, const int* __restrict__ if_sep, const int* __restrict__ perm, const double* __restrict__ x_if, double* __restrict__ x);
__global__ void pg_comm_scal_kernel(const double* __restrict__ scal, const int* __restrict__ fail, double* __restrict__ red);
__global__ void pg_sep_delta_kernel(int ns, const int* __restrict__ sep_pose, const int* __restrict__ perm, const double* __restrict__ x, double* __restrict__ delta);
template <bool FROMJ> __global__ void pg_backsub_kernel(int nseg, const int* __restrict__ seg_order, const int* __restrict__ sep_pose, const double* __restrict__ C, const double* __restrict__ E, const double* __restrict__ Dl, const double* __restrict__ gi, double* __restrict__ delta, int mp0, int mp1, const double* __restrict__ Jf, pg_weights W);
__global__ void pg_linerr_kernel(int n, int ne, pg_weights W, const int* __restrict__ ea, const int* __restrict__ eb, const int* __restrict__ eo, const double* __restrict__ ew, const double* __restrict__ r, const double* __restrict__ Ji, const double* __restrict__ delta, double* __restrict__ partial, int mp0, int mp1);
__global__ void pg_retract_kernel(int n, const pose_t* __restrict__ X, const double* __restrict__ delta, pose_t* __restrict__ Xn);
__global__ void pg_rng_attempts_kernel(long long nattempts, double* __restrict__ pairs, int* __restrict__ flags);
__global__ void pg_flag_blocksum_kernel(const int* __restrict__ flags, long long n, int* __restrict__ bsum);
__global__ void pg_flag_scan_kernel(int* __restrict__ bsum, int nb, int* __restrict__ total);
__global__ void pg_flag_compact_kernel(const int* __restrict__ flags, const double* __restrict__ pairs, long long n, const int* __restrict__ bsum, long long need_pairs, double* __restrict__ normals);
__global__ void lc_edge_compact_kernel(const int* __restrict__ flags, const int* __restrict__ bsum, const unsigned long long* __restrict__ slot, int total, const int* __restrict__ kp7_off, const double* __restrict__ kp7,
                                       const dsss_lc* __restrict__ lcs, const int* __restrict__ act_s, const int* __restrict__ frame_off, int cap, dsss_lc_edge* __restrict__ edges, int2* __restrict__ ab);
__global__ void pg_gather_dr_kernel(const unsigned long long* __restrict__ fptr, const int* __restrict__ foff, double* __restrict__ out);
__global__ void pg_gather_pose_kernel(int n, const int* __restrict__ idx, const pose_t* __restrict__ X, pose_t* __restrict__ out);
__global__ void pg_sep_xy_kernel(int ns, const int* __restrict__ sep_pose, const double* __restrict__ dr6, double* __restrict__ xy);
__global__ void pg_init_kernel(int n, const double* __restrict__ dr6, const double* __restrict__ normals, int add_noise, pose_t* __restrict__ X, pose_t* __restrict__ meas);
__global__ void pg_rpy_kernel(int n, const pose_t* __restrict__ X, double* __restrict__ rpy6);
__global__ void pg_build_map_kernel(int nupd, const int* __restrict__ rlrow, const int* __restrict__ rlptr, const int* __restrict__ rlcol, const int* __restrict__ rlpos, const int* __restrict__ colptr, const int* __restrict__ rowidx, const long long* __restrict__ mapptr, int* __restrict__ upd_map, const int* __restrict__ nupd_dev);
__global__ void pg_rl_count_kernel(int ns, const int* __restrict__ colptr, const int* __restrict__ rowidx, const char* __restrict__ binned, int* __restrict__ cnt);
template <typename T, int VAL>
__global__ void pg_scan_block_kernel(int n, const int* __restrict__ cnt, const int* __restrict__ colptr, T* __restrict__ out, T* __restrict__ block_sum);
template <typename T>
__global__ void pg_scan_tops_kernel(int nblocks, T* __restrict__ block_sum, T* __restrict__ total);
template <typename T>
__global__ void pg_scan_add_kernel(int n, T* __restrict__ out, const T* __restrict__ block_sum, const T* __restrict__ total);
__global__ void pg_rl_fill_kernel(int ns, const int* __restrict__ colptr, const int* __restrict__ rowidx, const char* __restrict__ binned, const int* __restrict__ rlptr, int* __restrict__ cur, int* __restrict__ rlcol, int* __restrict__ rlpos);
__global__ void pg_rl_sort_kernel(int ns, const int* __restrict__ rlptr, int* __restrict__ rlcol, int* __restrict__ rlpos, int* __restrict__ rlrow, int* __restrict__ fail);
__global__ void pg_fill_map_kernel(int* __restrict__ upd_map, const long long* __restrict__ total);
__global__ void pg_anc_rel_kernel(int ns, const int* __restrict__ colptr, const int* __restrict__ rowidx, const char* __restrict__ binned, const int* __restrict__ root_of, int* __restrict__ anc_first, int* __restrict__ anc_rel);
__global__ void pg_factor_subtree_kernel(const int* __restrict__ bin_perm, const int* __restrict__ binptr, const int* __restrict__ bincols, const int* __restrict__ colptr, const int* __restrict__ rlptr, const int* __restrict__ rlcol, const int* __restrict__ rlpos, const long long* __restrict__ mapptr, const int* __restrict__ upd_map, double* __restrict__ Lvals, double* __restrict__ x, int* __restrict__ fail, const int* __restrict__ binroot_ptr, const int* __restrict__ binroot_idx, const int* __restrict__ broot_b, const long long* __restrict__ broot_uoff, const int* __restrict__ broot_of_col, const int* __restrict__ anc_first, const int* __restrict__ anc_rel, double* __restrict__ ubin, double* __restrict__ rdiag);
__global__ void pg_factor_subtree_serial_kernel(const int* __restrict__ bin_perm, const int* __restrict__ binptr, const int* __restrict__ bincols, const int* __restrict__ colptr, const int* __restrict__ rlptr, const int* __restrict__ rlcol, const int* __restrict__ rlpos, const long long* __restrict__ mapptr, const int* __restrict__ upd_map, double* __restrict__ Lvals, double* __restrict__ x, int* __restrict__ fail, const int* __restrict__ binroot_ptr, const int* __restrict__ binroot_idx, const int* __restrict__ broot_b, const long long* __restrict__ broot_uoff, const int* __restrict__ broot_of_col, const int* __restrict__ anc_first, const int* __restrict__ anc_rel, double* __restrict__ ubin, double* __restrict__ rdiag);
__global__ void pg_bwd_subtree_kernel(const int* __restrict__ bin_perm, const int* __restrict__ binptr, const int* __restrict__ bincols, const int* __restrict__ colptr, const int* __restrict__ rowidx, const double* __restrict__ Lvals, double* __restrict__ x, const double* __restrict__ rdiag);
__global__ void pg_front_asm_kernel(const int* __restrict__ it_front, const int* __restrict__ it_row, const pg_front* __restrict__ FD, const pg_child* __restrict__ CH, const int* __restrict__ rel, const int* __restrict__ xr_ptr, const int* __restrict__ xr_child, const int* __restrict__ xr_row, const int* __restrict__ fa_rowptr, const int* __restrict__ fa_src, const int* __restrict__ fa_col, const int* __restrict__ fa_tr, const double* __restrict__ aval, const double* __restrict__ x, double* __restrict__ F, double* __restrict__ R);
__global__ void pg_front_syrk_kernel(const int* __restrict__ it_front, const int* __restrict__ it_step, const pg_front* __restrict__ FD, const int* __restrict__ tile_item, const int* __restrict__ tile_ij, double* __restrict__ F);
__global__ void pg_front_diag4_kernel(const int* __restrict__ it_front, const int* __restrict__ it_step, const pg_front* __restrict__ FD, double* __restrict__ F, double* __restrict__ R, int* __restrict__ fail, double* __restrict__ Tinv);
__global__ void pg_front_trsm2_kernel(const int* __restrict__ it_front, const int* __restrict__ it_step, const pg_front* __restrict__ FD, double* __restrict__ F, double* __restrict__ R, const double* __restrict__ Tinv);
template <int TS>
__global__ void pg_front_rsu_kernel(const int* __restrict__ it_front, const int* __restrict__ it_step, const pg_front* __restrict__ FD, const int* __restrict__ tile_item, const int* __restrict__ tile_ij, double* __restrict__ F, double* __restrict__ FL, double* __restrict__ R, const double* __restrict__ Tinv);
__global__ void pg_front_bwd_part_kernel(const int* __restrict__ it_front, const int* __restrict__ it_step, const pg_front* __restrict__ FD, const int* __restrict__ f_rows, const double* __restrict__ FL, const double* __restrict__ x, double* __restrict__ part, int maxchunks);
__global__ void pg_front_bwd2_kernel(const int* __restrict__ it_front, const int* __restrict__ it_step, const pg_front* __restrict__ FD, const int* __restrict__ f_rows, const double* __restrict__ F, const double* __restrict__ FL, const double* __restrict__ R, double* __restrict__ x, const double* __restrict__ Tinv, const double* __restrict__ part, int maxchunks);
```

Measured before the change: 9700 frames/s.

## Pipeline subtree backward solve with LDS-cached x and pass lambda by value

Adds a new backward subtree solve kernel that keeps solved bin columns in LDS, looks up a column's position through a precomputed colpos table, and double-buffers the fetch of the next column's L block while the current one is solved. A wave reduction built on DPP replaces the earlier serial path, which stays as a fallback when the bin exceeds the LDS budget. Lambda is now passed to the kernels as a value instead of being copied host-to-device. The fail flag and scalars are folded into one readback through an extended final-sum kernel. The new path costs an extra colpos buffer and a setup kernel, and it relies on intricate wave-level synchronisation.

```diff
diff --git a/diasss_amd/csrc/dsss_pg.hip b/diasss_amd/csrc/dsss_pg.hip
--- a/diasss_amd/csrc/dsss_pg.hip
+++ b/diasss_amd/csrc/dsss_pg.hip
@@ -103,7 +103,7 @@
     double *d_D1, *d_C1, *d_g1, *d_E1, *d_Dl1, *d_gi1, *d_delta1, *d_s2DL, *d_s2DR, *d_s2GL, *d_s2GR, *d_s2S;
     double *d_part, *d_scal, *d_red; int* d_fail;
     int *d_perm, *d_binperm = nullptr, *d_colptr, *d_rowidx, *d_rlptr, *d_rlcol, *d_rlpos, *d_rlrow, *d_binptr, *d_bincols, *d_dest, *d_map; long long* d_mapptr;
-    int *d_binroot_ptr, *d_binroot_idx, *d_broot_b, *d_broot_of_col, *d_anc_first, *d_anc_rel, *d_rel, *d_fa_src, *d_fa_col, *d_fa_tr, *d_frows, *d_xr_ptr;
+    int *d_binroot_ptr, *d_binroot_idx, *d_broot_b, *d_broot_of_col, *d_anc_first, *d_anc_rel, *d_colpos = nullptr, *d_rel, *d_fa_src, *d_fa_col, *d_fa_tr, *d_frows, *d_xr_ptr;
     int *d_xr_child, *d_xr_row, *d_fa_rowptr, *d_pk_child, *d_pk_row, *d_ifslot = nullptr, *d_ifsep = nullptr;
     long long* d_broot_uoff; pg_front* d_FD; pg_child* d_CH; pg_pack* d_PK;
     double *d_rdiag, *d_x, *d_L, *d_ubin, *d_aval, *d_F, *d_R, *d_FL, *d_Tinv, *d_bwp = nullptr;
@@ -111,7 +111,7 @@
     struct dsched { int *lv_front, *lv_step, *asm_front, *asm_row, *tile_item, *tile_ij; } DO = {}, DI = {};
     std::vector<int> ifslot;
     size_t nnzL = 0, ncv = 0, nif = 0, comm_total = 8, if_ld = 0, if_count = 0;
-    int nval = 0, bin_lo = 0, bin_hi = 0, nbins = 0, n_pack = 0, f_if = -1, bwd_lds = 0;
+    int nval = 0, bin_lo = 0, bin_hi = 0, nbins = 0, n_pack = 0, f_if = -1, bwd_lds = 0, bin_cap = 0;
     double lambda = 0, err = 0, err0 = 0;
     int iters = 0, nfact = 0;
     bool will_iterate = false, pre_lin = false, pre_chain = false, pre_bins = false;
@@ -122,7 +122,14 @@
     ~pg_solve() {
         give_coords();
         if (sym_thread.joinable()) sym_thread.join();
+        const auto Td = std::chrono::steady_clock::now();
         dv.release();
+        if (sw.opt.verbose) {
+            const double t_arena = ms_since(Td);
+            const auto Ta = std::chrono::steady_clock::now();
+            { pg_analysis dead; std::swap(dead, A); }
+            fprintf(stderr, "[dsss pg] teardown: arena %.3f ms, analysis tables %.3f ms\n", t_arena, ms_since(Ta));
+        }
     }
     void give_coords() { if (!coords_given) { coords_given = true; coords_prom.set_value(); } }
 
@@ -357,6 +364,9 @@
         return dv.rc;
     }
 
+    void sum_judged(double* out) {
+        hipLaunchKernelGGL(pg_final_sum_kernel, dim3(1), dim3(256), 0, st, d_part, nblk, 0.5, out, world > 1 ? (const double*)nullptr : (const double*)d_scal, d_fail, world > 1 ? (double*)nullptr : d_scal + 4);
+    }
     int reduce_scalars(double* host3, int* failed) {
         if (world > 1) {
             hipLaunchKernelGGL(pg_comm_scal_kernel, dim3(1), dim3(64), 0, st, d_scal, d_fail, d_red);
@@ -368,11 +378,10 @@
         } else {
             if (const int r = c->pg_scal_host.reserve(c, 8 * sizeof(double))) return r;
             double* const scal_host = c->pg_scal_host.as<double>();
-            HIPCHK(c, hipMemcpyAsync(scal_host, d_scal, 3 * sizeof(double), hipMemcpyDeviceToHost, st));
-            HIPCHK(c, hipMemcpyAsync(scal_host + 4, d_fail, sizeof(int), hipMemcpyDeviceToHost, st));
+            HIPCHK(c, hipMemcpyAsync(scal_host, d_scal + 4, 4 * sizeof(double), hipMemcpyDeviceToHost, st));
             HIPCHK(c, hipStreamSynchronize(st));
             host3[0] = scal_host[0]; host3[1] = scal_host[1]; host3[2] = scal_host[2];
-            *failed = *reinterpret_cast<const int*>(scal_host + 4);
+            *failed = scal_host[3] != 0.0;
         }
         return DSSS_OK;
     }
@@ -407,27 +416,25 @@
             if (win.p0 > 0) HIPCHK(c, hipMemcpyAsync(d_meas, warm, sizeof(pose_t), hipMemcpyDeviceToDevice, st));
         }
         hipLaunchKernelGGL(pg_linearize_kernel<false>, dim3(nblk), dim3(256), 0, st, n, ne, d_X, d_meas, W, d_ea, d_eb, d_eo, d_emeas, d_ew, (double*)nullptr, (double*)nullptr, d_part, mp0, mp1);
-        hipLaunchKernelGGL(pg_final_sum_kernel, dim3(1), dim3(256), 0, st, d_part, nblk, 0.5, d_scal);
+        HIPCHK(c, hipMemsetAsync(d_fail, 0, sizeof(int), st));
+        sum_judged(d_scal);
         double h3[3]; int failed = 0;
-        HIPCHK(c, hipMemsetAsync(d_fail, 0, sizeof(int), st));
         if (const int rc = reduce_scalars(h3, &failed)) return rc;
         lambda = c->pg.lambda0; err = err0 = h3[0];
         return DSSS_OK;
     }
 
     void chain_part() {
-        hipMemsetAsync(d_fail, 0, sizeof(int), st);
-        hipLaunchKernelGGL(pg_assemble_kernel, dim3((ns1 + PG_ASM_POSES - 1) / PG_ASM_POSES), dim3(6 * PG_ASM_POSES), 0, st, n, W, d_r, d_Ji, d_adj_ptr, d_adj_edge, d_ew, d_scal + 3, d_D, d_C, d_g, d_eo, mp0, mp1, d_sep1, ns1);
-        hipLaunchKernelGGL(pg_segment_kernel<true>, dim3((nseg1 + 31) / 32), dim3(256), 0, st, nseg1, d_ord1, d_sep1, d_D, d_C, d_g, d_E, d_Dl, d_gi, d_sDL, d_sDR, d_sGL, d_sGR, d_sS, d_fail, mp0, mp1, d_r, d_Ji, W, d_scal + 3);
+        hipLaunchKernelGGL(pg_assemble_kernel, dim3((ns1 + PG_ASM_POSES - 1) / PG_ASM_POSES), dim3(6 * PG_ASM_POSES), 0, st, n, W, d_r, d_Ji, d_adj_ptr, d_adj_edge, d_ew, lambda, d_D, d_C, d_g, d_eo, mp0, mp1, d_sep1, ns1);
+        hipLaunchKernelGGL(pg_segment_kernel<true>, dim3((nseg1 + 31) / 32), dim3(256), 0, st, nseg1, d_ord1, d_sep1, d_D, d_C, d_g, d_E, d_Dl, d_gi, d_sDL, d_sDR, d_sGL, d_sGR, d_sS, d_fail, mp0, mp1, d_r, d_Ji, W, lambda);
         hipLaunchKernelGGL(pg_chain1_kernel, dim3((unsigned)(((long long)ns1 * 42 + 255) / 256)), dim3(256), 0, st, ns1, d_sep1, d_D, d_g, d_sDL, d_sDR, d_sGL, d_sGR, d_sS, d_D1, d_C1, d_g1, mp0, mp1);
-        if (nseg > 0) hipLaunchKernelGGL(pg_segment_kernel<false>, dim3((nseg + 31) / 32), dim3(256), 0, st, nseg, d_ord2, d_t2, d_D1, d_C1, d_g1, d_E1, d_Dl1, d_gi1, d_s2DL, d_s2DR, d_s2GL, d_s2GR, d_s2S, d_fail, kp0, kp1, (const double*)nullptr, (const double*)nullptr, W, (const double*)nullptr);
+        if (nseg > 0) hipLaunchKernelGGL(pg_segment_kernel<false>, dim3((nseg + 31) / 32), dim3(256), 0, st, nseg, d_ord2, d_t2, d_D1, d_C1, d_g1, d_E1, d_Dl1, d_gi1, d_s2DL, d_s2DR, d_s2GL, d_s2GR, d_s2S, d_fail, kp0, kp1, (const double*)nullptr, (const double*)nullptr, W, 0.0);
     }
     int early_trial() {
         will_iterate = err > 0 && c->pg.max_iters > 0;
         if (!will_iterate) return DSSS_OK;
         hipLaunchKernelGGL(pg_linearize_kernel<true>, dim3(nblk), dim3(256), 0, st, n, ne, d_X, d_meas, W, d_ea, d_eb, d_eo, d_emeas, d_ew, d_r, d_Ji, d_part, mp0, mp1);
         hipLaunchKernelGGL(pg_final_sum_kernel, dim3(1), dim3(256), 0, st, d_part, nblk, 0.5, d_scal);
-        HIPCHK(c, hipMemcpyAsync(d_scal + 3, &lambda, sizeof(double), hipMemcpyHostToDevice, st));
         chain_part();
         pre_lin = pre_chain = true;
         if (nparts > 1) return DSSS_OK;
@@ -491,8 +498,15 @@
         { const int nb_all = (int)S.binptr.size() - 1, sel_lo = A.local ? 0 : part_lo, sel_hi = A.local ? 1 : part_hi;
           bin_lo = 0; while (bin_lo < nb_all && S.bin_part[bin_lo] < sel_lo) ++bin_lo; bin_hi = bin_lo; while (bin_hi < nb_all && S.bin_part[bin_hi] < sel_hi) ++bin_hi; }
         nbins = bin_hi - bin_lo;
-        return DSSS_OK;
-    }
+        bin_cap = 0;
+        for (int b = bin_lo; b < bin_hi; ++b) bin_cap = std::max(bin_cap, S.binptr[b + 1] - S.binptr[b]);
+        if (nbins > 0 && !bwd_serial()) {
+            if (dv.alloc(c, &d_colpos, (size_t)S.ns)) return dv.rc;
+            hipLaunchKernelGGL(pg_bin_pos_kernel, dim3(nbins), dim3(256), 0, st, d_binptr + bin_lo, d_bincols, d_colpos);
+        }
+        return DSSS_OK;
+    }
+    bool bwd_serial() const { return sw.bins_serial || (size_t)bin_cap * PG_BWD_COL_LDS > 48 * 1024; }
     void bottom_trial(double bins_flops) {
         hipMemsetAsync(d_L, 0, nnzL * 36 * sizeof(double), st);
         if (nparts > 1) hipMemsetAsync(d_comm, 0, comm_total * sizeof(double), st);
@@ -620,10 +634,7 @@
         }
     }
     int trial() {
-        if (!pre_chain) {
-            HIPCHK(c, hipMemcpyAsync(d_scal + 3, &lambda, sizeof(double), hipMemcpyHostToDevice, st));
-            chain_part();
-        }
+        if (!pre_chain) chain_part();
         pre_chain = false;
         if (!pre_bins) bottom_trial(std::max(0.0, S.flops_factor - S.flops_fronts));
         pre_bins = false;
@@ -648,7 +659,8 @@
         }
         run_levels_bwd(A.SO, DO);
         if (nbins > 0) { dsss_scope s7(c, DSSS_K_PG_SUBTREE);
-            hipLaunchKernelGGL(pg_bwd_subtree_kernel, dim3(nbins), dim3(64), 0, st, d_binperm + bin_lo, d_binptr, d_bincols, d_colptr, d_rowidx, d_L, d_x, d_rdiag); }
+            if (bwd_serial()) hipLaunchKernelGGL(pg_bwd_subtree_serial_kernel, dim3(nbins), dim3(64), 0, st, d_binperm + bin_lo, d_binptr, d_bincols, d_colptr, d_rowidx, d_L, d_x, d_rdiag);
+            else hipLaunchKernelGGL(pg_bwd_subtree_kernel, dim3(nbins), dim3(64), (size_t)bin_cap * PG_BWD_COL_LDS, st, d_binperm + bin_lo, d_binptr, d_bincols, d_colptr, d_rowidx, d_anc_first, d_colpos, d_L, d_x, d_rdiag, bin_cap); }
         hipLaunchKernelGGL(pg_sep_delta_kernel, dim3((ns + 255) / 256), dim3(256), 0, st, ns, d_t2, d_perm, d_x, d_delta1);
         if (nseg > 0)
             hipLaunchKernelGGL(pg_backsub_kernel<false>, dim3((nseg + 31) / 32), dim3(256), 0, st, nseg, d_ord2, d_t2, d_C1, d_E1, d_Dl1, d_gi1, d_delta1, kp0, kp1, (const double*)nullptr, W);
@@ -675,7 +687,7 @@
                 ++nfact;
                 hipLaunchKernelGGL(pg_retract_kernel, dim3((n + 255) / 256), dim3(256), 0, st, n, d_X, d_delta, d_Xn);
                 hipLaunchKernelGGL(pg_linearize_kernel<true>, dim3(nblk), dim3(256), 0, st, n, ne, d_Xn, d_meas, W, d_ea, d_eb, d_eo, d_emeas, d_ew, d_r2, d_Ji2, d_part, mp0, mp1);
-                hipLaunchKernelGGL(pg_final_sum_kernel, dim3(1), dim3(256), 0, st, d_part, nblk, 0.5, d_scal + 2);
+                sum_judged(d_scal + 2);
                 HIPCHK(c, hipGetLastError());
                 double h[3]; int failed = 0;
                 if (const int rc = reduce_scalars(h, &failed)) return rc;
diff --git a/diasss_amd/csrc/dsss_pg_bins.hip b/diasss_amd/csrc/dsss_pg_bins.hip
--- a/diasss_amd/csrc/dsss_pg_bins.hip
+++ b/diasss_amd/csrc/dsss_pg_bins.hip
@@ -582,7 +582,12 @@
     }
     u_update(prv, s_y[(ci_end - 1) & 1], s_arel[(ci_end - 1) & 1]);
 }
-__global__ __launch_bounds__(64) void pg_bwd_subtree_kernel(const int* __restrict__ bin_perm, const int* __restrict__ binptr, const int* __restrict__ bincols,
+__global__ __launch_bounds__(256) void pg_bin_pos_kernel(const int* __restrict__ binptr, const int* __restrict__ bincols, int* __restrict__ colpos)
+{
+    const int lo = binptr[blockIdx.x], hi = binptr[blockIdx.x + 1];
+    for (int ci = lo + threadIdx.x; ci < hi; ci += 256) colpos[bincols[ci]] = ci - lo;
+}
+__global__ __launch_bounds__(64) void pg_bwd_subtree_serial_kernel(const int* __restrict__ bin_perm, const int* __restrict__ binptr, const int* __restrict__ bincols,
                                                             const int* __restrict__ colptr, const int* __restrict__ rowidx,
                                                             const double* __restrict__ Lvals, double* __restrict__ x, const double* __restrict__ rdiag)
 {
@@ -633,6 +638,127 @@
         __builtin_amdgcn_s_barrier();
     }
 }
+struct pg_bw_col { double B[36], xr[6], pl, pr, px; int pos; };
+__device__ __forceinline__ void pg_ld6(double (&o)[6], const double* __restrict__ p)
+{
+    const double2* p2 = reinterpret_cast<const double2*>(p);
+#pragma unroll
+    for (int u = 0; u < 3; ++u) { const double2 v = p2[u]; o[2 * u] = v.x; o[2 * u + 1] = v.y; }
+}
+__device__ __forceinline__ void pg_ld36(double (&o)[36], const double* __restrict__ p)
+{
+    const double2* p2 = reinterpret_cast<const double2*>(p);
+#pragma unroll
+    for (int u = 0; u < 18; ++u) { const double2 v = p2[u]; o[2 * u] = v.x; o[2 * u + 1] = v.y; }
+}
+template <int CTRL>
+__device__ __forceinline__ double pg_dpp(double v)
+{
+    const int lo = __builtin_amdgcn_update_dpp(0, __double2loint(v), CTRL, 0xf, 0xf, false), hi = __builtin_amdgcn_update_dpp(0, __double2hiint(v), CTRL, 0xf, 0xf, false);
+    return __hiloint2double(hi, lo);
+}
+__device__ __forceinline__ double pg_lane0_sum(double v)
+{
+    v += __shfl_xor(v, 32, 64);
+    v += __shfl_xor(v, 16, 64);
+    v += pg_dpp<0x108>(v);
+    v += pg_dpp<0x104>(v);
+    v += pg_dpp<0x102>(v);
+    v += pg_dpp<0x101>(v);
+    return v;
+}
+__global__ __launch_bounds__(64) void pg_bwd_subtree_kernel(const int* __restrict__ bin_perm, const int* __restrict__ binptr, const int* __restrict__ bincols,
+                                                            const int* __restrict__ colptr, const int* __restrict__ rowidx, const int* __restrict__ anc_first,
+                                                            const int* __restrict__ colpos, const double* __restrict__ Lvals, double* __restrict__ x,
+                                                            const double* __restrict__ rdiag, int ncap)
+{
+    extern __shared__ __align__(16) double s_bw[];
+    __shared__ double s_pl[64], s_pr[64], s_px[64];
+    double* s_x = s_bw;
+    int4* s_d = reinterpret_cast<int4*>(s_bw + (size_t)ncap * 6);
+    const int lane = threadIdx.x;
+    const int bin = bin_perm[blockIdx.x];
+    const int ci_lo = binptr[bin], nc = binptr[bin + 1] - ci_lo;
+    if (nc <= 0 || nc > ncap) return;
+    for (int t = lane; t < nc; t += 64) {
+        const int j = bincols[ci_lo + t], c0 = colptr[j];
+        s_d[t] = make_int4(j, c0, colptr[j + 1] - c0, anc_first[j]);
+    }
+    __builtin_amdgcn_wave_barrier();
+    asm volatile("s_waitcnt lgkmcnt(0)" ::: "memory");
+    auto desc = [&](int t) {
+        const int4 d = s_d[t];
+        return make_int4(__builtin_amdgcn_readfirstlane(d.x), __builtin_amdgcn_readfirstlane(d.y), __builtin_amdgcn_readfirstlane(d.z), __builtin_amdgcn_readfirstlane(d.w));
+    };
+    auto rows = [&](const int4& d) { return rowidx[d.y + (lane < d.z - 1 ? lane + 1 : 0)]; };
+    auto fetch = [&](pg_bw_col& o, const int4& d, int row) __attribute__((always_inline)) {
+        const bool act = lane < d.z - 1;
+        pg_ld36(o.B, Lvals + (size_t)(d.y + (act ? lane + 1 : 0)) * 36);
+        pg_ld6(o.xr, x + (size_t)row * 6);
+        o.pos = colpos[row];
+        o.pl = Lvals[(size_t)d.y * 36 + min(lane, 35)];
+        o.pr = rdiag[(size_t)d.x * 6 + min(max(lane - 36, 0), 5)];
+        o.px = x[(size_t)d.x * 6 + min(max(lane - 42, 0), 5)];
+    };
+    auto solve = [&](const pg_bw_col& k, const int4& d, int t) __attribute__((always_inline)) {
+        const bool act = lane < d.z - 1, inb = act && lane + 1 < d.w;
+        s_pl[lane] = k.pl; s_pr[lane] = k.pr; s_px[lane] = k.px;
+        __builtin_amdgcn_wave_barrier();
+        const double* xs = s_x + (inb ? k.pos : 0) * 6;
+        double xl[6], xi[6];
+        pg_ld6(xl, xs);
+        asm volatile("" : "+v"(xl[0]), "+v"(xl[1]), "+v"(xl[2]), "+v"(xl[3]), "+v"(xl[4]), "+v"(xl[5]));
+#pragma unroll
+        for (int b = 0; b < 6; ++b) xi[b] = inb ? xl[b] : k.xr[b];
+        double acc[6];
+#pragma unroll
+        for (int a = 0; a < 6; ++a) {
+            double s = 0, z = 0;
+#pragma unroll
+            for (int b = 0; b < 6; ++b) s += k.B[b * 6 + a] * xi[b];
+            z += s;
+            acc[a] = act ? z : 0.0;
+        }
+#pragma unroll
+        for (int a = 0; a < 6; ++a) acc[a] = pg_lane0_sum(acc[a]);
+        if (lane == 0) {
+            const double* ld = s_pl; const double* ri = s_pr + 36; const double* xj = s_px + 42;
+            double v[6];
+#pragma unroll
+            for (int a = 5; a >= 0; --a) { double s = xj[a] - acc[a];
+#pragma unroll
+                                           for (int b = 0; b < 6; ++b) if (b > a) s -= ld[b * 6 + a] * v[b];
+                                           v[a] = s * ri[a]; }
+#pragma unroll
+            for (int a = 0; a < 6; ++a) { s_x[t * 6 + a] = v[a]; x[(size_t)d.x * 6 + a] = v[a]; }
+        }
+        __builtin_amdgcn_wave_barrier();
+        asm volatile("s_waitcnt lgkmcnt(0)" ::: "memory");
+    };
+    int t = nc - 1;
+    int4 d0 = desc(t), d1 = desc(max(t - 1, 0));
+    int r1 = rows(d1);
+    pg_bw_col ca, cb;
+    fetch(ca, d0, rows(d0));
+    for (;;) {
+        {
+            const int4 d2 = desc(max(t - 2, 0));
+            const int r2 = rows(d2);
+            fetch(cb, d1, r1);
+            solve(ca, d0, t);
+            d0 = d1; d1 = d2; r1 = r2;
+        }
+        if (--t < 0) break;
+        {
+            const int4 d2 = desc(max(t - 2, 0));
+            const int r2 = rows(d2);
+            fetch(ca, d1, r1);
+            solve(cb, d0, t);
+            d0 = d1; d1 = d2; r1 = r2;
+        }
+        if (--t < 0) break;
+    }
+}
 
 template __global__ void pg_scan_block_kernel<int, 0>(int, const int* __restrict__, const int* __restrict__, int* __restrict__, int* __restrict__);
 template __global__ void pg_scan_block_kernel<long long, 1>(int, const int* __restrict__, const int* __restrict__, long long* __restrict__, long long* __restrict__);
diff --git a/diasss_amd/csrc/dsss_pg_chain.hip b/diasss_amd/csrc/dsss_pg_chain.hip
--- a/diasss_amd/csrc/dsss_pg_chain.hip
+++ b/diasss_amd/csrc/dsss_pg_chain.hip
@@ -51,18 +51,27 @@
 template __global__ void pg_linearize_kernel<false>(int, int, const pose_t* __restrict__, const pose_t* __restrict__, pg_weights, const int* __restrict__, const int* __restrict__, const int* __restrict__, const pose_t* __restrict__, const double* __restrict__, double* __restrict__, double* __restrict__, double* __restrict__, int, int);
 template __global__ void pg_linearize_kernel<true>(int, int, const pose_t* __restrict__, const pose_t* __restrict__, pg_weights, const int* __restrict__, const int* __restrict__, const int* __restrict__, const pose_t* __restrict__, const double* __restrict__, double* __restrict__, double* __restrict__, double* __restrict__, int, int);
 
-__global__ __launch_bounds__(256) void pg_final_sum_kernel(const double* __restrict__ partial, int n, double scale, double* __restrict__ out)
+__global__ __launch_bounds__(256) void pg_final_sum_kernel(const double* __restrict__ partial, int n, double scale, double* out,
+                                                           const double* scal, int* __restrict__ fail, double* __restrict__ rec)
 {
     __shared__ double s_w[4];
     double acc = 0;
     for (int i = threadIdx.x; i < n; i += 256) acc += partial[i];
     const double s = block_sum256(acc, s_w);
-    if (threadIdx.x == 0) *out = s * scale;
+    if (threadIdx.x == 0) {
+        const double v = s * scale;
+        *out = v;
+        if (rec) {
+            for (int q = 0; q < 3; ++q) rec[q] = scal + q == out ? v : scal[q];
+            rec[3] = (double)*fail;
+            *fail = 0;
+        }
+    }
 }
 
 __global__ __launch_bounds__(6 * PG_ASM_POSES) void pg_assemble_kernel(int n, pg_weights W, const double* __restrict__ r, const double* __restrict__ Ji,
                                                           const int* __restrict__ adj_ptr, const int* __restrict__ adj_edge,
-                                                          const double* __restrict__ ew, const double* __restrict__ lambda_ptr,
+                                                          const double* __restrict__ ew, double lambda,
                                                           double* __restrict__ D, double* __restrict__ C, double* __restrict__ g,
                                                           const int* __restrict__ eo, int mp0, int mp1, const int* __restrict__ plist, int np)
 {
@@ -134,7 +143,6 @@
             gg += s;
         }
     }
-    const double lambda = *lambda_ptr;
     if (own_i) {
 #pragma unroll
         for (int b = 0; b < 6; ++b) if (b == a) Dd[b] += lambda;
@@ -197,7 +205,7 @@
                                                          double* __restrict__ E, double* __restrict__ Dl, double* __restrict__ gi,
                                                          double* __restrict__ segDL, double* __restrict__ segDR, double* __restrict__ segGL,
                                                          double* __restrict__ segGR, double* __restrict__ segS, int* __restrict__ fail, int mp0, int mp1,
-                                                         const double* __restrict__ rf, const double* __restrict__ Jf, pg_weights W, const double* __restrict__ lambda_ptr)
+                                                         const double* __restrict__ rf, const double* __restrict__ Jf, pg_weights W, double lambda_in)
 {
     __shared__ pg_seg_lds sh_all[256 / PG_SEG_LANES];
     const int grp = threadIdx.x / PG_SEG_LANES, c = threadIdx.x % PG_SEG_LANES;
@@ -214,7 +222,7 @@
     }
     double lambda = 0.0, rp = 0.0, rn = 0.0, jn[5] = { 0, 0, 0, 0, 0 }, gpre = 0.0, wa = 0.0;
     if constexpr (FROMJ) {
-        lambda = *lambda_ptr;
+        lambda = lambda_in;
         wa = c == 0 ? W.odo[0] : c == 1 ? W.odo[1] : c == 2 ? W.odo[2] : c == 3 ? W.odo[3] : c == 4 ? W.odo[4] : W.odo[5];
         if (c < 6) sh.Wo[c] = wa;
         for (int a = c; a < 36; a += PG_SEG_LANES) { sh.E[0][a] = C[(size_t)L * 36 + a]; sh.C[a] = Jf[(size_t)(L + 2) * 36 + a]; }
@@ -372,8 +380,8 @@
     for (int a = c; a < 36; a += PG_SEG_LANES) { segDR[(size_t)s * 36 + a] = sh.D[cb][a]; segS[(size_t)s * 36 + a] = sh.E[cb][a]; }
     if (c < 6) segGR[(size_t)s * 6 + c] = sh.G[cb][c];
 }
-template __global__ void pg_segment_kernel<false>(int, const int* __restrict__, const int* __restrict__, const double* __restrict__, const double* __restrict__, const double* __restrict__, double* __restrict__, double* __restrict__, double* __restrict__, double* __restrict__, double* __restrict__, double* __restrict__, double* __restrict__, double* __restrict__, int* __restrict__, int, int, const double* __restrict__, const double* __restrict__, pg_weights, const double* __restrict__);
-template __global__ void pg_segment_kernel<true>(int, const int* __restrict__, const int* __restrict__, const double* __restrict__, const double* __restrict__, const double* __restrict__, double* __restrict__, double* __restrict__, double* __restrict__, double* __restrict__, double* __restrict__, double* __restrict__, double* __restrict__, double* __restrict__, int* __restrict__, int, int, const double* __restrict__, const double* __restrict__, pg_weights, const double* __restrict__);
+template __global__ void pg_segment_kernel<false>(int, const int* __restrict__, const int* __restrict__, const double* __restrict__, const double* __restrict__, const double* __restrict__, double* __restrict__, double* __restrict__, double* __restrict__, double* __restrict__, double* __restrict__, double* __restrict__, double* __restrict__, double* __restrict__, int* __restrict__, int, int, const double* __restrict__, const double* __restrict__, pg_weights, double);
+template __global__ void pg_segment_kernel<true>(int, const int* __restrict__, const int* __restrict__, const double* __restrict__, const double* __restrict__, const double* __restrict__, double* __restrict__, double* __restrict__, double* __restrict__, double* __restrict__, double* __restrict__, double* __restrict__, double* __restrict__, double* __restrict__, int* __restrict__, int, int, const double* __restrict__, const double* __restrict__, pg_weights, double);
 
 __global__ __launch_bounds__(256) void pg_chain1_kernel(int ns1, const int* __restrict__ sep1, const double* __restrict__ D, const double* __restrict__ g,
                                                         const double* __restrict__ segDL, const double* __restrict__ segDR,
@@ -480,10 +488,10 @@
     if (q >= nif) return;
     for (int a = 0; a < 6; ++a) x[(size_t)perm[if_sep[q]] * 6 + a] = x_if[(size_t)q * 6 + a];
 }
-__global__ void pg_comm_scal_kernel(const double* __restrict__ scal, const int* __restrict__ fail, double* __restrict__ red)
+__global__ void pg_comm_scal_kernel(const double* __restrict__ scal, int* __restrict__ fail, double* __restrict__ red)
 {
     if (threadIdx.x < 3) red[threadIdx.x] = scal[threadIdx.x];
-    if (threadIdx.x == 3) red[3] = (double)*fail;
+    if (threadIdx.x == 3) { red[3] = (double)*fail; *fail = 0; }
 }
 
 __global__ __launch_bounds__(256) void pg_sep_delta_kernel(int ns, const int* __restrict__ sep_pose, const int* __restrict__ perm,
diff --git a/diasss_amd/csrc/dsss_pg_kernels.h b/diasss_amd/csrc/dsss_pg_kernels.h
--- a/diasss_amd/csrc/dsss_pg_kernels.h
+++ b/diasss_amd/csrc/dsss_pg_kernels.h
@@ -22,18 +22,19 @@
 #define PG_BWD2_SX 8192
 #define PG_BWD_SPLIT 2048
 #define PG_BWD_RC 512
+#define PG_BWD_COL_LDS 64
 #define RNG_PER_THREAD 16
 
 template <bool WJ> __global__ void pg_linearize_kernel(int n, int ne, const pose_t* __restrict__ X, const pose_t* __restrict__ meas, pg_weights W, const int* __restrict__ ea, const int* __restrict__ eb, const int* __restrict__ eo, const pose_t* __restrict__ emeas, const double* __restrict__ ew, double* __restrict__ r, double* __restrict__ Ji, double* __restrict__ partial, int mp0, int mp1);
-__global__ void pg_final_sum_kernel(const double* __restrict__ partial, int n, double scale, double* __restrict__ out);
-__global__ void pg_assemble_kernel(int n, pg_weights W, const double* __restrict__ r, const double* __restrict__ Ji, const int* __restrict__ adj_ptr, const int* __restrict__ adj_edge, const double* __restrict__ ew, const double* __restrict__ lambda_ptr, double* __restrict__ D, double* __restrict__ C, double* __restrict__ g, const int* __restrict__ eo, int mp0, int mp1, const int* __restrict__ plist, int np);
-template <bool FROMJ> __global__ void pg_segment_kernel(int nseg, const int* __restrict__ seg_order, const int* __restrict__ sep_pose, const double* __restrict__ D, const double* __restrict__ C, const double* __restrict__ g, double* __restrict__ E, double* __restrict__ Dl, double* __restrict__ gi, double* __restrict__ segDL, double* __restrict__ segDR, double* __restrict__ segGL, double* __restrict__ segGR, double* __restrict__ segS, int* __restrict__ fail, int mp0, int mp1, const double* __restrict__ rf, const double* __restrict__ Jf, pg_weights W, const double* __restrict__ lambda_ptr);
+__global__ void pg_final_sum_kernel(const double* __restrict__ partial, int n, double scale, double* out, const double* scal = nullptr, int* __restrict__ fail = nullptr, double* __restrict__ rec = nullptr);
+__global__ void pg_assemble_kernel(int n, pg_weights W, const double* __restrict__ r, const double* __restrict__ Ji, const int* __restrict__ adj_ptr, const int* __restrict__ adj_edge, const double* __restrict__ ew, double lambda, double* __restrict__ D, double* __restrict__ C, double* __restrict__ g, const int* __restrict__ eo, int mp0, int mp1, const int* __restrict__ plist, int np);
+template <bool FROMJ> __global__ void pg_segment_kernel(int nseg, const int* __restrict__ seg_order, const int* __restrict__ sep_pose, const double* __restrict__ D, const double* __restrict__ C, const double* __restrict__ g, double* __restrict__ E, double* __restrict__ Dl, double* __restrict__ gi, double* __restrict__ segDL, double* __restrict__ segDR, double* __restrict__ segGL, double* __restrict__ segGR, double* __restrict__ segS, int* __restrict__ fail, int mp0, int mp1, const double* __restrict__ rf, const double* __restrict__ Jf, pg_weights W, double lambda);
 __global__ void pg_chain1_kernel(int ns1, const int* __restrict__ sep1, const double* __restrict__ D, const double* __restrict__ g, const double* __restrict__ segDL, const double* __restrict__ segDR, const double* __restrict__ segGL, const double* __restrict__ segGR, const double* __restrict__ segS, double* __restrict__ D1, double* __restrict__ C1, double* __restrict__ g1, int mp0, int mp1);
 __global__ void pg_scatter_base_kernel(int ns, const int* __restrict__ sep_pose, const int* __restrict__ perm, const double* __restrict__ D, const double* __restrict__ g, const double* __restrict__ segDL, const double* __restrict__ segDR, const double* __restrict__ segGL, const double* __restrict__ segGR, const double* __restrict__ segS, const int* __restrict__ dest, double* __restrict__ Lvals, double* __restrict__ aval, double* __restrict__ rhs, const int* __restrict__ if_slot, double* __restrict__ aval_if, double* __restrict__ x_if, int mp0, int mp1);
 __global__ void pg_scatter_lc_kernel(int n, int ne, int ns, const double* __restrict__ Ji, const double* __restrict__ ew, const int* __restrict__ dest, double* __restrict__ Lvals, double* __restrict__ aval, double* __restrict__ aval_if, const int* __restrict__ eo, int mp0, int mp1, const int* __restrict__ lc_link);
 __global__ void pg_comm_pack_kernel(const int* __restrict__ it_child, const int* __restrict__ it_row, const pg_pack* __restrict__ PK);
 __global__ void pg_comm_xif_kernel(int nif, const int* __restrict__ if_sep, const int* __restrict__ perm, const double* __restrict__ x_if, double* __restrict__ x);
-__global__ void pg_comm_scal_kernel(const double* __restrict__ scal, const int* __restrict__ fail, double* __restrict__ red);
+__global__ void pg_comm_scal_kernel(const double* __restrict__ scal, int* __restrict__ fail, double* __restrict__ red);
 __global__ void pg_sep_delta_kernel(int ns, const int* __restrict__ sep_pose, const int* __restrict__ perm, const double* __restrict__ x, double* __restrict__ delta);
 template <bool FROMJ> __global__ void pg_backsub_kernel(int nseg, const int* __restrict__ seg_order, const int* __restrict__ sep_pose, const double* __restrict__ C, const double* __restrict__ E, const double* __restrict__ Dl, const double* __restrict__ gi, double* __restrict__ delta, int mp0, int mp1, const double* __restrict__ Jf, pg_weights W);
 __global__ void pg_linerr_kernel(int n, int ne, pg_weights W, const int* __restrict__ ea, const int* __restrict__ eb, const int* __restrict__ eo, const double* __restrict__ ew, const double* __restrict__ r, const double* __restrict__ Ji, const double* __restrict__ delta, double* __restrict__ partial, int mp0, int mp1);
@@ -63,7 +64,9 @@
 __global__ void pg_anc_rel_kernel(int ns, const int* __restrict__ colptr, const int* __restrict__ rowidx, const char* __restrict__ binned, const int* __restrict__ root_of, int* __restrict__ anc_first, int* __restrict__ anc_rel);
 __global__ void pg_factor_subtree_kernel(const int* __restrict__ bin_perm, const int* __restrict__ binptr, const int* __restrict__ bincols, const int* __restrict__ colptr, const int* __restrict__ rlptr, const int* __restrict__ rlcol, const int* __restrict__ rlpos, const long long* __restrict__ mapptr, const int* __restrict__ upd_map, double* __restrict__ Lvals, double* __restrict__ x, int* __restrict__ fail, const int* __restrict__ binroot_ptr, const int* __restrict__ binroot_idx, const int* __restrict__ broot_b, const long long* __restrict__ broot_uoff, const int* __restrict__ broot_of_col, const int* __restrict__ anc_first, const int* __restrict__ anc_rel, double* __restrict__ ubin, double* __restrict__ rdiag);
 __global__ void pg_factor_subtree_serial_kernel(const int* __restrict__ bin_perm, const int* __restrict__ binptr, const int* __restrict__ bincols, const int* __restrict__ colptr, const int* __restrict__ rlptr, const int* __restrict__ rlcol, const int* __restrict__ rlpos, const long long* __restrict__ mapptr, const int* __restrict__ upd_map, double* __restrict__ Lvals, double* __restrict__ x, int* __restrict__ fail, const int* __restrict__ binroot_ptr, const int* __restrict__ binroot_idx, const int* __restrict__ broot_b, const long long* __restrict__ broot_uoff, const int* __restrict__ broot_of_col, const int* __restrict__ anc_first, const int* __restrict__ anc_rel, double* __restrict__ ubin, double* __restrict__ rdiag);
-__global__ void pg_bwd_subtree_kernel(const int* __restrict__ bin_perm, const int* __restrict__ binptr, const int* __restrict__ bincols, const int* __restrict__ colptr, const int* __restrict__ rowidx, const double* __restrict__ Lvals, double* __restrict__ x, const double* __restrict__ rdiag);
+__global__ void pg_bin_pos_kernel(const int* __restrict__ binptr, const int* __restrict__ bincols, int* __restrict__ colpos);
+__global__ void pg_bwd_subtree_kernel(const int* __restrict__ bin_perm, const int* __restrict__ binptr, const int* __restrict__ bincols, const int* __restrict__ colptr, const int* __restrict__ rowidx, const int* __restrict__ anc_first, const int* __restrict__ colpos, const double* __restrict__ Lvals, double* __restrict__ x, const double* __restrict__ rdiag, int ncap);
+__global__ void pg_bwd_subtree_serial_kernel(const int* __restrict__ bin_perm, const int* __restrict__ binptr, const int* __restrict__ bincols, const int* __restrict__ colptr, const int* __restrict__ rowidx, const double* __restrict__ Lvals, double* __restrict__ x, const double* __restrict__ rdiag);
 __global__ void pg_front_asm_kernel(const int* __restrict__ it_front, const int* __restrict__ it_row, const pg_front* __restrict__ FD, const pg_child* __restrict__ CH, const int* __restrict__ rel, const int* __restrict__ xr_ptr, const int* __restrict__ xr_child, const int* __restrict__ xr_row, const int* __restrict__ fa_rowptr, const int* __restrict__ fa_src, const int* __restrict__ fa_col, const int* __restrict__ fa_tr, const double* __restrict__ aval, const double* __restrict__ x, double* __restrict__ F, double* __restrict__ R);
 __global__ void pg_front_syrk_kernel(const int* __restrict__ it_front, const int* __restrict__ it_step, const pg_front* __restrict__ FD, const int* __restrict__ tile_item, const int* __restrict__ tile_ij, double* __restrict__ F);
 __global__ void pg_front_diag4_kernel(const int* __restrict__ it_front, const int* __restrict__ it_step, const pg_front* __restrict__ FD, double* __restrict__ F, double* __restrict__ R, int* __restrict__ fail, double* __restrict__ Tinv);
```

Measured after the change: 9847 frames/s (median of 3 runs). About the same (+1.5%).
